# ChuhanZhou/News_Recommendation_Model

Hardware: NVIDIA B200
Metric: train_impressions_per_sec (higher is better)
Workload: dtype f32 (pair products as 3 x bf16 tcgen05 MMAs, fp32 accumulate; meets the fp32 tolerances)

## Files before the change

include/nrm_b200.h:

```cpp
#ifndef NRM_B200_H
#define NRM_B200_H

#include <stddef.h>
#include <stdint.h>

#ifdef __cplusplus
extern "C" {
#endif

#define NRM_OK            0
#define NRM_EINVAL       -1
#define NRM_EWORKSPACE   -2
#define NRM_ECUDA        -3
#define NRM_EUNSUPPORTED -4

#define NRM_PRECISION_FP32 0
#define NRM_PRECISION_BF16 1
#define NRM_PRECISION_BF16X3 2

#define NRM_MODE_BN_BATCH_STATS 1
#define NRM_MODE_KEEP_FOR_BWD   2
#define NRM_MODE_EVAL           0
#define NRM_MODE_TRAIN          3

int         nrm_version(void);
const char* nrm_last_error(void);

unsigned long long nrm_launch_count(void);
void        nrm_timing_enable(int on);
int         nrm_timing_report(char* buf, size_t buf_bytes);
int         nrm_debug_umma_selftest(const float* a0, const float* a1, const float* b0, const float* b1,
                                    float* out, int mode, int split, void* stream);

int         nrm_debug_mma_microbench(long long* out, int variant, int reps, int nk, void* stream);

size_t      nrm_peer_ctx_bytes(void);
size_t      nrm_peer_stats_bytes(void);
int         nrm_peer_flag_words(void);
int         nrm_peer_preload(void);
int         nrm_adam_step_allreduce(float* param, float* exp_avg, float* exp_avg_sq, long long n, void* adam_state,
                                    const void* peer_ctx, void* ticket, void* stream);
int         nrm_loss_backward_sparse(const long long* user_id, int B, int C, const float* grad_loss, float* dlogits, long long delta_numel,
                                     long long* sparse_uid, float* sparse_val, const void* scratch, size_t scratch_bytes, void* stream);
int         nrm_peer_wait_consumed(const void* adam_state, const void* peer_ctx, void* stream);
int         nrm_peer_allsum_stats(const double* local, int which, double* out, const void* adam_state, const void* peer_ctx, void* stream);

int         nrm_debug_rsprof(long long* host_out64);
long long   nrm_debug_ws_field(int B, int H, int C, int mode, const char* name, long long* bytes);
int         nrm_debug_headprof(long long* host_out32);

int         nrm_layout_entries(void);
const char* nrm_layout_name(int i);
long long   nrm_layout_offset(int i);
long long   nrm_layout_numel(int i);
long long   nrm_layout_fixed_floats(void);

size_t nrm_workspace_bytes(int B, int H, int C, int mode);
size_t nrm_workspace_e_offset(int B, int H, int C, int mode);

int nrm_forward(const double* x_history, const double* x_target, long long x_target_batch_stride,
                const double* x_global, long long x_global_batch_stride,
                int B, int H, int C,
                const float* params, float* bn_running_mean, float* bn_running_var,
                long long* bn_num_batches_tracked,
                int mode, int precision,
                float* logits, void* workspace, size_t workspace_bytes, void* stream);

int nrm_forward_encoder(const double* x_history, const double* x_target, long long x_target_batch_stride,
                        const double* x_global, long long x_global_batch_stride,
                        int B, int H, int C, const float* params, int mode, int precision,
                        double* bn_sums, void* workspace, size_t workspace_bytes, void* stream);
int nrm_forward_head(int B, int H, int C, const float* params, float* bn_running_mean, float* bn_running_var,
                     long long* bn_num_batches_tracked, int mode, int precision,
                     const double* bn_sums, long long bn_global_rows,
                     float* logits, void* workspace, size_t workspace_bytes, void* stream);

int nrm_backward(const double* x_history, const double* x_target, long long x_target_batch_stride,
                 const double* x_global, long long x_global_batch_stride,
                 int B, int H, int C, const float* params, int mode, int precision,
                 const float* dlogits, float* grads,
                 void* workspace, size_t workspace_bytes, void* stream);
int nrm_backward_head(int B, int H, int C, const float* params, int precision, const float* dlogits, float* grads,
                      double* bn_bwd_sums, void* workspace, size_t workspace_bytes, void* stream);
int nrm_backward_head_deferred(int B, int H, int C, const float* params, int precision, const float* dlogits, float* grads,
                               double* bn_bwd_sums, void* workspace, size_t workspace_bytes, void* stream);
int nrm_backward_encoder(const double* x_history, const double* x_target, long long x_target_batch_stride,
                         const double* x_global, long long x_global_batch_stride,
                         int B, int H, int C, const float* params, int mode, int precision,
                         const double* bn_bwd_sums, long long bn_global_rows, float* grads,
                         void* workspace, size_t workspace_bytes, void* stream);

typedef struct {
  const float* articles; int n_articles;
  const int* hist_article; const unsigned* hist_time; const float* hist_click;
  const int* cand_article; const unsigned* cand_time;
  const float* label32; double* label64;
} nrm_compact_batch;
int nrm_forward_compact(const nrm_compact_batch* batch, int B, int H, int C, const float* params, float* bn_running_mean,
                        float* bn_running_var, long long* bn_num_batches_tracked, int mode, int precision,
                        float* logits, void* workspace, size_t workspace_bytes, void* stream);
int nrm_forward_encoder_compact(const nrm_compact_batch* batch, int B, int H, int C, const float* params, int mode, int precision,
                                double* bn_sums, void* workspace, size_t workspace_bytes, void* stream);
int nrm_backward_compact(const nrm_compact_batch* batch, int B, int H, int C, const float* params, int mode, int precision,
                         const float* dlogits, float* grads, void* workspace, size_t workspace_bytes, void* stream);
int nrm_backward_encoder_compact(const nrm_compact_batch* batch, int B, int H, int C, const float* params, int mode, int precision,
                                 const double* bn_bwd_sums, long long bn_global_rows, float* grads, void* workspace,
                                 size_t workspace_bytes, void* stream);

int nrm_forward_scores(const double* x_history, const double* x_target, long long x_target_batch_stride,
                       const double* x_global, long long x_global_batch_stride, int B, int H, int C,
                       const float* params, float* bn_running_mean, float* bn_running_var, long long* bn_num_batches_tracked,
                       int mode, int precision, float* logits, float* scores, void* workspace, size_t workspace_bytes, void* stream);
int nrm_forward_scores_compact(const nrm_compact_batch* batch, int B, int H, int C, const float* params, float* bn_running_mean,
                               float* bn_running_var, long long* bn_num_batches_tracked, int mode, int precision,
                               float* logits, float* scores, void* workspace, size_t workspace_bytes, void* stream);
int nrm_history_topk(const float* scores, int B, int C, int H, int k, const double* x_history, const int* hist_article,
                     int* idx_out, float* val_out, void* stream);

size_t nrm_pool_workspace_bytes(int B, int H, int N, int chunk);
int nrm_forward_pool(const nrm_compact_batch* users, int B, int H, int N, int chunk, const float* params, const float* bn_running_mean,
                     const float* bn_running_var, int precision, float* logits, void* workspace, size_t workspace_bytes, void* stream);
int nrm_pool_topk(const float* logits, int n_models, long long model_stride, int B, int N, int k, const int* pool_article, int n_articles,
                  const int* hist_article, int H, int* pos_out, float* val_out, void* stream);

size_t nrm_loss_scratch_bytes(int B, int C);
int nrm_loss_forward(const float* logits, const float* delta, long long delta_numel,
                     const long long* user_id, const double* label, int B, int C, float alpha,
                     float* loss, void* scratch, size_t scratch_bytes, void* stream);
int nrm_loss_backward(const long long* user_id, int B, int C, const float* grad_loss,
                      float* dlogits, float* ddelta, long long delta_numel,
                      const void* scratch, size_t scratch_bytes, void* stream);

int nrm_adam_step(float* param, const float* grad, float* exp_avg, float* exp_avg_sq, long long n,
                  float lr, float beta1, float beta2, float eps, float weight_decay,
                  long long step, float grad_scale, void* stream);

int nrm_adam_step_device(float* param, const float* grad, float* exp_avg, float* exp_avg_sq, long long n,
                         void* adam_state, void* stream);

int nrm_batch_metrics(const float* scores, long long score_stride, const double* labels, long long label_stride,
                      const int* n_valid, int B, int C, int k, float* auc, float* hit, float* rr, float* ndcg,
                      void* stream);

int nrm_score_epilogue(const float* logits, int n_models, long long model_stride, long long row_stride, int B, int C,
                       const long long* empty_num, float* scores, int* ranks, void* stream);

size_t nrm_rank_strings_capacity(int B, int C);
int nrm_rank_strings(const long long* impression_id, const int* ranks, const long long* empty_num, int B, int C,
                     long long* offsets, char* out, long long capacity, void* stream);

int nrm_expand_compact(const float* articles, int n_articles, const int* hist_article, const unsigned* hist_time,
                       const float* hist_click, const int* cand_article, const unsigned* cand_time, const float* label32,
                       int B, int H, int C, double* x_history, double* x_target, double* x_global, double* label64,
                       void* stream);

#ifdef __cplusplus
}
#endif
#endif
```

news_recommendation_model_b200/_lib.py:

```python
from __future__ import annotations

import ctypes as C
import os
import subprocess
import threading

_HERE = os.path.dirname(os.path.abspath(__file__))
CSRC = os.path.join(_HERE, 'csrc')
LIB_PATH = os.path.join(CSRC, 'libnrm_b200.so')

_lock = threading.Lock()
_lib = None

vp, ll, i32, f32, sz = C.c_void_p, C.c_longlong, C.c_int, C.c_float, C.c_size_t

SIGNATURES = {
    'nrm_version': (i32, []),
    'nrm_last_error': (C.c_char_p, []),
    'nrm_launch_count': (C.c_ulonglong, []),
    'nrm_timing_enable': (None, [i32]),
    'nrm_timing_report': (i32, [C.c_char_p, sz]),
    'nrm_debug_umma_selftest': (i32, [vp, vp, vp, vp, vp, i32, i32, vp]),
    'nrm_debug_mma_microbench': (i32, [vp, i32, i32, i32, vp]),
    'nrm_debug_rsprof': (i32, [vp]),
    'nrm_debug_headprof': (i32, [vp]),
    'nrm_debug_ws_field': (ll, [i32, i32, i32, i32, C.c_char_p, vp]),
    'nrm_layout_entries': (i32, []),
    'nrm_layout_name': (C.c_char_p, [i32]),
    'nrm_layout_offset': (ll, [i32]),
    'nrm_layout_numel': (ll, [i32]),
    'nrm_layout_fixed_floats': (ll, []),
    'nrm_workspace_bytes': (sz, [i32, i32, i32, i32]),
    'nrm_workspace_e_offset': (sz, [i32, i32, i32, i32]),
    'nrm_forward': (i32, [vp, vp, ll, vp, ll, i32, i32, i32, vp, vp, vp, vp, i32, i32, vp, vp, sz, vp]),
    'nrm_forward_encoder': (i32, [vp, vp, ll, vp, ll, i32, i32, i32, vp, i32, i32, vp, vp, sz, vp]),
    'nrm_forward_head': (i32, [i32, i32, i32, vp, vp, vp, vp, i32, i32, vp, ll, vp, vp, sz, vp]),
    'nrm_backward': (i32, [vp, vp, ll, vp, ll, i32, i32, i32, vp, i32, i32, vp, vp, vp, sz, vp]),
    'nrm_forward_compact': (i32, [vp, i32, i32, i32, vp, vp, vp, vp, i32, i32, vp, vp, sz, vp]),
    'nrm_forward_encoder_compact': (i32, [vp, i32, i32, i32, vp, i32, i32, vp, vp, sz, vp]),
    'nrm_backward_compact': (i32, [vp, i32, i32, i32, vp, i32, i32, vp, vp, vp, sz, vp]),
    'nrm_backward_encoder_compact': (i32, [vp, i32, i32, i32, vp, i32, i32, vp, ll, vp, vp, sz, vp]),
    'nrm_backward_head': (i32, [i32, i32, i32, vp, i32, vp, vp, vp, vp, sz, vp]),
    'nrm_backward_head_deferred': (i32, [i32, i32, i32, vp, i32, vp, vp, vp, vp, sz, vp]),
    'nrm_backward_encoder': (i32, [vp, vp, ll, vp, ll, i32, i32, i32, vp, i32, i32, vp, ll, vp, vp, sz, vp]),
    'nrm_loss_scratch_bytes': (sz, [i32, i32]),
    'nrm_loss_forward': (i32, [vp, vp, ll, vp, vp, i32, i32, f32, vp, vp, sz, vp]),
    'nrm_loss_backward': (i32, [vp, i32, i32, vp, vp, vp, ll, vp, sz, vp]),
    'nrm_adam_step': (i32, [vp, vp, vp, vp, ll, f32, f32, f32, f32, f32, ll, f32, vp]),
    'nrm_adam_step_device': (i32, [vp, vp, vp, vp, ll, vp, vp]),
    'nrm_peer_ctx_bytes': (sz, []),
    'nrm_peer_stats_bytes': (sz, []),
    'nrm_peer_flag_words': (i32, []),
    'nrm_peer_preload': (i32, []),
    'nrm_adam_step_allreduce': (i32, [vp, vp, vp, ll, vp, vp, vp, vp]),
    'nrm_peer_wait_consumed': (i32, [vp, vp, vp]),
    'nrm_loss_backward_sparse': (i32, [vp, i32, i32, vp, vp, ll, vp, vp, vp, sz, vp]),
    'nrm_peer_allsum_stats': (i32, [vp, i32, vp, vp, vp, vp]),
    'nrm_batch_metrics': (i32, [vp, ll, vp, ll, vp, i32, i32, i32, vp, vp, vp, vp, vp]),
    'nrm_score_epilogue': (i32, [vp, i32, ll, ll, i32, i32, vp, vp, vp, vp]),
    'nrm_rank_strings_capacity': (sz, [i32, i32]),
    'nrm_rank_strings': (i32, [vp, vp, vp, i32, i32, vp, vp, ll, vp]),
    'nrm_expand_compact': (i32, [vp, i32, vp, vp, vp, vp, vp, vp, i32, i32, i32, vp, vp, vp, vp, vp]),
    'nrm_forward_scores': (i32, [vp, vp, ll, vp, ll, i32, i32, i32, vp, vp, vp, vp, i32, i32, vp, vp, vp, sz, vp]),
    'nrm_forward_scores_compact': (i32, [vp, i32, i32, i32, vp, vp, vp, vp, i32, i32, vp, vp, vp, sz, vp]),
    'nrm_history_topk': (i32, [vp, i32, i32, i32, i32, vp, vp, vp, vp, vp]),
    'nrm_pool_workspace_bytes': (sz, [i32, i32, i32, i32]),
    'nrm_forward_pool': (i32, [vp, i32, i32, i32, i32, vp, vp, vp, i32, vp, vp, sz, vp]),
    'nrm_pool_topk': (i32, [vp, i32, ll, i32, i32, i32, vp, i32, vp, i32, vp, vp, vp]),
}


class NrmError(RuntimeError):
    pass


def build(verbose: bool = False) -> str:
    out = subprocess.run(['make', '-C', CSRC, '-j8'], capture_output=True, text=True)
    if verbose or out.returncode != 0:
        print(out.stdout[-4000:])
        print(out.stderr[-4000:])
    if out.returncode != 0:
        raise NrmError('building libnrm_b200.so failed (see make output above)')
    return LIB_PATH


def load():
    global _lib
    with _lock:
        if _lib is not None:
            return _lib
        if not os.path.exists(LIB_PATH):
            raise NrmError(f'{LIB_PATH} is missing: run `python -c "import __graft_entry__ as g; g.build()"` '
                           f'(or `make -C {CSRC}`); there is no CPU fallback')
        lib = C.CDLL(LIB_PATH)
        for name, (res, args) in SIGNATURES.items():
            fn = getattr(lib, name)
            fn.restype = res
            fn.argtypes = args
        _lib = lib
        return lib


def check(rc: int, what: str) -> None:
    if rc != 0:
        msg = load().nrm_last_error().decode('utf-8', 'replace')
        raise NrmError(f'{what} failed with code {rc}: {msg}')


def layout():
    lib = load()
    entries = [(lib.nrm_layout_name(i).decode(), int(lib.nrm_layout_offset(i)), int(lib.nrm_layout_numel(i)))
               for i in range(lib.nrm_layout_entries())]
    return entries, int(lib.nrm_layout_fixed_floats())


class CompactBatchStruct(C.Structure):
    _fields_ = [('articles', C.c_void_p), ('n_articles', C.c_int), ('hist_article', C.c_void_p), ('hist_time', C.c_void_p),
                ('hist_click', C.c_void_p), ('cand_article', C.c_void_p), ('cand_time', C.c_void_p), ('label32', C.c_void_p),
                ('label64', C.c_void_p)]
```

news_recommendation_model_b200/csrc/nrm_api.cu:

```cuda
#include <cstdarg>
#include <cstdio>
#include <cstring>
#include <mutex>
#include <vector>

#include "nrm_kernels.cuh"

namespace nrm {

static thread_local char g_err[512] = "";

void set_error(const char* fmt, ...) {
  va_list ap;
  va_start(ap, fmt);
  vsnprintf(g_err, sizeof(g_err), fmt, ap);
  va_end(ap);
}
int cuda_fail(cudaError_t e, const char* what) {
  set_error("CUDA error %d (%s) at %s", (int)e, cudaGetErrorString(e), what);
  return NRM_ECUDA;
}
int current_device() {
  int dev = 0;
  if (cudaGetDevice(&dev) != cudaSuccess || dev < 0 || dev >= 64) return 0;
  return dev;
}
int sm_count() {
  static int n[64] = {};
  const int dev = current_device();
  int v = __atomic_load_n(&n[dev], __ATOMIC_RELAXED);
  if (v == 0) {
    if (cudaDeviceGetAttribute(&v, cudaDevAttrMultiProcessorCount, dev) != cudaSuccess || v <= 0) v = 148;
    __atomic_store_n(&n[dev], v, __ATOMIC_RELAXED);
  }
  return v;
}

static unsigned long long g_launches = 0;
void count_launch() { __atomic_fetch_add(&g_launches, 1ULL, __ATOMIC_RELAXED); }

constexpr int kTimerSlots = 40, kTimerRing = 256;
struct TimerSlot { const char* name; cudaEvent_t beg[kTimerRing], end[kTimerRing]; int used; bool made; };
static TimerSlot g_timers[kTimerSlots];
static int g_ntimers = 0;
static bool g_timing = false;
static std::mutex g_timer_mu;

KernelTimer::KernelTimer(const char* name, cudaStream_t stream) : slot_(-1), stream_(stream) {
  if (!g_timing) return;
  std::lock_guard<std::mutex> lock(g_timer_mu);
  int s = -1;
  for (int i = 0; i < g_ntimers; ++i) if (strcmp(g_timers[i].name, name) == 0) { s = i; break; }
  if (s < 0) { if (g_ntimers == kTimerSlots) return; s = g_ntimers++; g_timers[s].name = name; g_timers[s].used = 0; g_timers[s].made = false; }
  TimerSlot& t = g_timers[s];
  if (!t.made) { for (int i = 0; i < kTimerRing; ++i) { cudaEventCreate(&t.beg[i]); cudaEventCreate(&t.end[i]); } t.made = true; }
  if (t.used >= kTimerRing) return;
  slot_ = s;
  cudaEventRecord(t.beg[t.used], stream_);
}
KernelTimer::~KernelTimer() {
  if (slot_ < 0) return;
  std::lock_guard<std::mutex> lock(g_timer_mu);
  TimerSlot& t = g_timers[slot_];
  cudaEventRecord(t.end[t.used], stream_);
  t.used++;
}

struct SideStream {
  int dev; cudaStream_t caller;
  cudaStream_t stream; cudaEvent_t fork, join, fork2, join2, fork0, join0, join_tp, fork3, join3, fork4, join4;
  bool head_wgrad_pending = false; const float* wg_params = nullptr; float* wg_grads = nullptr; int wg_tiles = 0, wg_precision = 0;
};
static std::mutex g_side_mu;
static std::vector<SideStream*> g_sides;
static SideStream* side_stream(cudaStream_t caller) {
  const int dev = current_device();
  std::lock_guard<std::mutex> lock(g_side_mu);
  for (SideStream* p : g_sides)
    if (p->dev == dev && p->caller == caller) return p;
  SideStream* ss = new SideStream();
  ss->dev = dev; ss->caller = caller;
  bool ok = cudaStreamCreateWithFlags(&ss->stream, cudaStreamNonBlocking) == cudaSuccess;
  cudaEvent_t* evs[] = {&ss->fork, &ss->join, &ss->fork2, &ss->join2, &ss->fork0, &ss->join0, &ss->join_tp, &ss->fork3, &ss->join3,
                        &ss->fork4, &ss->join4};
  for (cudaEvent_t* e : evs) ok = ok && cudaEventCreateWithFlags(e, cudaEventDisableTiming) == cudaSuccess;
  if (!ok) { delete ss; return nullptr; }
  g_sides.push_back(ss);
  return ss;
}

bool pdl_enabled() {
  static const bool on = getenv("NRM_NO_PDL") == nullptr;
  return on;
}

struct LayoutEntry { const char* name; long long offset; long long numel; };
#define II "invariant_interest_model."
static const LayoutEntry kLayout[] = {
    {II "category_embedding.0.weight", P_CAT, NCAT * 32},
    {II "sentiment_embedding.0.weight", P_SENT_W, 16 * 3},
    {II "sentiment_embedding.0.bias", P_SENT_B, 16},
    {II "type_embedding.0.weight", P_TYPE, NTYPE * 8},
    {II "w1.weight", P_W1_W, 64 * XIN},
    {II "w1.bias", P_W1_B, 64},
    {II "year_embedding.0.weight", P_YEAR, NYEAR * 8},
    {II "month_embedding.0.weight", P_MONTH, NMONTH * 8},
    {II "day_embedding.0.weight", P_DAY, NDAY * 8},
    {II "hour_embedding.0.weight", P_HOUR, NHOUR * 8},
    {II "label_attention.mlp.fc1.weight", P_LA_FC1_W, 64 * 256},
    {II "label_attention.mlp.fc1.bias", P_LA_FC1_B, 64},
    {II "label_attention.mlp.fc2.weight", P_LA_FC2_W, 64},
    {II "label_attention.mlp.fc2.bias", P_LA_FC2_B, 1},
    {II "text_img_attention.mlp.fc1.weight", P_TI_FC1_W, 64 * 256},
    {II "text_img_attention.mlp.fc1.bias", P_TI_FC1_B, 64},
    {II "text_img_attention.mlp.fc2.weight", P_TI_FC2_W, 64},
    {II "text_img_attention.mlp.fc2.bias", P_TI_FC2_B, 1},
    {"instant_interest_model.out_fc.0.weight", P_INST_W, 8 * 3},
    {"instant_interest_model.out_fc.0.bias", P_INST_B, 8},
    {"bn.weight", P_BN_W, E},
    {"bn.bias", P_BN_B, E},
    {"gate.fc1.weight", P_GATE_FC1_W, HID * E},
    {"gate.fc1.bias", P_GATE_FC1_B, HID},
    {"gate.fc2.weight", P_GATE_FC2_W, E * HID},
    {"gate.fc2.bias", P_GATE_FC2_B, E},
    {"mlp.fc1.weight", P_MLP_FC1_W, HID * E},
    {"mlp.fc1.bias", P_MLP_FC1_B, HID},
    {"mlp.fc2.weight", P_MLP_FC2_W, E * HID},
    {"mlp.fc2.bias", P_MLP_FC2_B, E},
    {"out_mlp.fc1.weight", P_OUT_FC1_W, HID * E},
    {"out_mlp.fc1.bias", P_OUT_FC1_B, HID},
    {"out_mlp.fc2.weight", P_OUT_FC2_W, HID},
    {"out_mlp.fc2.bias", P_OUT_FC2_B, 1},
    {"delta", P_DELTA, -1},
};
#undef II
constexpr int kLayoutEntries = sizeof(kLayout) / sizeof(kLayout[0]);

size_t carve_workspace(Workspace& w, void* base, int B, int H, int C, int mode) {
  const bool training = (mode & NRM_MODE_KEEP_FOR_BWD) != 0;
  memset(&w, 0, sizeof(w));
  w.B = B; w.H = H; w.C = C;
  w.NH = (long long)B * H; w.R = (long long)B * C; w.N = w.NH + w.R;
  size_t off = 0;
  auto take = [&](size_t bytes) -> void* {
    void* p = base ? (char*)base + off : nullptr;
    off += (bytes + 255) & ~(size_t)255;
    return p;
  };
  const size_t f = sizeof(float);
  const size_t NH = (size_t)w.NH, R = (size_t)w.R, N = (size_t)w.N;
  w.xin_h = (float*)take(f * NH * XIN);
  w.xh = (float*)take(f * NH * 64);
  w.pca_h = (float*)take(f * NH * 64);
  w.e = (float*)take(f * R * E);
  w.mean = (float*)take(f * E);
  w.rstd = (float*)take(f * E);
  w.bn_sums = (double*)take(sizeof(double) * 2 * E);
  w.stat_part = (double*)take(sizeof(double) * STAT_BLOCKS * 2 * E);
  w.a1 = (float*)take(f * R * HID);
  w.gate = (float*)take(f * R * E);
  w.a2 = (float*)take(f * R * HID);
  w.y = (float*)take(f * R * E);
  w.a3 = (float*)take(f * R * HID);
  w.head_wt = (float*)take(f * (HEAD_WT_W1T + 64 * XIN));
  w.tp = (float*)take(f * 2 * R * 64);
  w.att_rs_img = (float*)take(attention_rs_image_bytes());
  w.head_img = (float*)take(head_tc_image_bytes());
  w.head_arrive = (unsigned int*)take(256);
  if (training) {
    w.da3 = (float*)take(f * R * HID); w.da2 = (float*)take(f * R * HID); w.da1 = (float*)take(f * R * HID);
    w.dy = (float*)take(f * R * E);
    w.dgate = (float*)take(f * R * E);
    w.de = (float*)take(f * R * E);
    w.dz = (float*)take(f * R * E);
    w.bn_bwd_sums = (double*)take(sizeof(double) * 2 * E);
    w.head_part_f = (float*)take(f * ((R + 31) / 32) * 68);
    w.head_part_bn = (double*)take(sizeof(double) * ((R + 31) / 32) * 2 * E);
    w.head_part_w = (float*)take(f * 5 * HEAD_WG_CHUNKS_MAX * (HID * E + E));
    w.dxh = (float*)take(f * NH * 64);
    w.dxt = (float*)take(f * R * 64);
    w.dxin_h = (float*)take(f * NH * XIN);
    {
      const size_t ffma = (size_t)ATT_BWD_CTAS_MAX * ATT_PARTIAL, tc = (size_t)ATT_TC_PARTS_MAX * ATT_TC_PARTIAL;
      w.att_part = (float*)take(f * 2 * (ffma > tc ? ffma : tc));
    }
    w.dtp = (float*)take(f * 2 * R * 64);
    {
      const size_t tiles = (size_t)attention_rs_tiles(B, H, C);
      w.att_dhid = (unsigned char*)take(tiles * 2 * 16384);
      w.att_sc = (float*)take(f * tiles * 512);
    }
    w.att_dA = (float*)take(f * 2 * 4096);
    w.tp_part = (float*)take(f * 2 * ((R + 31) / 32) * (4096 + 64));
    w.splitk = (float*)take(f * (size_t)(64 * XIN + 64) * W1_SPLITS);
    w.small_part = (float*)take(f * 1024 * 96);
    const size_t n32 = N * 6, n8 = N * 5;
    const size_t c32 = (n32 + SORT_CHUNK - 1) / SORT_CHUNK, c8 = (n8 + SORT_CHUNK - 1) / SORT_CHUNK;
    const size_t g32 = n32 / SEG_GROUP + NKEY32 + 1, g8 = n8 / SEG_GROUP + NKEY8 + 1;
    w.keys32 = (int*)take(sizeof(int) * n32); w.keys8 = (int*)take(sizeof(int) * n8);
    w.perm32 = (int*)take(sizeof(int) * n32); w.perm8 = (int*)take(sizeof(int) * n8);
    w.chunk_hist32 = (int*)take(sizeof(int) * c32 * NKEY32); w.chunk_hist8 = (int*)take(sizeof(int) * c8 * NKEY8);
    w.seg32 = (int*)take(sizeof(int) * 3 * (NKEY32 + 1)); w.seg8 = (int*)take(sizeof(int) * 3 * (NKEY8 + 1));
    w.gkey32 = (int*)take(sizeof(int) * g32); w.gkey8 = (int*)take(sizeof(int) * g8);
    w.gpart32 = (float*)take(f * g32 * 32); w.gpart8 = (float*)take(f * g8 * 8);
  }
  w.bytes = off;
  return off;
}

static int check_shape(const char* fn, int B, int H, int C) {
  if (B <= 0 || H <= 0 || C <= 0) { set_error("%s: B, H, C must be positive (got %d, %d, %d)", fn, B, H, C); return NRM_EINVAL; }
  if (((long long)B * H + (long long)B * C) * 6 >= (1LL << 31)) { set_error("%s: batch too large for 32-bit entry ids", fn); return NRM_EINVAL; }
  return NRM_OK;
}
static int get_workspace(const char* fn, Workspace& w, void* ws, size_t ws_bytes, int B, int H, int C, int mode) {
  if (ws == nullptr || ((uintptr_t)ws & 255) != 0) { set_error("%s: workspace must be non-null and 256-byte aligned", fn); return NRM_EWORKSPACE; }
  const size_t need = carve_workspace(w, ws, B, H, C, mode);
  if (need > ws_bytes) { set_error("%s: workspace too small (%zu < %zu bytes)", fn, ws_bytes, need); return NRM_EWORKSPACE; }
  return NRM_OK;
}

static int encoder_forward(const BatchPtrs& in, const float* P, Workspace& w, int mode, int precision, cudaStream_t s) {
  SideStream* ss = side_stream(s);
  if (ss == nullptr) { set_error("encoder_forward: cannot create the side stream"); return NRM_ECUDA; }
  const bool tc = precision != NRM_PRECISION_FP32;
  NRM_CUDA(cudaEventRecord(ss->fork0, s));
  NRM_CUDA(cudaStreamWaitEvent(ss->stream, ss->fork0, 0));
  NRM_TRY(launch_head_transpose(P, w, ss->stream));
  NRM_CUDA(cudaEventRecord(ss->join0, ss->stream));
  if (tc) {
    NRM_TRY(launch_attention_prep_rs(P, w, ss->stream));
    NRM_TRY(launch_head_images_tc(P, w, precision, (mode & NRM_MODE_KEEP_FOR_BWD) != 0, ss->stream));
  }
  { KernelTimer t("embed_rows", s);
    NRM_TRY(launch_embed_rows(in, P, w, (mode & NRM_MODE_KEEP_FOR_BWD) != 0, s)); }
  NRM_CUDA(cudaEventRecord(ss->fork, s));
  NRM_CUDA(cudaStreamWaitEvent(ss->stream, ss->fork, 0));
  if (tc) NRM_TRY(launch_candidate_tp(P, w, ss->stream));
  NRM_CUDA(cudaEventRecord(ss->join_tp, ss->stream));
  if (mode & NRM_MODE_KEEP_FOR_BWD) {
    NRM_TRY(launch_table_sort(w, ss->stream));
    NRM_CUDA(cudaEventRecord(ss->join, ss->stream));
  }
  NRM_CUDA(cudaStreamWaitEvent(s, ss->join0, 0));
  { KernelTimer t("w1_forward", s); NRM_TRY(launch_w1_forward(P, w, s)); }
  NRM_CUDA(cudaStreamWaitEvent(s, ss->join_tp, 0));
  if (!tc) {
    { KernelTimer t("attention_forward_label", s); NRM_TRY(launch_attention_forward(in, P, w, 0, precision, s)); }
    { KernelTimer t("attention_forward_textimg", s); NRM_TRY(launch_attention_forward(in, P, w, 1, precision, s)); }
  } else {
    KernelTimer t("attention_forward", s);
    NRM_TRY(launch_attention_forward_rs(in, w, precision, s));
  }
  if (mode & NRM_MODE_KEEP_FOR_BWD) NRM_CUDA(cudaStreamWaitEvent(s, ss->join, 0));
  return NRM_OK;
}

static int encoder_backward(const BatchPtrs& in, const float* P, Workspace& w, int precision, float* G, cudaStream_t s) {
  SideStream* ss = side_stream(s);
  if (ss == nullptr) { set_error("encoder_backward: cannot create the side stream"); return NRM_ECUDA; }
  const bool tc = precision != NRM_PRECISION_FP32;
  { KernelTimer t("attention_backward_label", s);
    if (tc) NRM_TRY(launch_attention_backward_rs(w, 0, precision, true, s)); else NRM_TRY(launch_attention_backward(in, P, w, 0, precision, s)); }
  if (tc) {
    KernelTimer t("attention_input_grad_label", s);
    NRM_TRY(launch_attention_input_grad_rs(w, precision, s));
  }
  NRM_CUDA(cudaEventRecord(ss->fork2, s));
  NRM_CUDA(cudaStreamWaitEvent(ss->stream, ss->fork2, 0));
  { KernelTimer t("attention_backward_textimg", s);
    if (tc) NRM_TRY(launch_attention_backward_rs(w, 1, precision, false, s)); else NRM_TRY(launch_attention_backward(in, P, w, 1, precision, s)); }
  { KernelTimer t("w1_backward", ss->stream);
    if (tc) NRM_TRY(launch_w1_backward_tc(P, w, G, precision, ss->stream)); else NRM_TRY(launch_w1_backward(P, w, G, ss->stream)); }
  NRM_CUDA(cudaEventRecord(ss->join2, ss->stream));
  if (ss->head_wgrad_pending) {
    ss->head_wgrad_pending = false;
    KernelTimer t("head_wgrad", ss->stream);
    NRM_TRY(launch_head_backward_wgrad(ss->wg_params, w, ss->wg_grads, ss->stream, ss->wg_tiles, ss->wg_precision));
  }
  { KernelTimer t("attention_finish", s);
    if (tc) NRM_TRY(launch_attention_finish_tc(P, w, G, s));
    else { NRM_TRY(launch_attention_finish(P, w, 0, precision, G, s)); NRM_TRY(launch_attention_finish(P, w, 1, precision, G, s)); } }
  NRM_CUDA(cudaStreamWaitEvent(s, ss->join2, 0));
  NRM_CUDA(cudaEventRecord(ss->fork3, s));
  NRM_CUDA(cudaStreamWaitEvent(ss->stream, ss->fork3, 0));
  { KernelTimer t("small_linear_grads", ss->stream); NRM_TRY(launch_small_linear_grads(in, w, G, ss->stream)); }
  NRM_CUDA(cudaEventRecord(ss->join3, ss->stream));
  NRM_TRY(launch_table_grads(w, G, s));
  NRM_CUDA(cudaStreamWaitEvent(s, ss->join3, 0));
  return NRM_OK;
}

}

using namespace nrm;

extern "C" int nrm_version(void) { return 100; }
extern "C" unsigned long long nrm_launch_count(void) { return __atomic_load_n(&g_launches, __ATOMIC_RELAXED); }
extern "C" void nrm_timing_enable(int on) {
  std::lock_guard<std::mutex> lock(g_timer_mu);
  g_timing = on != 0;
  for (int i = 0; i < g_ntimers; ++i) g_timers[i].used = 0;
}
extern "C" int nrm_timing_report(char* buf, size_t buf_bytes) {
  if (!buf || buf_bytes == 0) { set_error("nrm_timing_report: bad buffer"); return NRM_EINVAL; }
  size_t off = 0;
  buf[0] = 0;
  std::lock_guard<std::mutex> lock(g_timer_mu);
  for (int i = 0; i < g_ntimers; ++i) {
    TimerSlot& t = g_timers[i];
    double total = 0.0;
    for (int k = 0; k < t.used; ++k) {
      float ms = 0.f;
      NRM_CUDA(cudaEventSynchronize(t.end[k]));
      NRM_CUDA(cudaEventElapsedTime(&ms, t.beg[k], t.end[k]));
      total += ms;
    }
    float t_beg = 0.f, t_end = 0.f;
    if (t.used > 0 && g_ntimers > 0 && g_timers[0].used > 0) {
      cudaEventElapsedTime(&t_beg, g_timers[0].beg[g_timers[0].used - 1], t.beg[t.used - 1]);
      cudaEventElapsedTime(&t_end, g_timers[0].beg[g_timers[0].used - 1], t.end[t.used - 1]);
    }
    const int n = snprintf(buf + off, buf_bytes - off, "%s %d %.6f %.6f %.6f\n", t.name, t.used, total, t_beg, t_end);
    if (n < 0 || (size_t)n >= buf_bytes - off) break;
    off += (size_t)n;
  }
  return NRM_OK;
}
extern "C" int nrm_debug_rsprof(long long* host_out64) { return rsprof_read(host_out64); }
extern "C" long long nrm_debug_ws_field(int B, int H, int C, int mode, const char* name, long long* bytes) {
  if (B <= 0 || H <= 0 || C <= 0 || !name || !bytes) return -1;
  Workspace w;
  carve_workspace(w, reinterpret_cast<void*>(uintptr_t(256)), B, H, C, mode);
  const size_t R = (size_t)w.R, NH = (size_t)w.NH;
  struct F { const char* n; const void* p; size_t b; };
  const F fields[] = {{"e", w.e, R * E * 4}, {"de", w.de, R * E * 4}, {"dz", w.dz, R * E * 4}, {"dxh", w.dxh, NH * 64 * 4}, {"dxt", w.dxt, R * 64 * 4},
                      {"dxin_h", w.dxin_h, NH * XIN * 4}, {"att_dhid", w.att_dhid, (size_t)attention_rs_tiles(B, H, C) * 2 * 16384},
                      {"att_sc", w.att_sc, (size_t)attention_rs_tiles(B, H, C) * 512 * 4}, {"xh", w.xh, NH * 64 * 4}, {"dtp", w.dtp, 2 * R * 64 * 4},
                      {"tp", w.tp, 2 * R * 64 * 4}};
  for (const F& f : fields)
    if (strcmp(f.n, name) == 0 && f.p != nullptr) { *bytes = (long long)f.b; return (long long)(reinterpret_cast<uintptr_t>(f.p) - 256); }
  return -1;
}
extern "C" int nrm_debug_headprof(long long* host_out32) { return headprof_read(host_out32); }
extern "C" const char* nrm_last_error(void) { return g_err; }
extern "C" int nrm_layout_entries(void) { return kLayoutEntries; }
extern "C" const char* nrm_layout_name(int i) { return (i >= 0 && i < kLayoutEntries) ? kLayout[i].name : nullptr; }
extern "C" long long nrm_layout_offset(int i) { return (i >= 0 && i < kLayoutEntries) ? kLayout[i].offset : -1; }
extern "C" long long nrm_layout_numel(int i) { return (i >= 0 && i < kLayoutEntries) ? kLayout[i].numel : -1; }
extern "C" long long nrm_layout_fixed_floats(void) { return P_DELTA; }

extern "C" size_t nrm_workspace_bytes(int B, int H, int C, int mode) {
  if (B <= 0 || H <= 0 || C <= 0) return 0;
  Workspace w;
  return carve_workspace(w, nullptr, B, H, C, mode);
}

extern "C" size_t nrm_workspace_e_offset(int B, int H, int C, int mode) {
  if (B <= 0 || H <= 0 || C <= 0) return 0;
  Workspace w;
  carve_workspace(w, reinterpret_cast<void*>(uintptr_t(256)), B, H, C, mode);
  return (size_t)(reinterpret_cast<uintptr_t>(w.e) - 256);
}

static int forward_encoder_impl(const char* fn, const BatchPtrs& in, int B, int H, int C, const float* params, int mode, int precision,
                                double* bn_sums, void* workspace, size_t workspace_bytes, void* stream) {
  Workspace w;
  NRM_TRY(get_workspace(fn, w, workspace, workspace_bytes, B, H, C, mode));
  cudaStream_t s = (cudaStream_t)stream;
  NRM_TRY(encoder_forward(in, params, w, mode, precision, s));
  if (mode & NRM_MODE_BN_BATCH_STATS) {
    KernelTimer t("bn_statistics", s);
    NRM_TRY(launch_bn_partial_sums(w, s));
    if (bn_sums != nullptr && bn_sums != w.bn_sums)
      NRM_CUDA(cudaMemcpyAsync(bn_sums, w.bn_sums, sizeof(double) * 2 * E, cudaMemcpyDeviceToDevice, s));
  }
  return NRM_OK;
}

static int compact_batch(const char* fn, const nrm_compact_batch* cb, int precision, CompactPtrs& cp) {
  if (!cb || !cb->articles || cb->n_articles <= 0 || !cb->hist_article || !cb->hist_time || !cb->hist_click || !cb->cand_article || !cb->cand_time ||
      (cb->label32 && !cb->label64)) {
    set_error("%s: bad compact batch", fn); return NRM_EINVAL;
  }
  if ((reinterpret_cast<uintptr_t>(cb->articles) & 15) != 0) { set_error("%s: the article table must be 16-byte aligned", fn); return NRM_EINVAL; }
  if (precision == NRM_PRECISION_FP32) {
    set_error("%s: the compact wire format is read directly by the tensor-core precisions only (use nrm_expand_compact otherwise)", fn);
    return NRM_EUNSUPPORTED;
  }
  cp = CompactPtrs{cb->articles, cb->n_articles, cb->hist_article, cb->hist_time, cb->hist_click, cb->cand_article, cb->cand_time,
                   cb->label32, cb->label64};
  return NRM_OK;
}

extern "C" int nrm_forward_encoder(const double* x_history, const double* x_target, long long xt_bs, const double* x_global,
                                   long long xg_bs, int B, int H, int C, const float* params, int mode, int precision,
                                   double* bn_sums, void* workspace, size_t workspace_bytes, void* stream) {
  NRM_TRY(check_shape("nrm_forward_encoder", B, H, C));
  if (!x_history || !x_target || !x_global || !params) { set_error("nrm_forward_encoder: null pointer"); return NRM_EINVAL; }
  if (xt_bs < (long long)C * TC || xg_bs < (long long)C * GC) { set_error("nrm_forward_encoder: batch stride smaller than one impression"); return NRM_EINVAL; }
  const BatchPtrs in{x_history, x_target, xt_bs, x_global, xg_bs};
  return forward_encoder_impl("nrm_forward_encoder", in, B, H, C, params, mode, precision, bn_sums, workspace, workspace_bytes, stream);
}

extern "C" int nrm_forward_encoder_compact(const nrm_compact_batch* batch, int B, int H, int C, const float* params, int mode, int precision,
                                           double* bn_sums, void* workspace, size_t workspace_bytes, void* stream) {
  NRM_TRY(check_shape("nrm_forward_encoder_compact", B, H, C));
  if (!params) { set_error("nrm_forward_encoder_compact: null pointer"); return NRM_EINVAL; }
  CompactPtrs cp;
  NRM_TRY(compact_batch("nrm_forward_encoder_compact", batch, precision, cp));
  BatchPtrs in{nullptr, nullptr, 0, nullptr, 0};
  in.compact = &cp;
  return forward_encoder_impl("nrm_forward_encoder_compact", in, B, H, C, params, mode, precision, bn_sums, workspace, workspace_bytes, stream);
}

extern "C" int nrm_forward_head(int B, int H, int C, const float* params, float* bn_running_mean, float* bn_running_var,
                                  long long* bn_num_batches_tracked, int mode, int precision, const double* bn_sums,
                                  long long bn_global_rows, float* logits, void* workspace, size_t workspace_bytes,
                                  void* stream) {
  const int training = mode & NRM_MODE_BN_BATCH_STATS;
  NRM_TRY(check_shape("nrm_forward_head", B, H, C));
  if (!params || !bn_running_mean || !bn_running_var || !logits) { set_error("nrm_forward_head: null pointer"); return NRM_EINVAL; }
  if (training && !bn_num_batches_tracked) { set_error("nrm_forward_head: null num_batches_tracked"); return NRM_EINVAL; }
  Workspace w;
  NRM_TRY(get_workspace("nrm_forward_head", w, workspace, workspace_bytes, B, H, C, mode));
  const double* sums = bn_sums ? bn_sums : w.bn_sums;
  const long long rows = bn_global_rows > 0 ? bn_global_rows : w.R;
  KernelTimer t("head_forward", (cudaStream_t)stream);
  if (precision != NRM_PRECISION_FP32)
    return launch_head_forward_tc(params, w, precision, bn_running_mean, bn_running_var, bn_num_batches_tracked, training,
                                  (mode & NRM_MODE_KEEP_FOR_BWD) != 0, sums, rows, logits, (cudaStream_t)stream);
  return launch_head_forward(params, w, bn_running_mean, bn_running_var, bn_num_batches_tracked, training,
                             (mode & NRM_MODE_KEEP_FOR_BWD) != 0, sums, rows,
                             logits, (cudaStream_t)stream);
}

extern "C" int nrm_forward(const double* x_history, const double* x_target, long long xt_bs, const double* x_global,
                           long long xg_bs, int B, int H, int C, const float* params, float* bn_running_mean,
                           float* bn_running_var, long long* bn_num_batches_tracked, int mode, int precision,
                           float* logits, void* workspace, size_t workspace_bytes, void* stream) {
  NRM_TRY(nrm_forward_encoder(x_history, x_target, xt_bs, x_global, xg_bs, B, H, C, params, mode, precision, nullptr,
                              workspace, workspace_bytes, stream));
  return nrm_forward_head(B, H, C, params, bn_running_mean, bn_running_var, bn_num_batches_tracked, mode, precision, nullptr, 0,
                            logits, workspace, workspace_bytes, stream);
}

extern "C" int nrm_forward_compact(const nrm_compact_batch* batch, int B, int H, int C, const float* params, float* bn_running_mean,
                                   float* bn_running_var, long long* bn_num_batches_tracked, int mode, int precision,
                                   float* logits, void* workspace, size_t workspace_bytes, void* stream) {
  NRM_TRY(nrm_forward_encoder_compact(batch, B, H, C, params, mode, precision, nullptr, workspace, workspace_bytes, stream));
  return nrm_forward_head(B, H, C, params, bn_running_mean, bn_running_var, bn_num_batches_tracked, mode, precision, nullptr, 0,
                            logits, workspace, workspace_bytes, stream);
}

static int forward_scores_impl(const char* fn, const BatchPtrs& in, int B, int H, int C, const float* params, float* bn_running_mean,
                               float* bn_running_var, long long* bn_num_batches_tracked, int mode, int precision, float* logits,
                               float* scores, void* workspace, size_t workspace_bytes, void* stream) {
  if (mode != NRM_MODE_EVAL) { set_error("%s: scores are exported by eval-mode forwards only (mode must be NRM_MODE_EVAL, got %d)", fn, mode); return NRM_EINVAL; }
  if (!scores) { set_error("%s: null scores", fn); return NRM_EINVAL; }
  Workspace w;
  NRM_TRY(get_workspace(fn, w, workspace, workspace_bytes, B, H, C, mode));
  w.scores = scores;
  NRM_TRY(encoder_forward(in, params, w, mode, precision, (cudaStream_t)stream));
  return nrm_forward_head(B, H, C, params, bn_running_mean, bn_running_var, bn_num_batches_tracked, mode, precision, nullptr, 0,
                          logits, workspace, workspace_bytes, stream);
}

extern "C" int nrm_forward_scores(const double* x_history, const double* x_target, long long xt_bs, const double* x_global,
                                  long long xg_bs, int B, int H, int C, const float* params, float* bn_running_mean,
                                  float* bn_running_var, long long* bn_num_batches_tracked, int mode, int precision,
                                  float* logits, float* scores, void* workspace, size_t workspace_bytes, void* stream) {
  NRM_TRY(check_shape("nrm_forward_scores", B, H, C));
  if (!x_history || !x_target || !x_global || !params) { set_error("nrm_forward_scores: null pointer"); return NRM_EINVAL; }
  if (xt_bs < (long long)C * TC || xg_bs < (long long)C * GC) { set_error("nrm_forward_scores: batch stride smaller than one impression"); return NRM_EINVAL; }
  const BatchPtrs in{x_history, x_target, xt_bs, x_global, xg_bs};
  return forward_scores_impl("nrm_forward_scores", in, B, H, C, params, bn_running_mean, bn_running_var, bn_num_batches_tracked, mode,
                             precision, logits, scores, workspace, workspace_bytes, stream);
}

extern "C" int nrm_forward_scores_compact(const nrm_compact_batch* batch, int B, int H, int C, const float* params, float* bn_running_mean,
                                          float* bn_running_var, long long* bn_num_batches_tracked, int mode, int precision,
                                          float* logits, float* scores, void* workspace, size_t workspace_bytes, void* stream) {
  NRM_TRY(check_shape("nrm_forward_scores_compact", B, H, C));
  if (!params) { set_error("nrm_forward_scores_compact: null pointer"); return NRM_EINVAL; }
  CompactPtrs cp;
  NRM_TRY(compact_batch("nrm_forward_scores_compact", batch, precision, cp));
  BatchPtrs in{nullptr, nullptr, 0, nullptr, 0};
  in.compact = &cp;
  return forward_scores_impl("nrm_forward_scores_compact", in, B, H, C, params, bn_running_mean, bn_running_var, bn_num_batches_tracked,
                             mode, precision, logits, scores, workspace, workspace_bytes, stream);
}

struct PoolCarve { double* xh; double* xt; double* xg; float* out; void* ws; size_t ws_bytes, bytes; };
static void carve_pool(PoolCarve& pc, void* base, int B, int H, int N, int chunk) {
  const int C = chunk < N ? chunk : N;
  size_t off = 0;
  auto take = [&](size_t bytes) -> void* {
    void* p = base ? (char*)base + off : nullptr;
    off += (bytes + 255) & ~(size_t)255;
    return p;
  };
  pc.xh = (double*)take(sizeof(double) * B * H * HC);
  pc.xt = (double*)take(sizeof(double) * C * TC);
  pc.xg = (double*)take(sizeof(double) * C * GC);
  pc.out = (float*)take(sizeof(float) * B * C);
  Workspace w;
  pc.ws_bytes = carve_workspace(w, nullptr, B, H, C, NRM_MODE_EVAL);
  pc.ws = take(pc.ws_bytes);
  pc.bytes = off;
}

extern "C" size_t nrm_pool_workspace_bytes(int B, int H, int N, int chunk) {
  if (B <= 0 || H <= 0 || N <= 0 || chunk <= 0) return 0;
  PoolCarve pc;
  carve_pool(pc, nullptr, B, H, N, chunk);
  return pc.bytes;
}

extern "C" int nrm_forward_pool(const nrm_compact_batch* users, int B, int H, int N, int chunk, const float* params,
                                const float* bn_running_mean, const float* bn_running_var, int precision, float* logits,
                                void* workspace, size_t workspace_bytes, void* stream) {
  const char* fn = "nrm_forward_pool";
  if (B <= 0 || H <= 0 || N <= 0) { set_error("%s: B, H, N must be positive (got %d, %d, %d)", fn, B, H, N); return NRM_EINVAL; }
  if (chunk <= 0 || chunk % 8 != 0) { set_error("%s: chunk must be a positive multiple of 8 (got %d)", fn, chunk); return NRM_EINVAL; }
  if (precision < NRM_PRECISION_FP32 || precision > NRM_PRECISION_BF16X3) { set_error("%s: unknown precision %d", fn, precision); return NRM_EINVAL; }
  if (!users || !users->articles || users->n_articles <= 0 || !users->hist_article || !users->hist_time || !users->hist_click ||
      !users->cand_article || !users->cand_time) {
    set_error("%s: bad compact batch", fn); return NRM_EINVAL;
  }
  if (users->label32 || users->label64) { set_error("%s: the pool has no labels (label32 / label64 must be null)", fn); return NRM_EINVAL; }
  if ((reinterpret_cast<uintptr_t>(users->articles) & 15) != 0) { set_error("%s: the article table must be 16-byte aligned", fn); return NRM_EINVAL; }
  if (!params || !bn_running_mean || !bn_running_var || !logits) { set_error("%s: null pointer", fn); return NRM_EINVAL; }
  const int C = chunk < N ? chunk : N;
  NRM_TRY(check_shape(fn, B, H, C));
  if (workspace == nullptr || ((uintptr_t)workspace & 255) != 0) { set_error("%s: workspace must be non-null and 256-byte aligned", fn); return NRM_EWORKSPACE; }
  PoolCarve pc;
  carve_pool(pc, workspace, B, H, N, chunk);
  if (pc.bytes > workspace_bytes) { set_error("%s: workspace too small (%zu < %zu bytes)", fn, workspace_bytes, pc.bytes); return NRM_EWORKSPACE; }
  cudaStream_t s = (cudaStream_t)stream;
  const nrm_compact_batch& u = *users;
  NRM_TRY(launch_expand_compact(u.articles, u.n_articles, u.hist_article, u.hist_time, u.hist_click, nullptr, nullptr, nullptr, (long long)B * H, 0,
                                pc.xh, nullptr, nullptr, nullptr, s));
  float* run_mean = const_cast<float*>(bn_running_mean);
  float* run_var = const_cast<float*>(bn_running_var);
  for (int c0 = 0; c0 < N; c0 += C) {
    const int nc = N - c0 < C ? N - c0 : C;
    NRM_TRY(launch_expand_compact(u.articles, u.n_articles, nullptr, nullptr, nullptr, u.cand_article + c0, u.cand_time + c0, nullptr, 0, nc,
                                  nullptr, pc.xt, pc.xg, nullptr, s));
    const BatchPtrs in{pc.xh, pc.xt, 0, pc.xg, 0};
    NRM_TRY(forward_encoder_impl(fn, in, B, H, nc, params, NRM_MODE_EVAL, precision, nullptr, pc.ws, pc.ws_bytes, stream));
    float* out = nc == N ? logits : pc.out;
    NRM_TRY(nrm_forward_head(B, H, nc, params, run_mean, run_var, nullptr, NRM_MODE_EVAL, precision, nullptr, 0, out, pc.ws, pc.ws_bytes, stream));
    if (out != logits)
      NRM_CUDA(cudaMemcpy2DAsync(logits + c0, sizeof(float) * N, out, sizeof(float) * nc, sizeof(float) * nc, B, cudaMemcpyDeviceToDevice, s));
  }
  return NRM_OK;
}

static int backward_head(const char* fn, bool defer_wgrad, int B, int H, int C, const float* params, int precision, const float* dlogits, float* grads,
                         double* bn_bwd_sums, void* workspace, size_t workspace_bytes, void* stream) {
  NRM_TRY(check_shape(fn, B, H, C));
  if (!params || !dlogits || !grads) { set_error("%s: null pointer", fn); return NRM_EINVAL; }
  Workspace w;
  NRM_TRY(get_workspace(fn, w, workspace, workspace_bytes, B, H, C, NRM_MODE_KEEP_FOR_BWD));
  cudaStream_t s = (cudaStream_t)stream;
  const bool tc = precision != NRM_PRECISION_FP32;
  const int tiles = tc ? head_tc_tiles(w.R) : 0;
  if (!defer_wgrad) {
    KernelTimer t("head_backward", s);
    if (tc) NRM_TRY(launch_head_backward_dgrad_tc(params, w, precision, dlogits, grads, s));
    else { NRM_TRY(launch_head_backward_dgrad(params, w, dlogits, s)); NRM_TRY(launch_head_backward_bn(w, grads, s, 0)); }
    NRM_TRY(launch_head_backward_wgrad(params, w, grads, s, tiles, tc ? precision : 0));
  } else {
    SideStream* ss = side_stream(s);
    if (ss == nullptr) { set_error("%s: cannot create the side stream", fn); return NRM_ECUDA; }
    KernelTimer t("head_backward", s);
    if (tc) NRM_TRY(launch_head_backward_dgrad_tc(params, w, precision, dlogits, grads, s)); else NRM_TRY(launch_head_backward_dgrad(params, w, dlogits, s));
    ss->head_wgrad_pending = true; ss->wg_params = params; ss->wg_grads = grads; ss->wg_tiles = tiles; ss->wg_precision = tc ? precision : 0;
    if (!tc) NRM_TRY(launch_head_backward_bn(w, grads, s, 0));
  }
  if (bn_bwd_sums != nullptr && bn_bwd_sums != w.bn_bwd_sums)
    NRM_CUDA(cudaMemcpyAsync(bn_bwd_sums, w.bn_bwd_sums, sizeof(double) * 2 * E, cudaMemcpyDeviceToDevice, s));
  return NRM_OK;
}

extern "C" int nrm_backward_head(int B, int H, int C, const float* params, int precision, const float* dlogits, float* grads,
                                 double* bn_bwd_sums, void* workspace, size_t workspace_bytes, void* stream) {
  return backward_head("nrm_backward_head", false, B, H, C, params, precision, dlogits, grads, bn_bwd_sums, workspace, workspace_bytes, stream);
}

extern "C" int nrm_backward_head_deferred(int B, int H, int C, const float* params, int precision, const float* dlogits, float* grads,
                                          double* bn_bwd_sums, void* workspace, size_t workspace_bytes, void* stream) {
  return backward_head("nrm_backward_head_deferred", true, B, H, C, params, precision, dlogits, grads, bn_bwd_sums, workspace, workspace_bytes, stream);
}

static int backward_encoder_impl(const char* fn, const BatchPtrs& in, int B, int H, int C, const float* params, int mode, int precision,
                                 const double* bn_bwd_sums, long long bn_global_rows, float* grads, void* workspace, size_t workspace_bytes,
                                 void* stream) {
  const int training = mode & NRM_MODE_BN_BATCH_STATS;
  Workspace w;
  NRM_TRY(get_workspace(fn, w, workspace, workspace_bytes, B, H, C, NRM_MODE_KEEP_FOR_BWD));
  cudaStream_t s = (cudaStream_t)stream;
  const double* sums = bn_bwd_sums ? bn_bwd_sums : w.bn_bwd_sums;
  const long long rows = bn_global_rows > 0 ? bn_global_rows : w.R;
  NRM_TRY(launch_bn_backward_combine(params, w, training, sums, rows, precision != NRM_PRECISION_FP32, s));
  return encoder_backward(in, params, w, precision, grads, s);
}

extern "C" int nrm_backward_encoder(const double* x_history, const double* x_target, long long xt_bs,
                                    const double* x_global, long long xg_bs, int B, int H, int C, const float* params,
                                    int mode, int precision, const double* bn_bwd_sums, long long bn_global_rows,
                                    float* grads, void* workspace, size_t workspace_bytes, void* stream) {
  NRM_TRY(check_shape("nrm_backward_encoder", B, H, C));
  if (!x_history || !x_target || !x_global || !params || !grads) { set_error("nrm_backward_encoder: null pointer"); return NRM_EINVAL; }
  const BatchPtrs in{x_history, x_target, xt_bs, x_global, xg_bs};
  return backward_encoder_impl("nrm_backward_encoder", in, B, H, C, params, mode, precision, bn_bwd_sums, bn_global_rows, grads, workspace,
                               workspace_bytes, stream);
}

extern "C" int nrm_backward_encoder_compact(const nrm_compact_batch* batch, int B, int H, int C, const float* params, int mode, int precision,
                                            const double* bn_bwd_sums, long long bn_global_rows, float* grads, void* workspace,
                                            size_t workspace_bytes, void* stream) {
  NRM_TRY(check_shape("nrm_backward_encoder_compact", B, H, C));
  if (!params || !grads) { set_error("nrm_backward_encoder_compact: null pointer"); return NRM_EINVAL; }
  CompactPtrs cp;
  NRM_TRY(compact_batch("nrm_backward_encoder_compact", batch, precision, cp));
  BatchPtrs in{nullptr, nullptr, 0, nullptr, 0};
  in.compact = &cp;
  return backward_encoder_impl("nrm_backward_encoder_compact", in, B, H, C, params, mode, precision, bn_bwd_sums, bn_global_rows, grads, workspace,
                               workspace_bytes, stream);
}

static int backward_impl(const char* fn, const BatchPtrs& in, int B, int H, int C, const float* params, int mode, int precision,
                         const float* dlogits, float* grads, void* workspace, size_t workspace_bytes, void* stream) {
  const int training = mode & NRM_MODE_BN_BATCH_STATS;
  Workspace w;
  NRM_TRY(get_workspace(fn, w, workspace, workspace_bytes, B, H, C, NRM_MODE_KEEP_FOR_BWD));
  cudaStream_t s = (cudaStream_t)stream;
  SideStream* ss = side_stream(s);
  if (ss == nullptr) { set_error("%s: cannot create the side stream", fn); return NRM_ECUDA; }
  const bool htc = precision != NRM_PRECISION_FP32;
  const int tiles = htc ? head_tc_tiles(w.R) : 0;
  { KernelTimer t("head_backward", s);
    if (htc) NRM_TRY(launch_head_backward_dgrad_tc(params, w, precision, dlogits, grads, s)); else NRM_TRY(launch_head_backward_dgrad(params, w, dlogits, s));
    ss->head_wgrad_pending = true; ss->wg_params = params; ss->wg_grads = grads; ss->wg_tiles = tiles; ss->wg_precision = htc ? precision : 0;
    if (!htc) NRM_TRY(launch_head_backward_bn(w, grads, s, 0)); }
  NRM_TRY(launch_bn_backward_combine(params, w, training, w.bn_bwd_sums, w.R, htc, s));
  return encoder_backward(in, params, w, precision, grads, s);
}

extern "C" int nrm_backward(const double* x_history, const double* x_target, long long xt_bs, const double* x_global,
                            long long xg_bs, int B, int H, int C, const float* params, int mode, int precision,
                            const float* dlogits, float* grads, void* workspace, size_t workspace_bytes, void* stream) {
  NRM_TRY(check_shape("nrm_backward", B, H, C));
  if (!x_history || !x_target || !x_global || !params || !dlogits || !grads) { set_error("nrm_backward: null pointer"); return NRM_EINVAL; }
  const BatchPtrs in{x_history, x_target, xt_bs, x_global, xg_bs};
  return backward_impl("nrm_backward", in, B, H, C, params, mode, precision, dlogits, grads, workspace, workspace_bytes, stream);
}

extern "C" int nrm_backward_compact(const nrm_compact_batch* batch, int B, int H, int C, const float* params, int mode, int precision,
                                    const float* dlogits, float* grads, void* workspace, size_t workspace_bytes, void* stream) {
  NRM_TRY(check_shape("nrm_backward_compact", B, H, C));
  if (!params || !dlogits || !grads) { set_error("nrm_backward_compact: null pointer"); return NRM_EINVAL; }
  CompactPtrs cp;
  NRM_TRY(compact_batch("nrm_backward_compact", batch, precision, cp));
  BatchPtrs in{nullptr, nullptr, 0, nullptr, 0};
  in.compact = &cp;
  return backward_impl("nrm_backward_compact", in, B, H, C, params, mode, precision, dlogits, grads, workspace, workspace_bytes, stream);
}
```

news_recommendation_model_b200/csrc/nrm_head_tc.cu:

```cuda
#include "nrm_kernels.cuh"
#include <cstddef>

#include "nrm_umma.cuh"

namespace nrm {
namespace htc {

#ifdef NRM_RS_PROFILE
__device__ long long g_hprof[32];
#define HPROF(role, kind, stmt) do { const long long t__ = clock64(); stmt; if (blockIdx.x == 0 && (threadIdx.x & 31) == 0) g_hprof[(role) * 8 + (kind)] += clock64() - t__; } while (0)
#else
#define HPROF(role, kind, stmt) do { stmt; } while (0)
#endif

constexpr int ROWS = 64;
constexpr int N_EPI = 16;
constexpr int W_MMA = 16, W_LOAD = 17;
constexpr int THREADS = 32 * 20;
constexpr int EPI_THREADS = 32 * N_EPI;
constexpr int KE = 272, KH = 80;
constexpr int NN = 72;
constexpr int NW0 = 136, NW1 = 128;
constexpr uint32_t A_LBO = ROWS * 16;
constexpr uint32_t AW_PART = (KE / 8) * A_LBO;
constexpr uint32_t AN_PART = (KH / 8) * A_LBO;
constexpr uint32_t BN_LBO = NN * 16;
constexpr uint32_t BW_LBO = E * 16;
constexpr int NCHUNK = 5;
constexpr uint32_t SLOT = 3 * 8 * BN_LBO;
constexpr int STAGES = 3;
constexpr uint32_t IMG_STRIDE = 3 * (KH / 8) * BW_LBO;
constexpr uint32_t COL_W = 0, COL_N = 160, TMEM_COLS = 256;
constexpr int PAR_GAMMA = 0, PAR_BETA = E, PAR_BG2 = 2 * E, PAR_BM2 = 3 * E, PAR_BG1 = 4 * E, PAR_BM1 = 4 * E + NN, PAR_BO1 = 4 * E + 2 * NN,
              PAR_WO2 = 4 * E + 3 * NN, PAR_FLOATS = 8 * E;

__host__ __device__ constexpr int narrow_chunk_kb(int c) { return c < 4 ? 8 : 2; }
template <int NP> __host__ __device__ constexpr uint32_t narrow_chunk_off(int c) { return (uint32_t)c * NP * 8 * BN_LBO; }
template <int NP> __host__ __device__ constexpr uint32_t wide_chunk_off(int c) { return (uint32_t)c * NP * 2 * BW_LBO; }

__host__ __device__ constexpr int n_products(int NP) { return NP == 1 ? 1 : NP == 2 ? 3 : 6; }
__host__ __device__ constexpr int prod_a(int NP, int p) { return NP == 2 ? (p == 2 ? 1 : 0) : (p == 2 || p == 3) ? 1 : p == 5 ? 2 : 0; }
__host__ __device__ constexpr int prod_b(int NP, int p) { return NP == 2 ? (p == 1 ? 1 : 0) : (p == 1 || p == 3) ? 1 : p == 4 ? 2 : 0; }

template <int NP>
__device__ __forceinline__ void split_store8(unsigned char* dst, uint32_t part_bytes, const float* v) {
  uint32_t h[4], m[4], l[4];
#pragma unroll
  for (int i = 0; i < 4; ++i) {
    const float a = v[2 * i], b = v[2 * i + 1];
    const __nv_bfloat162 hh = __floats2bfloat162_rn(a, b);
    h[i] = *reinterpret_cast<const uint32_t*>(&hh);
    if (NP >= 2) {
      const float ra = a - __uint_as_float(h[i] << 16), rb = b - __uint_as_float(h[i] & 0xffff0000u);
      const __nv_bfloat162 mm = __floats2bfloat162_rn(ra, rb);
      m[i] = *reinterpret_cast<const uint32_t*>(&mm);
      if (NP >= 3) {
        const __nv_bfloat162 ll = __floats2bfloat162_rn(ra - __uint_as_float(m[i] << 16), rb - __uint_as_float(m[i] & 0xffff0000u));
        l[i] = *reinterpret_cast<const uint32_t*>(&ll);
      }
    }
  }
  *reinterpret_cast<uint4*>(dst) = make_uint4(h[0], h[1], h[2], h[3]);
  if (NP >= 2) *reinterpret_cast<uint4*>(dst + part_bytes) = make_uint4(m[0], m[1], m[2], m[3]);
  if (NP >= 3) *reinterpret_cast<uint4*>(dst + 2 * part_bytes) = make_uint4(l[0], l[1], l[2], l[3]);
}

struct ImgDesc { long long src; int so, si, narrow; };
__constant__ ImgDesc c_img[10] = {
    {P_GATE_FC1_W, E, 1, 1},   {P_GATE_FC2_W, HID, 1, 0}, {P_MLP_FC1_W, E, 1, 1},  {P_MLP_FC2_W, HID, 1, 0}, {P_OUT_FC1_W, E, 1, 1},
    {P_OUT_FC1_W, 1, E, 0},    {P_MLP_FC2_W, 1, HID, 1},  {P_MLP_FC1_W, 1, E, 0},  {P_GATE_FC2_W, 1, HID, 1}, {P_GATE_FC1_W, 1, E, 0}};

template <int NP>
__global__ void __launch_bounds__(256)
head_image_kernel(const float* __restrict__ P, unsigned char* __restrict__ img, int first_layer, unsigned int* __restrict__ arrive) {
  pdl_wait();
  pdl_trigger();
  if (blockIdx.x == 0 && blockIdx.y == 0 && threadIdx.x == 0) *arrive = 0u;
  const int layer = first_layer + blockIdx.y;
  const ImgDesc d = c_img[layer];
  const float* src = P + d.src;
  unsigned char* out = img + (size_t)layer * IMG_STRIDE;
  const int nrow = d.narrow ? NN : E, nkb = d.narrow ? KE / 8 : KH / 8;
  const int nout = d.narrow ? HID : E, nin = d.narrow ? E : HID;
  for (int it = blockIdx.x * 256 + threadIdx.x; it < nrow * nkb; it += gridDim.x * 256) {
    const int n = it % nrow, kb = it / nrow;
    float v[8];
#pragma unroll
    for (int i = 0; i < 8; ++i) {
      const int k = 8 * kb + i;
      v[i] = (n < nout && k < nin) ? __ldg(src + (long long)n * d.so + (long long)k * d.si) : 0.f;
    }
    uint32_t off, part;
    if (d.narrow) {
      const int c = kb < 32 ? kb >> 3 : 4, kbl = kb - 8 * c;
      part = (uint32_t)narrow_chunk_kb(c) * BN_LBO;
      off = narrow_chunk_off<NP>(c) + (uint32_t)kbl * BN_LBO;
    } else {
      const int c = kb >> 1, kbl = kb & 1;
      part = 2 * BW_LBO;
      off = wide_chunk_off<NP>(c) + (uint32_t)kbl * BW_LBO;
    }
    split_store8<NP>(out + off + (uint32_t)(n >> 3) * 128u + (uint32_t)(n & 7) * 16u, part, v);
  }
}

struct Smem {
  __align__(128) unsigned char aw[3 * AW_PART];
  __align__(128) unsigned char an[3 * AN_PART];
  __align__(128) unsigned char ring[STAGES][SLOT];
  float mean[E], rstd[E];
  float red[4][ROWS + 4];
  float par[PAR_FLOATS];
  uint64_t full[STAGES], empty[STAGES];
  uint64_t a_ready, d_ready;
  uint32_t tmem_base;
};

__device__ __forceinline__ void epi_sync() { __syncwarp(); asm volatile("bar.sync 1, %0;\n" ::"n"(EPI_THREADS) : "memory"); }
__device__ __forceinline__ void operand_written(uint64_t* bar) {
  umma::fence_async_smem();
  umma::fence_before_sync();
  __syncwarp();
  if ((threadIdx.x & 31) == 0) umma::mbar_arrive(bar);
}

template <int NP>
__device__ __forceinline__ void loader(Smem& sm, const unsigned char* __restrict__ img, int first_layer, bool first_narrow, long long my_tiles) {
  uint32_t g = 0;
  for (long long t = 0; t < my_tiles; ++t)
    for (int l = 0; l < 5; ++l) {
      const bool narrow = ((l & 1) == 0) == first_narrow;
      const unsigned char* base = img + (size_t)(first_layer + l) * IMG_STRIDE;
      for (int c = 0; c < NCHUNK; ++c, ++g) {
        const int slot = g % STAGES, use = g / STAGES;
        if (use > 0) HPROF(0, 0, umma::mbar_wait(&sm.empty[slot], (uint32_t)((use - 1) & 1)));
        const uint32_t off = narrow ? narrow_chunk_off<NP>(c) : wide_chunk_off<NP>(c);
        const uint32_t bytes = narrow ? (uint32_t)(NP * narrow_chunk_kb(c)) * BN_LBO : (uint32_t)NP * 2 * BW_LBO;
        umma::bulk_load(sm.ring[slot], base + off, bytes, &sm.full[slot]);
      }
    }
}

template <int NP, int KS>
__device__ __forceinline__ void narrow_chunk(uint32_t tmem_d, uint32_t a_addr, uint32_t b_addr, bool accumulate) {
  constexpr uint32_t ID_N = umma::make_idesc_bf16(64, NN);
  constexpr uint32_t bpart = (uint32_t)(2 * KS) * BN_LBO;
#pragma unroll
  for (int p = 0; p < n_products(NP); ++p) {
    const uint64_t da = umma::make_desc(a_addr + prod_a(NP, p) * AW_PART, A_LBO, 128);
    const uint64_t db = umma::make_desc(b_addr + prod_b(NP, p) * bpart, BN_LBO, 128);
#pragma unroll
    for (int ks = 0; ks < KS; ++ks)
      umma::mma_bf16(tmem_d, da + (uint64_t)(ks * ((2 * A_LBO) >> 4)), db + (uint64_t)(ks * ((2 * BN_LBO) >> 4)), ID_N,
                     (accumulate || p > 0 || ks > 0) ? 1u : 0u);
  }
}

template <int NP>
__device__ __forceinline__ void issuer(Smem& sm, uint32_t tmem, bool first_narrow, long long my_tiles) {
  constexpr uint32_t ID_W0 = umma::make_idesc_bf16(64, NW0), ID_W1 = umma::make_idesc_bf16(64, NW1);
  const uint32_t aw = umma::smem_u32(sm.aw), an = umma::smem_u32(sm.an);
  uint32_t g = 0, ause = 0;
  for (long long t = 0; t < my_tiles; ++t)
    for (int l = 0; l < 5; ++l) {
      const bool narrow = ((l & 1) == 0) == first_narrow;
      HPROF(1, 0, umma::mbar_wait(&sm.a_ready, ause & 1));
      ++ause;
      umma::fence_after_sync();
      for (int c = 0; c < NCHUNK; ++c, ++g) {
        const int slot = g % STAGES;
        HPROF(1, 1, umma::mbar_wait(&sm.full[slot], (uint32_t)((g / STAGES) & 1)));
        umma::fence_after_sync();
        const uint32_t rb = umma::smem_u32(sm.ring[slot]);
        if (narrow) {
          const uint32_t a0 = aw + (uint32_t)(8 * c) * A_LBO;
          if (c < 4) narrow_chunk<NP, 4>(tmem + COL_N, a0, rb, c > 0);
          else narrow_chunk<NP, 1>(tmem + COL_N, a0, rb, true);
        } else {
#pragma unroll
          for (int p = 0; p < n_products(NP); ++p) {
            const uint64_t da = umma::make_desc(an + prod_a(NP, p) * AN_PART + (uint32_t)(2 * c) * A_LBO, A_LBO, 128);
            const uint64_t db = umma::make_desc(rb + prod_b(NP, p) * (2 * BW_LBO), BW_LBO, 128);
            const uint32_t acc = (c > 0 || p > 0) ? 1u : 0u;
            umma::mma_bf16(tmem + COL_W, da, db, ID_W0, acc);
            umma::mma_bf16(tmem + COL_W + (16u << 16), da, db + (uint64_t)(((NW0 / 8) * 128) >> 4), ID_W1, acc);
          }
        }
        umma::mma_commit(&sm.empty[slot]);
      }
      umma::mma_commit(&sm.d_ready);
    }
}

__device__ __forceinline__ int wide_kb0(int q) { return q == 0 ? 0 : 4 * q + 1; }
__device__ __forceinline__ int wide_nkb(int q) { return q == 0 ? 5 : 4; }
__device__ __forceinline__ int narrow_kb0(int q) { return q == 0 ? 0 : 2 * q + 1; }
__device__ __forceinline__ int narrow_nkb(int q) { return q == 0 ? 3 : 2; }

__device__ __forceinline__ void load_wide(uint32_t tmem_lane, int q, float* v ) {
  const uint32_t a = tmem_lane + COL_W + 8 * wide_kb0(q);
  umma::tmem_ld32(a, v);
  if (q == 0) umma::tmem_ld8(a + 32, v + 32);
}
__device__ __forceinline__ void load_narrow(uint32_t tmem_lane, int q, float* v ) {
  const uint32_t a = tmem_lane + COL_N + 8 * narrow_kb0(q);
  umma::tmem_ld16(a, v);
  if (q == 0) umma::tmem_ld8(a + 16, v + 16);
}

__device__ __forceinline__ uint32_t a_off(int row, int kb) { return (uint32_t)kb * A_LBO + (uint32_t)(row >> 3) * 128u + (uint32_t)(row & 7) * 16u; }

template <int NP>
__global__ void __launch_bounds__(THREADS, 1)
head_forward_tc_kernel(const float* __restrict__ e, const double* __restrict__ bn_sums, long long bn_rows, int training,
                       float* __restrict__ run_mean, float* __restrict__ run_var, long long* __restrict__ nbt,
                       float* __restrict__ mean_out, float* __restrict__ rstd_out, const float* __restrict__ P,
                       const unsigned char* __restrict__ img, long long R, int keep, float* __restrict__ a1g, float* __restrict__ gateg,
                       float* __restrict__ a2g, float* __restrict__ yg, float* __restrict__ a3g, float* __restrict__ logits) {
#ifdef NRM_RS_PROFILE
  const long long t_entry = clock64();
#endif
  pdl_wait();
  pdl_trigger();
  extern __shared__ __align__(128) unsigned char smem_raw[];
  Smem& sm = *reinterpret_cast<Smem*>(smem_raw);
  const int tid = threadIdx.x, warp = tid >> 5, lane = tid & 31;
  const long long ntiles = (R + ROWS - 1) / ROWS;
  const long long my_tiles = (long long)blockIdx.x < ntiles ? (ntiles - 1 - blockIdx.x) / gridDim.x + 1 : 0;
  if (tid == 0) {
    for (int j = 0; j < STAGES; ++j) { umma::mbar_init(&sm.full[j], 1); umma::mbar_init(&sm.empty[j], 1); }
    umma::mbar_init(&sm.a_ready, N_EPI);
    umma::mbar_init(&sm.d_ready, 1);
  }
  if (warp == W_MMA) umma::tmem_alloc(&sm.tmem_base, TMEM_COLS);
  if (tid < ROWS) {
#pragma unroll
    for (int p = 0; p < 3; ++p) {
      *reinterpret_cast<uint4*>(sm.aw + p * AW_PART + a_off(tid, KE / 8 - 1)) = make_uint4(0, 0, 0, 0);
      *reinterpret_cast<uint4*>(sm.an + p * AN_PART + a_off(tid, KH / 8 - 1)) = make_uint4(0, 0, 0, 0);
    }
  }
  umma::fence_async_smem();
  umma::fence_before_sync();
  __syncthreads();
  umma::fence_after_sync();
  const uint32_t tmem = sm.tmem_base;

  if (warp >= N_EPI) {
    asm volatile("setmaxnreg.dec.sync.aligned.u32 32;\n");
    if (warp == W_LOAD) {
      if (umma::elect_one()) HPROF(0, 7, loader<NP>(sm, img, 0, true, my_tiles));
    } else if (warp == W_MMA) {
      if (umma::elect_one()) HPROF(1, 7, issuer<NP>(sm, tmem, true, my_tiles));
    }
  } else {
    asm volatile("setmaxnreg.inc.sync.aligned.u32 112;\n");
    const int sp = warp & 3, q = warp >> 2, l16 = lane & 15, half = lane >> 4;
    const int row = 16 * sp + l16;
    const uint32_t tmem_lane = tmem + ((uint32_t)(32 * sp) << 16);
    for (int i = tid; i < E; i += EPI_THREADS) {
      sm.par[PAR_GAMMA + i] = __ldg(P + P_BN_W + i); sm.par[PAR_BETA + i] = __ldg(P + P_BN_B + i);
      sm.par[PAR_BG2 + i] = __ldg(P + P_GATE_FC2_B + i); sm.par[PAR_BM2 + i] = __ldg(P + P_MLP_FC2_B + i);
    }
    if (tid < NN) {
      const bool in = tid < HID;
      sm.par[PAR_BG1 + tid] = in ? __ldg(P + P_GATE_FC1_B + tid) : 0.f; sm.par[PAR_BM1 + tid] = in ? __ldg(P + P_MLP_FC1_B + tid) : 0.f;
      sm.par[PAR_BO1 + tid] = in ? __ldg(P + P_OUT_FC1_B + tid) : 0.f;  sm.par[PAR_WO2 + tid] = in ? __ldg(P + P_OUT_FC2_W + tid) : 0.f;
    }
    if (tid < E) {
      const int n = tid;
      float m, v;
      if (training) {
        const double dm = bn_sums[n] / (double)bn_rows;
        double dv = bn_sums[E + n] / (double)bn_rows - dm * dm;
        if (dv < 0.0) dv = 0.0;
        m = (float)dm; v = (float)dv;
        if (blockIdx.x == 0) {
          const double unbiased = bn_rows > 1 ? dv * (double)bn_rows / (double)(bn_rows - 1) : dv;
          run_mean[n] = (1.f - BN_MOMENTUM) * run_mean[n] + BN_MOMENTUM * m;
          run_var[n] = (1.f - BN_MOMENTUM) * run_var[n] + BN_MOMENTUM * (float)unbiased;
          if (n == 0) *nbt += 1;
        }
      } else {
        m = run_mean[n]; v = run_var[n];
      }
      const float rs = 1.0f / sqrtf(v + BN_EPS);
      sm.mean[n] = m; sm.rstd[n] = rs;
      if (blockIdx.x == 0) { mean_out[n] = m; rstd_out[n] = rs; }
    }
    constexpr int PRO_ITEMS = ROWS * (E / 8), PRO_IT = (PRO_ITEMS + EPI_THREADS - 1) / EPI_THREADS;
    auto load_e_items = [&](long long r0, int nr, float4 (&ev)[PRO_IT][2]) {
#pragma unroll
      for (int u = 0; u < PRO_IT; ++u) {
        const int it = tid + u * EPI_THREADS, r = it & (ROWS - 1), kb = it >> 6;
        ev[u][0] = ev[u][1] = make_float4(0.f, 0.f, 0.f, 0.f);
        if (it < PRO_ITEMS && r < nr) {
          const float4* ep = reinterpret_cast<const float4*>(e + (r0 + r) * E + 8 * kb);
          ev[u][0] = __ldg(ep); ev[u][1] = __ldg(ep + 1);
        }
      }
    };
    epi_sync();
#ifdef NRM_RS_PROFILE
    if (blockIdx.x == 0 && tid == 0) g_hprof[24] += clock64() - t_entry;
#endif
    uint32_t duse = 0;
    for (long long t = 0; t < my_tiles; ++t) {
      const long long r0 = ((long long)blockIdx.x + t * gridDim.x) * ROWS;
      const int nr = (int)min((long long)ROWS, R - r0);
      const bool live = row < nr;
#ifdef NRM_RS_PROFILE
      const long long tp0 = clock64();
#endif
      float4 ev0[PRO_IT][2];
      load_e_items(r0, nr, ev0);
#pragma unroll
      for (int u = 0; u < PRO_IT; ++u) {
        const int it = tid + u * EPI_THREADS, r = it & (ROWS - 1), kb = it >> 6;
        if (it >= PRO_ITEMS) break;
        (void)nr;
        const float xv[8] = {ev0[u][0].x, ev0[u][0].y, ev0[u][0].z, ev0[u][0].w, ev0[u][1].x, ev0[u][1].y, ev0[u][1].z, ev0[u][1].w};
        float z[8];
#pragma unroll
        for (int i = 0; i < 8; ++i) {
          const int c = 8 * kb + i;
          z[i] = (xv[i] - sm.mean[c]) * sm.rstd[c] * sm.par[PAR_GAMMA + c] + sm.par[PAR_BETA + c];
        }
        split_store8<NP>(sm.aw + a_off(r, kb), AW_PART, z);
      }
      operand_written(&sm.a_ready);
#ifdef NRM_RS_PROFILE
      if (blockIdx.x == 0 && tid == 0) g_hprof[2 * 8 + 2] += clock64() - tp0;
#endif

      auto narrow_epilogue = [&](const float* bias, float* keepg, bool last, float& dot) {
        HPROF(2, 0, umma::mbar_wait(&sm.d_ready, duse & 1));
        ++duse;
        umma::fence_after_sync();
        float v[24];
        HPROF(2, 4, load_narrow(tmem_lane, q, v));
        umma::fence_before_sync();
        if (half == 0) {
          const int kb0 = narrow_kb0(q), nkb = narrow_nkb(q);
#pragma unroll
          for (int j = 0; j < 3; ++j) {
            if (j >= nkb) break;
            const int kb = kb0 + j;
            float a[8], gl[8];
#pragma unroll
            for (int i = 0; i < 8; ++i) {
              a[i] = v[8 * j + i] + bias[8 * kb + i];
              gl[i] = gelu_f(a[i]);
            }
            if (keepg != nullptr && live) {
              float* kp = keepg + (r0 + row) * HID + 8 * kb;
              if (kb < 8) {
#pragma unroll
                for (int i = 0; i < 4; ++i) reinterpret_cast<float2*>(kp)[i] = make_float2(a[2 * i], a[2 * i + 1]);
              } else {
                reinterpret_cast<float2*>(kp)[0] = make_float2(a[0], a[1]);
              }
            }
            if (last) {
#pragma unroll
              for (int i = 0; i < 8; ++i) dot = fmaf(gl[i], sm.par[PAR_WO2 + 8 * kb + i], dot);
            } else {
              split_store8<NP>(sm.an + a_off(row, kb), AN_PART, gl);
            }
          }
        }
      };
      auto wide_epilogue = [&](const float* bias, float* keepg, bool gating) {
        const int kb0 = wide_kb0(q);
        const int nkb = (half == 1 && q == 3) ? 3 : wide_nkb(q);
        const int c00 = NW0 * half + 8 * kb0;
        float4 ge[5][2];
        if (gating) {
#pragma unroll
          for (int j = 0; j < 5; ++j) {
            ge[j][0] = ge[j][1] = make_float4(0.f, 0.f, 0.f, 0.f);
            if (j < nkb && live) {
              const float4* ep = reinterpret_cast<const float4*>(e + (r0 + row) * E + c00 + 8 * j);
              ge[j][0] = __ldg(ep); ge[j][1] = __ldg(ep + 1);
            }
          }
        }
        HPROF(2, 1, umma::mbar_wait(&sm.d_ready, duse & 1));
        ++duse;
        umma::fence_after_sync();
        float v[40];
        HPROF(2, 4, load_wide(tmem_lane, q, v));
        umma::fence_before_sync();
#pragma unroll
        for (int j = 0; j < 5; ++j) {
          if (j >= nkb) break;
          const int c0 = c00 + 8 * j;
          float o[8];
          const float4 b0 = *reinterpret_cast<const float4*>(bias + c0), b1 = *reinterpret_cast<const float4*>(bias + c0 + 4);
          o[0] = v[8 * j] + b0.x; o[1] = v[8 * j + 1] + b0.y; o[2] = v[8 * j + 2] + b0.z; o[3] = v[8 * j + 3] + b0.w;
          o[4] = v[8 * j + 4] + b1.x; o[5] = v[8 * j + 5] + b1.y; o[6] = v[8 * j + 6] + b1.z; o[7] = v[8 * j + 7] + b1.w;
          if (live) {
            if (keepg != nullptr) {
              float4* kp = reinterpret_cast<float4*>(keepg + (r0 + row) * E + c0);
              kp[0] = make_float4(o[0], o[1], o[2], o[3]);
              kp[1] = make_float4(o[4], o[5], o[6], o[7]);
            }
            if (gating) {
              o[0] *= ge[j][0].x; o[1] *= ge[j][0].y; o[2] *= ge[j][0].z; o[3] *= ge[j][0].w;
              o[4] *= ge[j][1].x; o[5] *= ge[j][1].y; o[6] *= ge[j][1].z; o[7] *= ge[j][1].w;
            }
          } else {
#pragma unroll
            for (int i = 0; i < 8; ++i) o[i] = 0.f;
          }
          split_store8<NP>(sm.aw + a_off(row, (NW0 / 8) * half + kb0 + j), AW_PART, o);
        }
      };
      float dot = 0.f;
      narrow_epilogue(sm.par + PAR_BG1, keep ? a1g : nullptr, false, dot);
      HPROF(2, 3, operand_written(&sm.a_ready));
      wide_epilogue(sm.par + PAR_BG2, keep ? gateg : nullptr, true);
      HPROF(2, 3, operand_written(&sm.a_ready));
      narrow_epilogue(sm.par + PAR_BM1, keep ? a2g : nullptr, false, dot);
      HPROF(2, 3, operand_written(&sm.a_ready));
      wide_epilogue(sm.par + PAR_BM2, keep ? yg : nullptr, false);
      HPROF(2, 3, operand_written(&sm.a_ready));
      narrow_epilogue(sm.par + PAR_BO1, keep ? a3g : nullptr, true, dot);
      if (half == 0) sm.red[q][row] = dot;
      epi_sync();
#ifdef NRM_RS_PROFILE
      if (blockIdx.x == 0 && tid == 0) g_hprof[2 * 8 + 7] += clock64() - tp0;
#endif
      if (tid < ROWS && tid < nr) logits[r0 + tid] = ((sm.red[0][tid] + sm.red[1][tid]) + sm.red[2][tid]) + sm.red[3][tid] + __ldg(P + P_OUT_FC2_B);
      epi_sync();
    }
  }
  umma::fence_before_sync();
  __syncthreads();
  if (warp == W_MMA) umma::tmem_dealloc(tmem, TMEM_COLS);
#ifdef NRM_RS_PROFILE
  if (blockIdx.x == 0 && tid == 0) g_hprof[25] += clock64() - t_entry;
#endif
}


constexpr int HB_F = 68;

template <int NP>
__global__ void __launch_bounds__(THREADS, 1)
head_backward_tc_kernel(const float* __restrict__ e, const float* __restrict__ mean, const float* __restrict__ rstd,
                        const float* __restrict__ P, const unsigned char* __restrict__ img, long long R, const float* __restrict__ dr,
                        const float* __restrict__ a1g, const float* __restrict__ gateg, const float* __restrict__ a2g,
                        const float* __restrict__ a3g, float* __restrict__ da3g, float* __restrict__ dyg, float* __restrict__ da2g,
                        float* __restrict__ dgateg, float* __restrict__ da1g, float* __restrict__ dzg, float* __restrict__ deg,
                        float* __restrict__ part_f, double* __restrict__ part_bn, unsigned int* __restrict__ arrive,
                        float* __restrict__ grads, double* __restrict__ bn_bwd_sums) {
  pdl_wait();
  pdl_trigger();
  extern __shared__ __align__(128) unsigned char smem_raw[];
  Smem& sm = *reinterpret_cast<Smem*>(smem_raw);
  const int tid = threadIdx.x, warp = tid >> 5, lane = tid & 31;
  const long long ntiles = (R + ROWS - 1) / ROWS;
  const long long my_tiles = (long long)blockIdx.x < ntiles ? (ntiles - 1 - blockIdx.x) / gridDim.x + 1 : 0;
  if (tid == 0) {
    for (int j = 0; j < STAGES; ++j) { umma::mbar_init(&sm.full[j], 1); umma::mbar_init(&sm.empty[j], 1); }
    umma::mbar_init(&sm.a_ready, N_EPI);
    umma::mbar_init(&sm.d_ready, 1);
  }
  if (warp == W_MMA) umma::tmem_alloc(&sm.tmem_base, TMEM_COLS);
  if (tid < ROWS) {
#pragma unroll
    for (int p = 0; p < 3; ++p) {
      *reinterpret_cast<uint4*>(sm.aw + p * AW_PART + a_off(tid, KE / 8 - 1)) = make_uint4(0, 0, 0, 0);
      *reinterpret_cast<uint4*>(sm.an + p * AN_PART + a_off(tid, KH / 8 - 1)) = make_uint4(0, 0, 0, 0);
    }
  }
  umma::fence_async_smem();
  umma::fence_before_sync();
  __syncthreads();
  umma::fence_after_sync();
  const uint32_t tmem = sm.tmem_base;

  if (warp >= N_EPI) {
    asm volatile("setmaxnreg.dec.sync.aligned.u32 32;\n");
    if (warp == W_LOAD) {
      if (umma::elect_one()) loader<NP>(sm, img, 5, false, my_tiles);
    } else if (warp == W_MMA) {
      if (umma::elect_one()) issuer<NP>(sm, tmem, false, my_tiles);
    }
  } else {
    asm volatile("setmaxnreg.inc.sync.aligned.u32 112;\n");
    const int sp = warp & 3, q = warp >> 2, l16 = lane & 15, half = lane >> 4;
    const int row = 16 * sp + l16;
    const uint32_t tmem_lane = tmem + ((uint32_t)(32 * sp) << 16);
    for (int i = tid; i < E; i += EPI_THREADS) { sm.mean[i] = __ldg(mean + i); sm.rstd[i] = __ldg(rstd + i); }
    uint32_t duse = 0;
    for (long long t = 0; t < my_tiles; ++t) {
      const long long tile = (long long)blockIdx.x + t * gridDim.x;
      const long long r0 = tile * ROWS;
      const int nr = (int)min((long long)ROWS, R - r0);
      const bool live = row < nr;
      float* colsum = sm.par;
      constexpr int PRO_ITEMS = ROWS * (NN / 8);
#pragma unroll
      for (int u = 0; u < (PRO_ITEMS + EPI_THREADS - 1) / EPI_THREADS; ++u) {
        const int it = tid + u * EPI_THREADS;
        if (it >= PRO_ITEMS) break;
        const int r = it & (ROWS - 1), kb = it >> 6;
        float d[8], tg[8];
#pragma unroll
        for (int i = 0; i < 8; ++i) { d[i] = 0.f; tg[i] = 0.f; }
        if (r < nr) {
          const float drr = __ldg(dr + r0 + r);
          const float* ap = a3g + (r0 + r) * HID + 8 * kb;
          float av[8];
#pragma unroll
          for (int i = 0; i < 4; ++i) {
            float2 x = make_float2(0.f, 0.f);
            if (8 * kb + 2 * i < HID) x = __ldg(reinterpret_cast<const float2*>(ap) + i);
            av[2 * i] = x.x; av[2 * i + 1] = x.y;
          }
#pragma unroll
          for (int i = 0; i < 8; ++i) {
            const int c = 8 * kb + i;
            if (c < HID) {
              float gp;
              const float g = gelu_both(av[i], gp);
              d[i] = drr * __ldg(P + P_OUT_FC2_W + c) * gp;
              tg[i] = drr * g;
            }
          }
          float* dp = da3g + (r0 + r) * HID + 8 * kb;
#pragma unroll
          for (int i = 0; i < 4; ++i)
            if (8 * kb + 2 * i < HID) reinterpret_cast<float2*>(dp)[i] = make_float2(d[2 * i], d[2 * i + 1]);
        }
        split_store8<NP>(sm.an + a_off(r, kb), AN_PART, d);
#pragma unroll
        for (int i = 0; i < 8; ++i) {
#pragma unroll
          for (int o = 16; o > 0; o >>= 1) tg[i] += __shfl_xor_sync(0xffffffffu, tg[i], o);
        }
        if (lane == 0) {
#pragma unroll
          for (int i = 0; i < 8; ++i) colsum[(r >> 5) * NN + 8 * kb + i] = tg[i];
        }
      }
      operand_written(&sm.a_ready);
      if (warp == 0) {
        float s = (lane < nr ? __ldg(dr + r0 + lane) : 0.f) + (lane + 32 < nr ? __ldg(dr + r0 + lane + 32) : 0.f);
#pragma unroll
        for (int o = 16; o > 0; o >>= 1) s += __shfl_xor_sync(0xffffffffu, s, o);
        if (lane == 0) part_f[tile * HB_F + HID] = s;
      }
      epi_sync();
      if (tid < HID) part_f[tile * HB_F + tid] = colsum[tid] + colsum[NN + tid];

      auto wide_layer = [&](auto&& prefetch, auto&& finish, bool to_operand) {
        const int kb0 = wide_kb0(q);
        const int nkb = (half == 1 && q == 3) ? 3 : wide_nkb(q);
        const int c00 = NW0 * half + 8 * kb0;
        prefetch(c00, nkb);
        umma::mbar_wait(&sm.d_ready, duse & 1);
        ++duse;
        umma::fence_after_sync();
        float v[40];
        load_wide(tmem_lane, q, v);
        umma::fence_before_sync();
#pragma unroll
        for (int j = 0; j < 5; ++j) {
          if (j >= nkb) break;
          float o[8];
#pragma unroll
          for (int i = 0; i < 8; ++i) o[i] = live ? v[8 * j + i] : 0.f;
          finish(j, c00 + 8 * j, o);
          if (to_operand) split_store8<NP>(sm.aw + a_off(row, (NW0 / 8) * half + kb0 + j), AW_PART, o);
        }
      };
      auto narrow_layer = [&](const float* ag, float* dag) {
        const int kb0 = narrow_kb0(q), nkb = narrow_nkb(q);
        float av[24];
#pragma unroll
        for (int i = 0; i < 24; ++i) av[i] = 0.f;
        if (half == 0 && live) {
#pragma unroll
          for (int j = 0; j < 3; ++j) {
            if (j >= nkb) break;
            const float* ap = ag + (r0 + row) * HID + 8 * (kb0 + j);
#pragma unroll
            for (int i = 0; i < 4; ++i)
              if (8 * (kb0 + j) + 2 * i < HID) {
                const float2 x = __ldg(reinterpret_cast<const float2*>(ap) + i);
                av[8 * j + 2 * i] = x.x; av[8 * j + 2 * i + 1] = x.y;
              }
          }
        }
        umma::mbar_wait(&sm.d_ready, duse & 1);
        ++duse;
        umma::fence_after_sync();
        float v[24];
        load_narrow(tmem_lane, q, v);
        umma::fence_before_sync();
        if (half == 0) {
#pragma unroll
          for (int j = 0; j < 3; ++j) {
            if (j >= nkb) break;
            const int kb = kb0 + j;
            float d[8];
#pragma unroll
            for (int i = 0; i < 8; ++i) d[i] = (live && 8 * kb + i < HID) ? v[8 * j + i] * gelu_grad_f(av[8 * j + i]) : 0.f;
            if (live) {
              float* dp = dag + (r0 + row) * HID + 8 * kb;
#pragma unroll
              for (int i = 0; i < 4; ++i)
                if (8 * kb + 2 * i < HID) reinterpret_cast<float2*>(dp)[i] = make_float2(d[2 * i], d[2 * i + 1]);
            }
            split_store8<NP>(sm.an + a_off(row, kb), AN_PART, d);
          }
        }
      };
      auto store8 = [&](float* base, int c0, const float* o) {
        float4* p4 = reinterpret_cast<float4*>(base + (r0 + row) * E + c0);
        p4[0] = make_float4(o[0], o[1], o[2], o[3]);
        p4[1] = make_float4(o[4], o[5], o[6], o[7]);
      };
      auto load8 = [&](const float* base, int c0, float4 (&x)[2]) {
        const float4* p4 = reinterpret_cast<const float4*>(base + (r0 + row) * E + c0);
        x[0] = __ldg(p4); x[1] = __ldg(p4 + 1);
      };

      wide_layer([](int, int) {}, [&](int, int c0, float* o) { if (live) store8(dyg, c0, o); }, true);
      operand_written(&sm.a_ready);
      narrow_layer(a2g, da2g);
      operand_written(&sm.a_ready);
      {
        float4 ev[5][2];
        wide_layer(
            [&](int c00, int nkb) {
#pragma unroll
              for (int j = 0; j < 5; ++j) {
                ev[j][0] = ev[j][1] = make_float4(0.f, 0.f, 0.f, 0.f);
                if (j < nkb && live) load8(e, c00 + 8 * j, ev[j]);
              }
            },
            [&](int j, int c0, float* o) {
              if (live) store8(deg, c0, o);
              o[0] *= ev[j][0].x; o[1] *= ev[j][0].y; o[2] *= ev[j][0].z; o[3] *= ev[j][0].w;
              o[4] *= ev[j][1].x; o[5] *= ev[j][1].y; o[6] *= ev[j][1].z; o[7] *= ev[j][1].w;
              if (live) store8(dgateg, c0, o);
            },
            true);
      }
      operand_written(&sm.a_ready);
      narrow_layer(a1g, da1g);
      operand_written(&sm.a_ready);
      {
        float4 ev[5][2];
        float* bnp = sm.par;
        const uint32_t hmask = half ? 0xffff0000u : 0x0000ffffu;
        wide_layer(
            [&](int c00, int nkb) {
#pragma unroll
              for (int j = 0; j < 5; ++j) {
                ev[j][0] = ev[j][1] = make_float4(0.f, 0.f, 0.f, 0.f);
                if (j < nkb && live) load8(e, c00 + 8 * j, ev[j]);
              }
              epi_sync();
            },
            [&](int j, int c0, float* o) {
              if (live) store8(dzg, c0, o);
              const float xe[8] = {ev[j][0].x, ev[j][0].y, ev[j][0].z, ev[j][0].w, ev[j][1].x, ev[j][1].y, ev[j][1].z, ev[j][1].w};
#pragma unroll
              for (int i = 0; i < 8; ++i) {
                float s = o[i];
                float sx = o[i] * ((xe[i] - sm.mean[c0 + i]) * sm.rstd[c0 + i]);
#pragma unroll
                for (int of = 8; of > 0; of >>= 1) {
                  s += __shfl_xor_sync(hmask, s, of);
                  sx += __shfl_xor_sync(hmask, sx, of);
                }
                if (l16 == 0) { bnp[sp * 2 * E + c0 + i] = s; bnp[sp * 2 * E + E + c0 + i] = sx; }
              }
            },
            false);
      }
      epi_sync();
      for (int i = tid; i < 2 * E; i += EPI_THREADS)
        part_bn[tile * 2 * E + i] = ((double)sm.par[i] + (double)sm.par[2 * E + i]) + ((double)sm.par[4 * E + i] + (double)sm.par[6 * E + i]);
      epi_sync();
    }
    __threadfence();
    epi_sync();
    if (tid == 0) {
      const unsigned int prev = atomicAdd(arrive, 1u);
      sm.tmem_base = (prev == gridDim.x - 1) ? 1u : 0u;
    }
    epi_sync();
    if (sm.tmem_base != 0u) {
      __threadfence();
      for (int i = tid; i < 2 * E; i += EPI_THREADS) {
        double acc = 0.0;
#pragma unroll 8
        for (long long tl = 0; tl < ntiles; ++tl) acc += __ldcg(part_bn + tl * 2 * E + i);
        bn_bwd_sums[i] = acc;
        if (i < E) grads[P_BN_B + i] = (float)acc; else grads[P_BN_W + (i - E)] = (float)acc;
      }
      if (tid == 0) *arrive = 0u;
    }
  }
  umma::fence_before_sync();
  __syncthreads();
  if (warp == W_MMA) umma::tmem_dealloc(tmem, TMEM_COLS);
}


constexpr int WG_THREADS = 256;
constexpr uint32_t WG_QPART = (KE / 8) * A_LBO, WG_PPART = (KH / 8) * A_LBO;
constexpr uint32_t WG_COLS = 256;
constexpr int WG_PART = HID * E + E;
struct WgSmem {
  __align__(128) unsigned char q[2 * WG_QPART];
  __align__(128) unsigned char p[2 * WG_PPART];
  uint64_t mbar;
  uint32_t tmem_base;
};

template <int NP>
__global__ void __launch_bounds__(WG_THREADS, 1)
head_wgrad_tc_kernel(const float* __restrict__ e, const float* __restrict__ mean, const float* __restrict__ rstd, const float* __restrict__ P,
                     long long R, int rows_per_chunk, const float* __restrict__ a1g, const float* __restrict__ gateg,
                     const float* __restrict__ a2g, const float* __restrict__ yg, const float* __restrict__ da3g, const float* __restrict__ dyg,
                     const float* __restrict__ da2g, const float* __restrict__ dgateg, const float* __restrict__ da1g, float* __restrict__ part) {
  pdl_wait();
  pdl_trigger();
  extern __shared__ __align__(128) unsigned char smem_raw[];
  WgSmem& sm = *reinterpret_cast<WgSmem*>(smem_raw);
  const int layer = blockIdx.y, tid = threadIdx.x, warp = tid >> 5, lane = tid & 31;
  const long long rbeg = (long long)blockIdx.x * rows_per_chunk, rend = min(R, rbeg + rows_per_chunk);
  const float* Psrc = layer == 0 ? da3g : layer == 1 ? a2g : layer == 2 ? da2g : layer == 3 ? a1g : da1g;
  const float* Qsrc = layer == 0 ? yg : layer == 1 ? dyg : layer == 2 ? gateg : layer == 3 ? dgateg : e;
  const bool p_gelu = layer == 1 || layer == 3, wide_bias = p_gelu;
  if (tid == 0) umma::mbar_init(&sm.mbar, 1);
  if (warp == 0) umma::tmem_alloc(&sm.tmem_base, WG_COLS);
  umma::fence_before_sync();
  __syncthreads();
  umma::fence_after_sync();
  const uint32_t tmem = sm.tmem_base;
  constexpr uint32_t ID128 = umma::make_idesc_bf16(128, NN, true, true), ID64 = umma::make_idesc_bf16(64, NN, true, true);
  uint32_t phase = 0;
  bool started = false;
  for (long long t0 = rbeg; t0 < rend; t0 += ROWS) {
    const int nr = (int)min((long long)ROWS, rend - t0);
    constexpr int QITEMS = ROWS * (KE / 8), QIT = (QITEMS + WG_THREADS - 1) / WG_THREADS;
    constexpr int QBATCH = 5;
#pragma unroll 1
    for (int u0 = 0; u0 < QIT; u0 += QBATCH) {
      float4 qv[QBATCH][2], ev[QBATCH][2];
#pragma unroll
      for (int u = 0; u < QBATCH; ++u) {
        const int it = tid + (u0 + u) * WG_THREADS, r = it & (ROWS - 1), kb = it >> 6;
        qv[u][0] = qv[u][1] = ev[u][0] = ev[u][1] = make_float4(0.f, 0.f, 0.f, 0.f);
        if (u0 + u < QIT && it < QITEMS && r < nr && kb < E / 8) {
          const long long gi = (t0 + r) * E + 8 * kb;
          qv[u][0] = __ldg(reinterpret_cast<const float4*>(Qsrc + gi)); qv[u][1] = __ldg(reinterpret_cast<const float4*>(Qsrc + gi) + 1);
          if (layer == 2) { ev[u][0] = __ldg(reinterpret_cast<const float4*>(e + gi)); ev[u][1] = __ldg(reinterpret_cast<const float4*>(e + gi) + 1); }
        }
      }
#pragma unroll
      for (int u = 0; u < QBATCH; ++u) {
        const int it = tid + (u0 + u) * WG_THREADS, r = it & (ROWS - 1), kb = it >> 6;
        if (u0 + u >= QIT || it >= QITEMS) break;
        float v[8] = {qv[u][0].x, qv[u][0].y, qv[u][0].z, qv[u][0].w, qv[u][1].x, qv[u][1].y, qv[u][1].z, qv[u][1].w};
        if (r < nr) {
          if (kb < E / 8) {
            if (layer == 2) {
              v[0] *= ev[u][0].x; v[1] *= ev[u][0].y; v[2] *= ev[u][0].z; v[3] *= ev[u][0].w;
              v[4] *= ev[u][1].x; v[5] *= ev[u][1].y; v[6] *= ev[u][1].z; v[7] *= ev[u][1].w;
            } else if (layer == 4) {
#pragma unroll
              for (int i = 0; i < 8; ++i) {
                const int c = 8 * kb + i;
                v[i] = (v[i] - __ldg(mean + c)) * __ldg(rstd + c) * __ldg(P + P_BN_W + c) + __ldg(P + P_BN_B + c);
              }
            }
          } else {
            v[0] = 1.0f;
          }
        }
        split_store8<NP>(sm.q + a_off(r, kb), WG_QPART, v);
      }
    }
    for (int it = tid; it < ROWS * (KH / 8); it += WG_THREADS) {
      const int r = it & (ROWS - 1), kb = it >> 6;
      float v[8];
#pragma unroll
      for (int i = 0; i < 8; ++i) v[i] = 0.f;
      if (r < nr) {
        const float* ap = Psrc + (t0 + r) * HID + 8 * kb;
#pragma unroll
        for (int i = 0; i < 4; ++i)
          if (8 * kb + 2 * i < HID) {
            const float2 x = __ldg(reinterpret_cast<const float2*>(ap) + i);
            v[2 * i] = p_gelu ? gelu_f(x.x) : x.x; v[2 * i + 1] = p_gelu ? gelu_f(x.y) : x.y;
          }
        if (kb == HID / 8) v[HID & 7] = 1.0f;
      }
      split_store8<NP>(sm.p + a_off(r, kb), WG_PPART, v);
    }
    umma::fence_async_smem();
    umma::fence_before_sync();
    __syncthreads();
    if (warp == 0 && umma::elect_one()) {
      umma::fence_after_sync();
      const uint32_t qa = umma::smem_u32(sm.q), pa = umma::smem_u32(sm.p);
#pragma unroll
      for (int pr = 0; pr < n_products(NP); ++pr) {
        const uint32_t qo = prod_a(NP, pr) * WG_QPART, po = prod_b(NP, pr) * WG_PPART;
        const uint64_t db = umma::make_desc(pa + po, 128, A_LBO);
#pragma unroll
        for (int blk = 0; blk < 3; ++blk) {
          const uint32_t f0 = blk == 0 ? 0 : blk == 1 ? 128 : 208;
          const uint64_t da = umma::make_desc(qa + qo + (f0 / 8) * A_LBO, 128, A_LBO);
#pragma unroll
          for (int ks = 0; ks < ROWS / 16; ++ks)
            umma::mma_bf16(tmem + NN * blk, da + (uint64_t)(ks * (256 >> 4)), db + (uint64_t)(ks * (256 >> 4)), blk == 2 ? ID64 : ID128,
                           (started || pr > 0 || ks > 0) ? 1u : 0u);
        }
      }
      umma::mma_commit(&sm.mbar);
    }
    started = true;
    umma::mbar_wait(&sm.mbar, phase);
    phase ^= 1;
  }
  umma::fence_after_sync();
  float* out = part + ((long long)layer * gridDim.x + blockIdx.x) * WG_PART;
  const int sp = warp & 3, half = warp >> 2;
  float v[40];
#pragma unroll 1
  for (int blk = 0; blk < 3; ++blk) {
    const uint32_t a = tmem + NN * blk + 36 * half + ((uint32_t)(32 * sp) << 16);
    umma::tmem_ld32(a, v);
    umma::tmem_ld8(a + 32, v + 32);
    int f;
    bool ok;
    if (blk < 2) { f = 128 * blk + 32 * sp + lane; ok = true; }
    else { f = 208 + 16 * sp + lane; ok = lane < 16 && f >= 256; }
    if (ok) {
#pragma unroll
      for (int j = 0; j < 36; ++j) {
        const int n = 36 * half + j;
        const float x = started ? v[j] : 0.f;
        if (f < E) {
          if (n < HID) out[n * E + f] = x;
          else if (n == HID && wide_bias) out[HID * E + f] = x;
        } else if (f == E && !wide_bias && n < HID) {
          out[HID * E + n] = x;
        }
      }
    }
  }
  umma::fence_before_sync();
  __syncthreads();
  if (warp == 0) umma::tmem_dealloc(tmem, WG_COLS);
}

}

int headprof_read(long long* host_out32) {
#ifdef NRM_RS_PROFILE
  long long zero[32] = {0};
  NRM_CUDA(cudaDeviceSynchronize());
  NRM_CUDA(cudaMemcpyFromSymbol(host_out32, htc::g_hprof, sizeof(zero)));
  NRM_CUDA(cudaMemcpyToSymbol(htc::g_hprof, zero, sizeof(zero)));
  return NRM_OK;
#else
  (void)host_out32;
  set_error("nrm_debug_headprof: library built without -DNRM_RS_PROFILE");
  return NRM_EINVAL;
#endif
}

size_t head_tc_image_bytes() { return (size_t)10 * htc::IMG_STRIDE; }

static int head_np(int precision) { return precision == NRM_PRECISION_BF16 ? 2 : 3; }

int launch_head_images_tc(const float* P, Workspace& w, int precision, bool with_backward, cudaStream_t s) {
  unsigned char* img = reinterpret_cast<unsigned char*>(w.head_img);
  const dim3 grid(10, with_backward ? 10 : 5);
  if (head_np(precision) == 2) launch_pdl(htc::head_image_kernel<2>, grid, dim3(256), 0, s, P, img, 0, w.head_arrive);
  else launch_pdl(htc::head_image_kernel<3>, grid, dim3(256), 0, s, P, img, 0, w.head_arrive);
  NRM_LAUNCH_CHECK("head_image_kernel");
  return NRM_OK;
}

template <int NP>
static int launch_fwd(const float* P, Workspace& w, float* run_mean, float* run_var, long long* nbt, int training, int keep,
                      const double* bn_sums, long long bn_rows, float* logits, cudaStream_t s) {
  static DeviceOnce configured;
  if (configured.first_time())
    NRM_CUDA(cudaFuncSetAttribute(htc::head_forward_tc_kernel<NP>, cudaFuncAttributeMaxDynamicSharedMemorySize, (int)sizeof(htc::Smem)));
  const long long ntiles = (w.R + htc::ROWS - 1) / htc::ROWS;
  const int grid = (int)min(ntiles, (long long)sm_count());
  launch_pdl(htc::head_forward_tc_kernel<NP>, dim3(grid), dim3(htc::THREADS), sizeof(htc::Smem), s, w.e, bn_sums, bn_rows, training, run_mean,
             run_var, nbt, w.mean, w.rstd, P, reinterpret_cast<const unsigned char*>(w.head_img), w.R, keep, w.a1, w.gate, w.a2, w.y, w.a3, logits);
  NRM_LAUNCH_CHECK("head_forward_tc_kernel");
  return NRM_OK;
}

int launch_head_forward_tc(const float* P, Workspace& w, int precision, float* run_mean, float* run_var, long long* nbt, int training, int keep,
                           const double* bn_sums, long long bn_rows, float* logits, cudaStream_t s) {
  return head_np(precision) == 2 ? launch_fwd<2>(P, w, run_mean, run_var, nbt, training, keep, bn_sums, bn_rows, logits, s)
                                 : launch_fwd<3>(P, w, run_mean, run_var, nbt, training, keep, bn_sums, bn_rows, logits, s);
}


template <int NP>
static int launch_bwd(const float* P, Workspace& w, const float* dlogits, float* G, cudaStream_t s) {
  static DeviceOnce configured;
  if (configured.first_time())
    NRM_CUDA(cudaFuncSetAttribute(htc::head_backward_tc_kernel<NP>, cudaFuncAttributeMaxDynamicSharedMemorySize, (int)sizeof(htc::Smem)));
  const long long ntiles = (w.R + htc::ROWS - 1) / htc::ROWS;
  const int grid = (int)min(ntiles, (long long)sm_count());
  launch_pdl(htc::head_backward_tc_kernel<NP>, dim3(grid), dim3(htc::THREADS), sizeof(htc::Smem), s, w.e, w.mean, w.rstd, P,
             reinterpret_cast<const unsigned char*>(w.head_img), w.R, dlogits, w.a1, w.gate, w.a2, w.a3, w.da3, w.dy, w.da2, w.dgate, w.da1, w.dz,
             w.de, w.head_part_f, w.head_part_bn, w.head_arrive, G, w.bn_bwd_sums);
  NRM_LAUNCH_CHECK("head_backward_tc_kernel");
  return NRM_OK;
}


int launch_head_wgrad_tc(const float* P, Workspace& w, int precision, int rows_per_chunk, int nchunks, cudaStream_t s) {
  static DeviceOnce configured;
  if (configured.first_time()) {
    NRM_CUDA(cudaFuncSetAttribute(htc::head_wgrad_tc_kernel<1>, cudaFuncAttributeMaxDynamicSharedMemorySize, (int)sizeof(htc::WgSmem)));
    NRM_CUDA(cudaFuncSetAttribute(htc::head_wgrad_tc_kernel<2>, cudaFuncAttributeMaxDynamicSharedMemorySize, (int)sizeof(htc::WgSmem)));
  }
  if (precision == NRM_PRECISION_BF16)
    launch_pdl(htc::head_wgrad_tc_kernel<1>, dim3(nchunks, 5), dim3(htc::WG_THREADS), sizeof(htc::WgSmem), s, w.e, w.mean, w.rstd, P, w.R, rows_per_chunk,
               w.a1, w.gate, w.a2, w.y, w.da3, w.dy, w.da2, w.dgate, w.da1, w.head_part_w);
  else
    launch_pdl(htc::head_wgrad_tc_kernel<2>, dim3(nchunks, 5), dim3(htc::WG_THREADS), sizeof(htc::WgSmem), s, w.e, w.mean, w.rstd, P, w.R, rows_per_chunk,
               w.a1, w.gate, w.a2, w.y, w.da3, w.dy, w.da2, w.dgate, w.da1, w.head_part_w);
  NRM_LAUNCH_CHECK("head_wgrad_tc_kernel");
  return NRM_OK;
}

int head_tc_tiles(long long R) { return (int)((R + htc::ROWS - 1) / htc::ROWS); }
int launch_head_backward_dgrad_tc(const float* P, Workspace& w, int precision, const float* dlogits, float* G, cudaStream_t s) {
  return head_np(precision) == 2 ? launch_bwd<2>(P, w, dlogits, G, s) : launch_bwd<3>(P, w, dlogits, G, s);
}

}
```

news_recommendation_model_b200/csrc/nrm_kernels.cuh:

```cuda
#pragma once
#include "nrm_common.cuh"

namespace nrm {

struct CompactPtrs {
  const float* articles; int n_articles;
  const int* hist_article; const unsigned* hist_time; const float* hist_click;
  const int* cand_article; const unsigned* cand_time;
  const float* label32; double* label64;
};
struct BatchPtrs {
  const double* xh;
  const double* xt; long long xt_bs;
  const double* xg; long long xg_bs;
  const CompactPtrs* compact = nullptr;
};

int launch_embed_rows(const BatchPtrs& in, const float* P, Workspace& w, bool with_keys, cudaStream_t s);
int launch_table_sort(Workspace& w, cudaStream_t s);
int launch_table_grads(Workspace& w, float* grads, cudaStream_t s);
int launch_small_linear_grads(const BatchPtrs& in, Workspace& w, float* grads, cudaStream_t s);

int launch_w1_forward(const float* P, Workspace& w, cudaStream_t s);
int launch_w1_backward(const float* P, Workspace& w, float* grads, cudaStream_t s);

int launch_w1_backward_tc(const float* P, Workspace& w, float* grads, int precision, cudaStream_t s);

int launch_attention_forward(const BatchPtrs& in, const float* P, Workspace& w, int branch, int precision, cudaStream_t s);
int launch_attention_backward(const BatchPtrs& in, const float* P, Workspace& w, int branch, int precision, cudaStream_t s);
int launch_attention_finish(const float* P, Workspace& w, int branch, int precision, float* grads, cudaStream_t s);

int launch_candidate_tp(const float* P, Workspace& w, cudaStream_t s);
int launch_attention_finish_tc(const float* P, Workspace& w, float* grads, cudaStream_t s);

size_t attention_rs_image_bytes();
int rsprof_read(long long* host_out64);
int launch_attention_prep_rs(const float* P, Workspace& w, cudaStream_t s);
int launch_attention_forward_rs(const BatchPtrs& in, Workspace& w, int precision, cudaStream_t s);
int launch_attention_forward_rs_scores(Workspace& w, int precision, cudaStream_t s);
int launch_attention_backward_rs(Workspace& w, int branch, int precision, bool export_dhid, cudaStream_t s);
int launch_attention_input_grad_rs(Workspace& w, int precision, cudaStream_t s);
long long attention_rs_tiles(int B, int H, int C);

int launch_head_transpose(const float* P, Workspace& w, cudaStream_t s);
int launch_head_forward_fused(const float* P, Workspace& w, float* run_mean, float* run_var, long long* nbt, int training, int keep,
                              const double* bn_sums, long long bn_rows, float* logits, cudaStream_t s);
int launch_head_backward_dgrad(const float* P, Workspace& w, const float* dlogits, cudaStream_t s);
int launch_head_backward_bn(Workspace& w, float* grads, cudaStream_t s, int dgrad_tiles);
int launch_head_backward_wgrad(const float* P, Workspace& w, float* grads, cudaStream_t s, int dgrad_tiles, int tc_precision = 0);
int launch_head_backward_fused(const float* P, Workspace& w, const float* dlogits, float* grads, cudaStream_t s);

size_t head_tc_image_bytes();
int headprof_read(long long* host_out32);
int launch_head_images_tc(const float* P, Workspace& w, int precision, bool with_backward, cudaStream_t s);
int head_tc_tiles(long long R);
int launch_head_wgrad_tc(const float* P, Workspace& w, int precision, int rows_per_chunk, int nchunks, cudaStream_t s);
int launch_head_backward_dgrad_tc(const float* P, Workspace& w, int precision, const float* dlogits, float* grads, cudaStream_t s);
int launch_head_forward_tc(const float* P, Workspace& w, int precision, float* run_mean, float* run_var, long long* nbt, int training, int keep,
                           const double* bn_sums, long long bn_rows, float* logits, cudaStream_t s);

int launch_expand_compact(const float* articles, int n_articles, const int* hist_article, const unsigned* hist_time, const float* hist_click,
                          const int* cand_article, const unsigned* cand_time, const float* label32, long long NH, long long R,
                          double* x_history, double* x_target, double* x_global, double* label64, cudaStream_t s);

int launch_pool_topk(const float* logits, int n_models, long long model_stride, int B, int N, int k, const int* pool_article, int n_articles,
                     const int* hist_article, int H, int* pos_out, float* val_out, cudaStream_t s);

int launch_bn_partial_sums(Workspace& w, cudaStream_t s);
int launch_head_forward(const float* P, Workspace& w, float* run_mean, float* run_var, long long* nbt,
                        int training, int keep, const double* bn_sums, long long global_rows, float* logits, cudaStream_t s);
int launch_head_backward(const float* P, Workspace& w, const float* dlogits, float* grads, cudaStream_t s);
int launch_bn_backward_combine(const float* P, Workspace& w, int training, const double* bn_bwd_sums,
                               long long global_rows, bool de_holds_dx, cudaStream_t s);

}
```

news_recommendation_model_b200/csrc/nrm_loss_adam.cu:

```cuda
#include "nrm_kernels.cuh"

namespace nrm {

constexpr int LOSS_BLOCKS = 64;

struct LossScratch {
  float* dlog;
  float* drow;
  double* lpart;
  unsigned* ticket;
};
static size_t carve_loss(LossScratch& ls, void* base, int B, int C) {
  size_t off = 0;
  auto take = [&](size_t bytes) { void* p = base ? (char*)base + off : nullptr; off += (bytes + 255) & ~(size_t)255; return p; };
  ls.dlog = (float*)take(sizeof(float) * (size_t)B * C);
  ls.drow = (float*)take(sizeof(float) * (size_t)B);
  ls.lpart = (double*)take(sizeof(double) * LOSS_BLOCKS * 2);
  ls.ticket = (unsigned*)take(sizeof(unsigned));
  return off;
}

__device__ __forceinline__ float warp_max(float v) {
#pragma unroll
  for (int o = 16; o > 0; o >>= 1) v = fmaxf(v, __shfl_xor_sync(0xffffffffu, v, o));
  return v;
}
__device__ __forceinline__ float warp_sum(float v) {
#pragma unroll
  for (int o = 16; o > 0; o >>= 1) v += __shfl_xor_sync(0xffffffffu, v, o);
  return v;
}

__device__ __forceinline__ float bce_softmax_term(const float* __restrict__ out, const double* __restrict__ label, int C,
                                                  float shift, float invN, float coef, float* __restrict__ dl,
                                                  bool accumulate, float* rowsum) {
  const int lane = threadIdx.x & 31;
  float mx = -INFINITY;
  for (int c = lane; c < C; c += 32) mx = fmaxf(mx, out[c] + shift);
  mx = warp_max(mx);
  float sum = 0.f;
  for (int c = lane; c < C; c += 32) sum += expf(out[c] + shift - mx);
  sum = warp_sum(sum);
  float loss = 0.f, dot = 0.f;
  for (int c = lane; c < C; c += 32) {
    const float p = expf(out[c] + shift - mx) / sum;
    const float y = (float)label[c];
    loss -= y * fmaxf(logf(p), -100.f) + (1.f - y) * fmaxf(logf(1.f - p), -100.f);
    const float dp = (p - y) / fmaxf((1.f - p) * p, 1e-12f) * invN;
    dot = fmaf(dp, p, dot);
  }
  dot = warp_sum(dot);
  float rs = 0.f;
  for (int c = lane; c < C; c += 32) {
    const float p = expf(out[c] + shift - mx) / sum;
    const float y = (float)label[c];
    const float dp = (p - y) / fmaxf((1.f - p) * p, 1e-12f) * invN;
    const float d = coef * p * (dp - dot);
    dl[c] = accumulate ? dl[c] + d : d;
    rs += d;
  }
  *rowsum = warp_sum(rs);
  return loss;
}

__global__ void __launch_bounds__(256)
loss_forward_kernel(const float* __restrict__ logits, const float* __restrict__ delta, const long long* __restrict__ uid,
                    const double* __restrict__ label, int B, int C, long long delta_numel, float alpha, float* __restrict__ dlog,
                    float* __restrict__ drow, double* __restrict__ lpart, unsigned* __restrict__ ticket, float* __restrict__ loss) {
  pdl_wait();
  pdl_trigger();
  __shared__ double red[8][2];
  const int warp = threadIdx.x >> 5, lane = threadIdx.x & 31;
  const float invN = 1.0f / ((float)B * (float)C);
  double l1 = 0.0, l2 = 0.0;
  for (int b = blockIdx.x * 8 + warp; b < B; b += gridDim.x * 8) {
    const float* o = logits + (long long)b * C;
    const double* y = label + (long long)b * C;
    float* dl = dlog + (long long)b * C;
    const long long id = uid[b];
    const bool id_ok = id >= 0 && id < delta_numel;
    const float sh = id_ok ? delta[id] : 0.f;
    if (!id_ok) l2 = __longlong_as_double(0x7ff8000000000000LL);
    float rs1, rs2;
    const float a = bce_softmax_term(o, y, C, 0.f, invN, 1.f - alpha, dl, false, &rs1);
    __syncwarp();
    const float c = bce_softmax_term(o, y, C, sh, invN, alpha, dl, true, &rs2);
    l1 += (double)warp_sum(a);
    l2 += (double)warp_sum(c);
    if (lane == 0) drow[b] = rs2;
  }
  if (lane == 0) { red[warp][0] = l1; red[warp][1] = l2; }
  __syncthreads();
  __shared__ unsigned last_block;
  if (threadIdx.x == 0) {
    double s1 = 0.0, s2 = 0.0;
    for (int i = 0; i < 8; ++i) { s1 += red[i][0]; s2 += red[i][1]; }
    lpart[blockIdx.x * 2 + 0] = s1; lpart[blockIdx.x * 2 + 1] = s2;
    __threadfence();
    last_block = atomicAdd(ticket, 1u) == gridDim.x - 1 ? 1u : 0u;
  }
  __syncthreads();
  if (last_block != 0u && warp == 0) {
    __threadfence();
    double s1 = 0.0, s2 = 0.0;
    for (unsigned i = lane; i < gridDim.x; i += 32) { s1 += __ldcg(lpart + i * 2); s2 += __ldcg(lpart + i * 2 + 1); }
    double t1 = 0.0, t2 = 0.0;
    for (int l = 0; l < 32; ++l) { t1 += __shfl_sync(0xffffffffu, s1, l); t2 += __shfl_sync(0xffffffffu, s2, l); }
    if (lane == 0) {
      const double n = (double)B * (double)C;
      const float a = (float)(t1 / n), c = (float)(t2 / n);
      *loss = (1.f - alpha) * a + alpha * c;
      *ticket = 0u;
    }
  }
}

constexpr int LOSS_UID_STAGE = 4096;
__global__ void __launch_bounds__(256)
loss_backward_kernel(const float* __restrict__ dlog, const float* __restrict__ grad_loss, long long n, int nscale, float* __restrict__ out,
                     const long long* __restrict__ uid, const float* __restrict__ drow, int B, float* __restrict__ ddelta,
                     long long delta_numel) {
  pdl_wait();
  pdl_trigger();
  if ((int)blockIdx.x < nscale) {
    const long long i = (long long)blockIdx.x * 256 + threadIdx.x;
    if (i < n) out[i] = dlog[i] * __ldg(grad_loss);
    return;
  }
  extern __shared__ long long s_uid[];
  const bool staged = B <= LOSS_UID_STAGE;
  if (staged) {
    for (int j = threadIdx.x; j < B; j += 256) s_uid[j] = uid[j];
    __syncthreads();
  }
  const long long* ids = staged ? s_uid : uid;
  const int b = (blockIdx.x - nscale) * 8 + (threadIdx.x >> 5);
  const int lane = threadIdx.x & 31;
  if (b >= B) return;
  const long long id = ids[b];
  if (id < 0 || id >= delta_numel) return;
  bool dup = false;
  for (int j0 = 0; j0 < b && !dup; j0 += 32) {
    const int j = j0 + lane;
    dup = __any_sync(0xffffffffu, j < b && ids[j] == id);
  }
  if (dup) return;
  float acc = 0.f;
  for (int j = b + lane; j < B; j += 32) if (ids[j] == id) acc += drow[j];
  float tot = 0.f;
  for (int l = 0; l < 32; ++l) tot += __shfl_sync(0xffffffffu, acc, l);
  if (lane == 0) ddelta[id] = tot * __ldg(grad_loss);
}

__global__ void __launch_bounds__(256)
loss_backward_sparse_kernel(const float* __restrict__ dlog, const float* __restrict__ grad_loss, long long n, float* __restrict__ out,
                            const long long* __restrict__ uid, const float* __restrict__ drow, int B, long long delta_numel,
                            long long* __restrict__ suid, float* __restrict__ sval) {
  pdl_wait();
  pdl_trigger();
  const long long i = (long long)blockIdx.x * 256 + threadIdx.x;
  const float gl = __ldg(grad_loss);
  if (i < n) out[i] = dlog[i] * gl;
  if (i < B) {
    const long long id = uid[i];
    suid[i] = (id >= 0 && id < delta_numel) ? id : -1;
    sval[i] = drow[i] * gl;
  }
}

struct AdamArgs { float step_size, bc2_sqrt, beta1, beta2, eps, wd, grad_scale; };

__device__ __forceinline__ void adam_one(float& p, float g, float& m, float& v, const AdamArgs& a) {
  g = fmaf(a.wd, p, g * a.grad_scale);
  m = m + (g - m) * (1.f - a.beta1);
  v = fmaf((1.f - a.beta2) * g, g, v * a.beta2);
  const float denom = sqrtf(v) / a.bc2_sqrt + a.eps;
  p = p - a.step_size * (m / denom);
}

__global__ void __launch_bounds__(256)
adam_kernel(float* __restrict__ p, const float* __restrict__ g, float* __restrict__ m, float* __restrict__ v,
            long long n, AdamArgs a) {
  pdl_wait();
  pdl_trigger();
  const long long n4 = n >> 2;
  const long long stride = (long long)gridDim.x * 256;
  for (long long i = (long long)blockIdx.x * 256 + threadIdx.x; i < n4; i += stride) {
    float4 pp = reinterpret_cast<float4*>(p)[i];
    const float4 gg = reinterpret_cast<const float4*>(g)[i];
    float4 mm = reinterpret_cast<float4*>(m)[i];
    float4 vv = reinterpret_cast<float4*>(v)[i];
    adam_one(pp.x, gg.x, mm.x, vv.x, a); adam_one(pp.y, gg.y, mm.y, vv.y, a);
    adam_one(pp.z, gg.z, mm.z, vv.z, a); adam_one(pp.w, gg.w, mm.w, vv.w, a);
    reinterpret_cast<float4*>(p)[i] = pp; reinterpret_cast<float4*>(m)[i] = mm; reinterpret_cast<float4*>(v)[i] = vv;
  }
  for (long long i = (n4 << 2) + (long long)blockIdx.x * 256 + threadIdx.x; i < n; i += stride)
    adam_one(p[i], g[i], m[i], v[i], a);
}

__global__ void __launch_bounds__(256)
adam_scalar_kernel(float* __restrict__ p, const float* __restrict__ g, float* __restrict__ m, float* __restrict__ v,
                   long long n, AdamArgs a) {
  pdl_wait();
  pdl_trigger();
  const long long stride = (long long)gridDim.x * 256;
  for (long long i = (long long)blockIdx.x * 256 + threadIdx.x; i < n; i += stride) adam_one(p[i], g[i], m[i], v[i], a);
}

struct AdamDeviceState {
  long long step;
  float lr, beta1, beta2, eps, wd, grad_scale;
  float step_size, bc2_sqrt;
};
static_assert(sizeof(AdamDeviceState) == 40, "AdamDeviceState layout is part of the C ABI");

__global__ void adam_prepare_kernel(AdamDeviceState* st) {
  pdl_wait();
  pdl_trigger();
  if (threadIdx.x != 0 || blockIdx.x != 0) return;
  const long long t = ++st->step;
  const double bc1 = 1.0 - pow((double)st->beta1, (double)t);
  const double bc2 = 1.0 - pow((double)st->beta2, (double)t);
  st->step_size = (float)((double)st->lr / bc1);
  st->bc2_sqrt = (float)sqrt(bc2);
}

__global__ void __launch_bounds__(256)
adam_device_kernel(float* __restrict__ p, const float* __restrict__ g, float* __restrict__ m, float* __restrict__ v,
                   long long n, const AdamDeviceState* __restrict__ st) {
  pdl_wait();
  pdl_trigger();
  AdamArgs a;
  a.step_size = st->step_size; a.bc2_sqrt = st->bc2_sqrt; a.beta1 = st->beta1; a.beta2 = st->beta2;
  a.eps = st->eps; a.wd = st->wd; a.grad_scale = st->grad_scale;
  const long long n4 = n >> 2;
  const long long stride = (long long)gridDim.x * 256;
  for (long long i = (long long)blockIdx.x * 256 + threadIdx.x; i < n4; i += stride) {
    float4 pp = reinterpret_cast<float4*>(p)[i];
    const float4 gg = reinterpret_cast<const float4*>(g)[i];
    float4 mm = reinterpret_cast<float4*>(m)[i];
    float4 vv = reinterpret_cast<float4*>(v)[i];
    adam_one(pp.x, gg.x, mm.x, vv.x, a); adam_one(pp.y, gg.y, mm.y, vv.y, a);
    adam_one(pp.z, gg.z, mm.z, vv.z, a); adam_one(pp.w, gg.w, mm.w, vv.w, a);
    reinterpret_cast<float4*>(p)[i] = pp; reinterpret_cast<float4*>(m)[i] = mm; reinterpret_cast<float4*>(v)[i] = vv;
  }
  for (long long i = (n4 << 2) + (long long)blockIdx.x * 256 + threadIdx.x; i < n; i += stride)
    adam_one(p[i], g[i], m[i], v[i], a);
}

constexpr int PEER_MAX = 8;
constexpr int PEER_FLAG_BASE = 64;
enum { PEER_SLOT_READY = 0, PEER_SLOT_CONSUMED = 1, PEER_SLOT_STATS_FWD = 2, PEER_SLOT_STATS_BWD = 3 };
constexpr int BN_STATS = 2 * E;
struct PeerCtx {
  int rank, world;
  long long n;
  const float* grad[PEER_MAX];
  unsigned* pad[PEER_MAX];
  double* stats[PEER_MAX];
  const long long* suid[PEER_MAX];
  const float* sval[PEER_MAX];
  long long* acc;
  unsigned* gridbar;
  long long delta_off, delta_n;
  long long rows;
};
static_assert(sizeof(PeerCtx) == 16 + 5 * 8 * PEER_MAX + 5 * 8, "PeerCtx layout is part of the C ABI");
constexpr double DELTA_FIXED_SCALE = 17592186044416.0;

__device__ __forceinline__ void st_release_sys(unsigned* p, unsigned v) { asm volatile("st.release.sys.global.u32 [%0], %1;\n" ::"l"(p), "r"(v) : "memory"); }
__device__ __forceinline__ unsigned ld_acquire_sys(const unsigned* p) {
  unsigned v;
  asm volatile("ld.acquire.sys.global.u32 %0, [%1];\n" : "=r"(v) : "l"(p) : "memory");
  return v;
}
__device__ __forceinline__ float4 ld_peer_f4(const float* p) {
  float4 v;
  asm volatile("ld.volatile.global.v4.f32 {%0, %1, %2, %3}, [%4];\n" : "=f"(v.x), "=f"(v.y), "=f"(v.z), "=f"(v.w) : "l"(p) : "memory");
  return v;
}
__device__ __forceinline__ float ld_peer_f(const float* p) { float v; asm volatile("ld.volatile.global.f32 %0, [%1];\n" : "=f"(v) : "l"(p) : "memory"); return v; }
__device__ __forceinline__ double ld_peer_d(const double* p) { double v; asm volatile("ld.volatile.global.f64 %0, [%1];\n" : "=d"(v) : "l"(p) : "memory"); return v; }

__device__ __forceinline__ void peer_signal(const PeerCtx* c, int slot, unsigned epoch) {
  if ((int)threadIdx.x < c->world) {
    __threadfence_system();
    st_release_sys(c->pad[threadIdx.x] + PEER_FLAG_BASE + slot * PEER_MAX + c->rank, epoch);
  }
}
__device__ __forceinline__ void peer_wait(const PeerCtx* c, int slot, unsigned epoch) {
  if ((int)threadIdx.x < c->world) {
    const unsigned* p = c->pad[c->rank] + PEER_FLAG_BASE + slot * PEER_MAX + threadIdx.x;
    const long long t0 = clock64();
    while ((int)(ld_acquire_sys(p) - epoch) < 0) {
      if (clock64() - t0 > 20000000000LL) asm volatile("trap;\n");
    }
  }
}

__global__ void __launch_bounds__(256)
adam_allreduce_kernel(float* __restrict__ p, float* __restrict__ m, float* __restrict__ v, const AdamDeviceState* __restrict__ st,
                      const PeerCtx* __restrict__ c, unsigned* __restrict__ ticket) {
  pdl_wait();
  pdl_trigger();
  __shared__ int is_last;
  const unsigned epoch = (unsigned)st->step;
  if (blockIdx.x == 0) peer_signal(c, PEER_SLOT_READY, epoch);
  peer_wait(c, PEER_SLOT_READY, epoch);
  __syncthreads();
  AdamArgs a;
  a.step_size = st->step_size; a.bc2_sqrt = st->bc2_sqrt; a.beta1 = st->beta1; a.beta2 = st->beta2;
  a.eps = st->eps; a.wd = st->wd; a.grad_scale = st->grad_scale;
  const int world = c->world;
  const float inv = 1.0f / (float)world;
  const bool sparse = c->delta_n > 0;
  const long long n = sparse ? c->delta_off : c->n, n4 = n >> 2;
  const long long stride = (long long)gridDim.x * 256;
  if (sparse) {
    const long long rows = c->rows, total = rows * world;
    for (long long e = (long long)blockIdx.x * 256 + threadIdx.x; e < total; e += stride) {
      const int r = (int)(e / rows);
      const long long b = e - r * rows;
      long long id; float val;
      asm volatile("ld.volatile.global.s64 %0, [%1];\n" : "=l"(id) : "l"(c->suid[r] + b) : "memory");
      val = ld_peer_f(c->sval[r] + b);
      if (id >= 0 && id < c->delta_n) atomicAdd(reinterpret_cast<unsigned long long*>(c->acc + id), (unsigned long long)__double2ll_rn((double)val * DELTA_FIXED_SCALE));
    }
  }
  for (long long i = (long long)blockIdx.x * 256 + threadIdx.x; i < n4; i += stride) {
    float4 x[PEER_MAX];
#pragma unroll
    for (int r = 0; r < PEER_MAX; ++r)
      if (r < world) x[r] = ld_peer_f4(c->grad[r] + 4 * i);
    float4 gg = x[0];
#pragma unroll
    for (int r = 1; r < PEER_MAX; ++r)
      if (r < world) { gg.x += x[r].x; gg.y += x[r].y; gg.z += x[r].z; gg.w += x[r].w; }
    gg.x *= inv; gg.y *= inv; gg.z *= inv; gg.w *= inv;
    float4 pp = reinterpret_cast<float4*>(p)[i];
    float4 mm = reinterpret_cast<float4*>(m)[i];
    float4 vv = reinterpret_cast<float4*>(v)[i];
    adam_one(pp.x, gg.x, mm.x, vv.x, a); adam_one(pp.y, gg.y, mm.y, vv.y, a);
    adam_one(pp.z, gg.z, mm.z, vv.z, a); adam_one(pp.w, gg.w, mm.w, vv.w, a);
    reinterpret_cast<float4*>(p)[i] = pp; reinterpret_cast<float4*>(m)[i] = mm; reinterpret_cast<float4*>(v)[i] = vv;
  }
  for (long long i = (n4 << 2) + (long long)blockIdx.x * 256 + threadIdx.x; i < n; i += stride) {
    float g = ld_peer_f(c->grad[0] + i);
    for (int r = 1; r < world; ++r) g += ld_peer_f(c->grad[r] + i);
    adam_one(p[i], g * inv, m[i], v[i], a);
  }
  if (sparse) {
    __syncthreads();
    if (threadIdx.x == 0) {
      __threadfence();
      const unsigned gen = *reinterpret_cast<volatile unsigned*>(c->gridbar + 1);
      if (atomicAdd(c->gridbar, 1u) == gridDim.x - 1) {
        *reinterpret_cast<volatile unsigned*>(c->gridbar) = 0u;
        __threadfence();
        atomicAdd(c->gridbar + 1, 1u);
      } else {
        const long long t0 = clock64();
        while (*reinterpret_cast<volatile unsigned*>(c->gridbar + 1) == gen) {
          if (clock64() - t0 > 20000000000LL) asm volatile("trap;\n");
        }
      }
      __threadfence();
    }
    __syncthreads();
    const double unscale = 1.0 / DELTA_FIXED_SCALE;
    float* dp = p + c->delta_off; float* dm = m + c->delta_off; float* dv = v + c->delta_off;
    for (long long i = (long long)blockIdx.x * 256 + threadIdx.x; i < c->delta_n; i += stride) {
      const long long acc = c->acc[i];
      if (acc != 0) c->acc[i] = 0;
      adam_one(dp[i], (float)((double)acc * unscale) * inv, dm[i], dv[i], a);
    }
  }
  __syncthreads();
  if (threadIdx.x == 0) {
    __threadfence();
    is_last = atomicAdd(ticket, 1u) == gridDim.x - 1;
  }
  __syncthreads();
  if (is_last) {
    if (threadIdx.x == 0) *ticket = 0u;
    peer_signal(c, PEER_SLOT_CONSUMED, epoch);
  }
}

__global__ void peer_wait_consumed_kernel(const AdamDeviceState* __restrict__ st, const PeerCtx* __restrict__ c) {
  pdl_wait();
  pdl_trigger();
  peer_wait(c, PEER_SLOT_CONSUMED, (unsigned)st->step);
}

__global__ void __launch_bounds__(544)
peer_allsum_stats_kernel(const double* __restrict__ local, int which, double* __restrict__ out, const AdamDeviceState* __restrict__ st,
                         const PeerCtx* __restrict__ c) {
  pdl_wait();
  pdl_trigger();
  const unsigned epoch = (unsigned)st->step + 1u;
  const int t = threadIdx.x;
  double* mine = c->stats[c->rank] + which * BN_STATS;
  if (t < BN_STATS) mine[t] = local[t];
  __threadfence_system();
  __syncthreads();
  peer_signal(c, PEER_SLOT_STATS_FWD + which, epoch);
  peer_wait(c, PEER_SLOT_STATS_FWD + which, epoch);
  __syncthreads();
  if (t < BN_STATS) {
    double x[PEER_MAX];
#pragma unroll
    for (int r = 0; r < PEER_MAX; ++r)
      if (r < c->world) x[r] = ld_peer_d(c->stats[r] + which * BN_STATS + t);
    double s = 0.0;
#pragma unroll
    for (int r = 0; r < PEER_MAX; ++r)
      if (r < c->world) s += x[r];
    out[t] = s;
  }
}

}

using namespace nrm;

extern "C" size_t nrm_peer_ctx_bytes(void) { return sizeof(PeerCtx); }
extern "C" size_t nrm_peer_stats_bytes(void) { return sizeof(double) * 2 * BN_STATS; }
extern "C" int nrm_peer_flag_words(void) { return PEER_FLAG_BASE + 4 * PEER_MAX; }
extern "C" int nrm_peer_preload(void) {
  cudaFuncAttributes a;
  NRM_CUDA(cudaFuncGetAttributes(&a, adam_allreduce_kernel));
  NRM_CUDA(cudaFuncGetAttributes(&a, peer_wait_consumed_kernel));
  NRM_CUDA(cudaFuncGetAttributes(&a, peer_allsum_stats_kernel));
  NRM_CUDA(cudaFuncGetAttributes(&a, loss_backward_sparse_kernel));
  return NRM_OK;
}

extern "C" int nrm_adam_step_allreduce(float* param, float* exp_avg, float* exp_avg_sq, long long n, void* adam_state,
                                       const void* peer_ctx, void* ticket, void* stream) {
  if (!param || !exp_avg || !exp_avg_sq || !adam_state || !peer_ctx || !ticket || n <= 0) { set_error("nrm_adam_step_allreduce: bad argument"); return NRM_EINVAL; }
  if ((((uintptr_t)param | (uintptr_t)exp_avg | (uintptr_t)exp_avg_sq) & 15) != 0) { set_error("nrm_adam_step_allreduce: buffers must be 16-byte aligned"); return NRM_EINVAL; }
  cudaStream_t s = (cudaStream_t)stream;
  AdamDeviceState* st = (AdamDeviceState*)adam_state;
  launch_pdl(adam_prepare_kernel, dim3(1), dim3(32), 0, s, st);
  NRM_LAUNCH_CHECK("adam_prepare_kernel");
  long long blocks = ((n + 3) / 4 + 255) / 256;
  static DeviceOnce configured;
  static int per_sm[64];
  const int dev = current_device();
  if (configured.first_time() || per_sm[dev & 63] == 0) {
    int nb = 0;
    NRM_CUDA(cudaOccupancyMaxActiveBlocksPerMultiprocessor(&nb, adam_allreduce_kernel, 256, 0));
    per_sm[dev & 63] = nb > 0 ? nb : 1;
  }
  const long long cap = (long long)sm_count() * per_sm[dev & 63];
  if (blocks > cap) blocks = cap;
  KernelTimer t("adam", s);
  launch_pdl(adam_allreduce_kernel, dim3((int)blocks), dim3(256), 0, s, param, exp_avg, exp_avg_sq, st, (const PeerCtx*)peer_ctx, (unsigned*)ticket);
  NRM_LAUNCH_CHECK("adam_allreduce_kernel");
  return NRM_OK;
}
extern "C" int nrm_peer_wait_consumed(const void* adam_state, const void* peer_ctx, void* stream) {
  if (!adam_state || !peer_ctx) { set_error("nrm_peer_wait_consumed: bad argument"); return NRM_EINVAL; }
  launch_pdl(peer_wait_consumed_kernel, dim3(1), dim3(32), 0, (cudaStream_t)stream, (const AdamDeviceState*)adam_state, (const PeerCtx*)peer_ctx);
  NRM_LAUNCH_CHECK("peer_wait_consumed_kernel");
  return NRM_OK;
}
extern "C" int nrm_peer_allsum_stats(const double* local, int which, double* out, const void* adam_state, const void* peer_ctx, void* stream) {
  if (!local || !out || !adam_state || !peer_ctx || which < 0 || which > 1) { set_error("nrm_peer_allsum_stats: bad argument"); return NRM_EINVAL; }
  launch_pdl(peer_allsum_stats_kernel, dim3(1), dim3(544), 0, (cudaStream_t)stream, local, which, out, (const AdamDeviceState*)adam_state,
             (const PeerCtx*)peer_ctx);
  NRM_LAUNCH_CHECK("peer_allsum_stats_kernel");
  return NRM_OK;
}

extern "C" int nrm_adam_step_device(float* param, const float* grad, float* exp_avg, float* exp_avg_sq, long long n,
                                    void* adam_state, void* stream) {
  if (!param || !grad || !exp_avg || !exp_avg_sq || !adam_state || n < 0) { set_error("nrm_adam_step_device: bad argument"); return NRM_EINVAL; }
  if ((((uintptr_t)param | (uintptr_t)grad | (uintptr_t)exp_avg | (uintptr_t)exp_avg_sq) & 15) != 0) {
    set_error("nrm_adam_step_device: buffers must be 16-byte aligned"); return NRM_EINVAL;
  }
  cudaStream_t s = (cudaStream_t)stream;
  AdamDeviceState* st = (AdamDeviceState*)adam_state;
  launch_pdl(adam_prepare_kernel, dim3(1), dim3(32), 0, s, st);
  NRM_LAUNCH_CHECK("adam_prepare_kernel");
  if (n == 0) return NRM_OK;
  long long blocks = ((n + 3) / 4 + 255) / 256;
  const long long cap = (long long)sm_count() * 16;
  if (blocks > cap) blocks = cap;
  KernelTimer t("adam", s);
  launch_pdl(adam_device_kernel, dim3((int)blocks), dim3(256), 0, s, param, grad, exp_avg, exp_avg_sq, n, st);
  NRM_LAUNCH_CHECK("adam_device_kernel");
  return NRM_OK;
}

extern "C" size_t nrm_loss_scratch_bytes(int B, int C) {
  LossScratch ls;
  return carve_loss(ls, nullptr, B > 0 ? B : 1, C > 0 ? C : 1);
}

extern "C" int nrm_loss_forward(const float* logits, const float* delta, long long delta_numel, const long long* user_id,
                                const double* label, int B, int C, float alpha, float* loss, void* scratch, size_t scratch_bytes,
                                void* stream) {
  if (!logits || !delta || delta_numel <= 0 || !user_id || !label || !loss || !scratch || B <= 0 || C <= 0) {
    set_error("nrm_loss_forward: bad argument"); return NRM_EINVAL;
  }
  LossScratch ls;
  if (carve_loss(ls, scratch, B, C) > scratch_bytes) { set_error("nrm_loss_forward: scratch too small"); return NRM_EWORKSPACE; }
  cudaStream_t s = (cudaStream_t)stream;
  const int blocks = min(LOSS_BLOCKS, (B + 7) / 8);
  launch_pdl(loss_forward_kernel, dim3(blocks), dim3(256), 0, s, logits, delta, user_id, label, B, C, delta_numel, alpha, ls.dlog, ls.drow, ls.lpart,
             ls.ticket, loss);
  NRM_LAUNCH_CHECK("loss_forward_kernel");
  return NRM_OK;
}

extern "C" int nrm_loss_backward(const long long* user_id, int B, int C, const float* grad_loss, float* dlogits,
                                 float* ddelta, long long delta_numel, const void* scratch, size_t scratch_bytes, void* stream) {
  if (!user_id || !grad_loss || !dlogits || !scratch || B <= 0 || C <= 0) {
    set_error("nrm_loss_backward: bad argument"); return NRM_EINVAL;
  }
  LossScratch ls;
  if (carve_loss(ls, const_cast<void*>(scratch), B, C) > scratch_bytes) { set_error("nrm_loss_backward: scratch too small"); return NRM_EWORKSPACE; }
  cudaStream_t s = (cudaStream_t)stream;
  const long long n = (long long)B * C;
  const int nscale = (int)((n + 255) / 256);
  const bool want_delta = ddelta != nullptr && delta_numel > 0;
  if (want_delta) NRM_CUDA(cudaMemsetAsync(ddelta, 0, sizeof(float) * (size_t)delta_numel, s));
  launch_pdl(loss_backward_kernel, dim3(nscale + (want_delta ? (B + 7) / 8 : 0)), dim3(256),
             (want_delta && B <= LOSS_UID_STAGE) ? sizeof(long long) * (size_t)B : 0, s, ls.dlog, grad_loss, n, nscale, dlogits,
             user_id, ls.drow, B, ddelta, delta_numel);
  NRM_LAUNCH_CHECK("loss_backward_kernel");
  return NRM_OK;
}

extern "C" int nrm_loss_backward_sparse(const long long* user_id, int B, int C, const float* grad_loss, float* dlogits, long long delta_numel,
                                        long long* sparse_uid, float* sparse_val, const void* scratch, size_t scratch_bytes, void* stream) {
  if (!user_id || !grad_loss || !dlogits || !sparse_uid || !sparse_val || !scratch || B <= 0 || C <= 0) {
    set_error("nrm_loss_backward_sparse: bad argument"); return NRM_EINVAL;
  }
  LossScratch ls;
  if (carve_loss(ls, const_cast<void*>(scratch), B, C) > scratch_bytes) { set_error("nrm_loss_backward_sparse: scratch too small"); return NRM_EWORKSPACE; }
  const long long n = (long long)B * C;
  launch_pdl(loss_backward_sparse_kernel, dim3((int)((n + 255) / 256)), dim3(256), 0, (cudaStream_t)stream, ls.dlog, grad_loss, n, dlogits, user_id,
             ls.drow, B, delta_numel, sparse_uid, sparse_val);
  NRM_LAUNCH_CHECK("loss_backward_sparse_kernel");
  return NRM_OK;
}

extern "C" int nrm_adam_step(float* param, const float* grad, float* exp_avg, float* exp_avg_sq, long long n, float lr,
                             float beta1, float beta2, float eps, float weight_decay, long long step, float grad_scale,
                             void* stream) {
  if (!param || !grad || !exp_avg || !exp_avg_sq || n < 0 || step < 1) { set_error("nrm_adam_step: bad argument"); return NRM_EINVAL; }
  if (n == 0) return NRM_OK;
  AdamArgs a;
  const double bc1 = 1.0 - pow((double)beta1, (double)step);
  const double bc2 = 1.0 - pow((double)beta2, (double)step);
  a.step_size = (float)((double)lr / bc1);
  a.bc2_sqrt = (float)sqrt(bc2);
  a.beta1 = beta1; a.beta2 = beta2; a.eps = eps; a.wd = weight_decay; a.grad_scale = grad_scale;
  cudaStream_t s = (cudaStream_t)stream;
  const bool aligned = (((uintptr_t)param | (uintptr_t)grad | (uintptr_t)exp_avg | (uintptr_t)exp_avg_sq) & 15) == 0;
  const long long work = aligned ? (n + 3) / 4 : n;
  long long blocks = (work + 255) / 256;
  const long long cap = (long long)sm_count() * 16;
  if (blocks > cap) blocks = cap;
  KernelTimer t("adam", s);
  if (aligned) launch_pdl(adam_kernel, dim3((int)blocks), dim3(256), 0, s, param, grad, exp_avg, exp_avg_sq, n, a);
  else launch_pdl(adam_scalar_kernel, dim3((int)blocks), dim3(256), 0, s, param, grad, exp_avg, exp_avg_sq, n, a);
  NRM_LAUNCH_CHECK("adam_kernel");
  return NRM_OK;
}
```

news_recommendation_model_b200/trainer.py:

```python
from __future__ import annotations

import ctypes
import struct
from typing import List, Optional

import torch

from . import _lib, engine
from .config import HIST_COLS, TGT_COLS, GLOBAL_COLS

_p = engine._ptr


class _Slot:
    def __init__(self, B, H, C, dev):
        self.xh = torch.empty(B, H, HIST_COLS, dtype=torch.float64, device=dev)
        self.xt = torch.empty(B, C, TGT_COLS, dtype=torch.float64, device=dev)
        self.xg = torch.empty(B, C, GLOBAL_COLS, dtype=torch.float64, device=dev)
        self.label = torch.empty(B, C, dtype=torch.float64, device=dev)
        self.uid = torch.empty(B, dtype=torch.int64, device=dev)
        self.ready = torch.cuda.Event()
        self.consumed = torch.cuda.Event()
        self.graph_fb: Optional[torch.cuda.CUDAGraph] = None
        self.graph_adam: Optional[torch.cuda.CUDAGraph] = None
        self.used = False
        self.compact = None
        self.wire = 'packed'
        self.rows = B
        self.graph_wire = None


class LossHandle:

    def __init__(self, host_slot: torch.Tensor, event: torch.cuda.Event):
        self._host, self._event = host_slot, event

    def item(self) -> float:
        self._event.synchronize()
        return float(self._host.item())


class FusedTrainStep:
    SYNC_BN = True
    SPARSE_DELTA_MIN = 65536

    def __init__(self, model, B: int, H: int, C: int, *, lr=1e-3, betas=(0.9, 0.999), eps=1e-8, weight_decay=1e-5,
                 alpha=0.95, use_graph=True, ring=8, nslots=2, articles=None):
        self.model, self.B, self.H, self.C, self.alpha = model, B, H, C, float(alpha)
        self.articles = articles
        self.flat = model.flat_parameters()
        dev = self.flat.device
        self.dev, self.lib = dev, _lib.load()
        self.dp = model._dp
        world = self.dp.world if self.dp is not None else 1
        self.precision = model._precision_code()
        self.mode = engine.MODE_BN_BATCH_STATS | engine.MODE_KEEP_FOR_BWD
        self.compact_direct = self.precision != 0
        n = self.flat.total
        self.sparse_delta = self.dp is not None and self.flat.delta_numel >= self.SPARSE_DELTA_MIN
        self.peer = None
        if self.dp is not None:
            self.peer = self.dp.peer_context(n, dev, B, self.flat.fixed, self.flat.delta_numel if self.sparse_delta else 0)
        self.sparse_delta = self.sparse_delta and self.peer is not None
        self.grads = self.peer.grads if self.peer is not None else torch.zeros(n, dtype=torch.float32, device=dev)
        self.exp_avg = torch.zeros(n, dtype=torch.float32, device=dev)
        self.exp_avg_sq = torch.zeros(n, dtype=torch.float32, device=dev)
        raw = struct.pack('<q8f', 0, lr, betas[0], betas[1], eps, weight_decay, 1.0, 0.0, 0.0)
        self.adam_state = torch.frombuffer(bytearray(raw), dtype=torch.uint8).to(dev)
        ws_bytes = int(self.lib.nrm_workspace_bytes(B, H, C, self.mode))
        self.ws = torch.empty(ws_bytes, dtype=torch.uint8, device=dev)
        ls_bytes = int(self.lib.nrm_loss_scratch_bytes(B, C))
        self.loss_scratch = torch.zeros(ls_bytes, dtype=torch.uint8, device=dev)
        self.logits = torch.empty(B, C, dtype=torch.float32, device=dev)
        self.dlogits = torch.empty(B, C, dtype=torch.float32, device=dev)
        self.one = torch.ones((), dtype=torch.float32, device=dev)
        self.loss_dev = torch.zeros(ring, dtype=torch.float32, device=dev)
        self.loss_host = torch.zeros(ring, dtype=torch.float32).pin_memory()
        self.ring, self.count = ring, 0
        self.slots: List[_Slot] = [_Slot(B, H, C, dev) for _ in range(nslots)]
        self.loaded = 0
        self.copy_stream = torch.cuda.Stream(dev)
        self.use_graph = use_graph and not (self.dp is not None and self.dp.sync_bn and self.peer is None)
        self.one_graph = self.dp is None or self.peer is not None
        self.world = world
        self._tail_scratch = {}
        self._warmup()

    def _warmup(self):
        lib, m, f, s = self.lib, self.model, self.flat, self.slots[0]
        for t in (s.xh, s.xt, s.xg, s.label, s.uid):
            t.zero_()
        saved = (m.bn.running_mean.clone(), m.bn.running_var.clone(), m.bn.num_batches_tracked.clone())
        scratch_loss = self.loss_dev.new_zeros(())
        n0 = lib.nrm_launch_count()
        self._warming = True
        self._forward_backward(s, scratch_loss)
        self._warming = False
        if self.peer is not None:
            _lib.check(lib.nrm_peer_preload(), 'nrm_peer_preload')
        self.launches_per_step = int(lib.nrm_launch_count() - n0) + 2
        with torch.no_grad():
            m.bn.running_mean.copy_(saved[0]); m.bn.running_var.copy_(saved[1]); m.bn.num_batches_tracked.copy_(saved[2])
        self.grads.zero_()
        st = self.adam_state.clone()
        tiny = [torch.zeros(4, dtype=torch.float32, device=self.dev) for _ in range(4)]
        _lib.check(lib.nrm_adam_step_device(_p(tiny[0]), _p(tiny[1]), _p(tiny[2]), _p(tiny[3]), 4, _p(st),
                                            engine._stream(self.dev)), 'nrm_adam_step_device')
        torch.cuda.synchronize(self.dev)

    def _forward_backward(self, s: _Slot, loss_out: torch.Tensor, B: Optional[int] = None, loss_scratch: Optional[torch.Tensor] = None):
        lib, m, f = self.lib, self.model, self.flat
        st = engine._stream(self.dev)
        H, C = self.H, self.C
        B = self.B if B is None else B
        loss_scratch = self.loss_scratch if loss_scratch is None else loss_scratch
        warming = getattr(self, '_warming', False)
        sync_bn = self.dp is not None and self.dp.sync_bn and not warming
        direct = s.wire == 'compact' and self.compact_direct
        cb = ctypes.byref(s.cstruct) if direct else None
        if not sync_bn:
            if direct:
                _lib.check(lib.nrm_forward_compact(cb, B, H, C, _p(f.buf), _p(m.bn.running_mean), _p(m.bn.running_var),
                                                   _p(m.bn.num_batches_tracked), self.mode, self.precision, _p(self.logits), _p(self.ws),
                                                   self.ws.numel(), st), 'nrm_forward_compact')
            else:
                _lib.check(lib.nrm_forward(_p(s.xh), _p(s.xt), C * TGT_COLS, _p(s.xg), C * GLOBAL_COLS, B, H, C, _p(f.buf),
                                           _p(m.bn.running_mean), _p(m.bn.running_var), _p(m.bn.num_batches_tracked), self.mode,
                                           self.precision, _p(self.logits), _p(self.ws), self.ws.numel(), st), 'nrm_forward')
        else:
            sums = self._bn_sums(0)
            if direct:
                _lib.check(lib.nrm_forward_encoder_compact(cb, B, H, C, _p(f.buf), self.mode, self.precision, _p(sums), _p(self.ws),
                                                           self.ws.numel(), st), 'nrm_forward_encoder_compact')
            else:
                _lib.check(lib.nrm_forward_encoder(_p(s.xh), _p(s.xt), C * TGT_COLS, _p(s.xg), C * GLOBAL_COLS, B, H, C, _p(f.buf), self.mode,
                                                   self.precision, _p(sums), _p(self.ws), self.ws.numel(), st), 'nrm_forward_encoder')
            gsums = self._exchange_stats(0, sums, B * C)
            _lib.check(lib.nrm_forward_head(B, H, C, _p(f.buf), _p(m.bn.running_mean), _p(m.bn.running_var), _p(m.bn.num_batches_tracked),
                                            self.mode, self.precision, _p(gsums), B * C * self.world, _p(self.logits), _p(self.ws), self.ws.numel(), st),
                       'nrm_forward_head')
        delta = f.buf[f.fixed:f.fixed + f.delta_numel]
        _lib.check(lib.nrm_loss_forward(_p(self.logits), _p(delta), f.delta_numel, _p(s.uid), _p(s.label), B, C, self.alpha, _p(loss_out),
                                        _p(loss_scratch), loss_scratch.numel(), st), 'nrm_loss_forward')
        if self.peer is not None and not warming:
            _lib.check(lib.nrm_peer_wait_consumed(_p(self.adam_state), _p(self.peer.ctx), st), 'nrm_peer_wait_consumed')
        if self.sparse_delta and not warming:
            _lib.check(lib.nrm_loss_backward_sparse(_p(s.uid), B, C, _p(self.one), _p(self.dlogits), f.delta_numel, _p(self.peer.sparse_uid),
                                                    _p(self.peer.sparse_val), _p(loss_scratch), loss_scratch.numel(), st), 'nrm_loss_backward_sparse')
        else:
            ddelta = self.grads[f.fixed:f.fixed + f.delta_numel]
            _lib.check(lib.nrm_loss_backward(_p(s.uid), B, C, _p(self.one), _p(self.dlogits), _p(ddelta), f.delta_numel,
                                             _p(loss_scratch), loss_scratch.numel(), st), 'nrm_loss_backward')
        if not sync_bn:
            if direct:
                _lib.check(lib.nrm_backward_compact(cb, B, H, C, _p(f.buf), self.mode, self.precision, _p(self.dlogits), _p(self.grads),
                                                    _p(self.ws), self.ws.numel(), st), 'nrm_backward_compact')
            else:
                _lib.check(lib.nrm_backward(_p(s.xh), _p(s.xt), C * TGT_COLS, _p(s.xg), C * GLOBAL_COLS, B, H, C, _p(f.buf), self.mode,
                                            self.precision, _p(self.dlogits), _p(self.grads), _p(self.ws), self.ws.numel(), st),
                           'nrm_backward')
        else:
            sums = self._bn_sums(1)
            _lib.check(lib.nrm_backward_head_deferred(B, H, C, _p(f.buf), self.precision, _p(self.dlogits), _p(self.grads), _p(sums), _p(self.ws),
                                                      self.ws.numel(), st), 'nrm_backward_head_deferred')
            gsums = self._exchange_stats(1, sums, B * C)
            if direct:
                _lib.check(lib.nrm_backward_encoder_compact(cb, B, H, C, _p(f.buf), self.mode, self.precision, _p(gsums), B * C * self.world,
                                                            _p(self.grads), _p(self.ws), self.ws.numel(), st), 'nrm_backward_encoder_compact')
            else:
                _lib.check(lib.nrm_backward_encoder(_p(s.xh), _p(s.xt), C * TGT_COLS, _p(s.xg), C * GLOBAL_COLS, B, H, C, _p(f.buf), self.mode,
                                                    self.precision, _p(gsums), B * C * self.world, _p(self.grads), _p(self.ws), self.ws.numel(), st),
                           'nrm_backward_encoder')

    def _bn_sums(self, which: int) -> torch.Tensor:
        if self.peer is not None:
            return self.peer.stats_local[which]
        if not hasattr(self, '_sums_local'):
            self._sums_local = torch.zeros(2, 528, dtype=torch.float64, device=self.dev)
        return self._sums_local[which]

    def _exchange_stats(self, which: int, sums: torch.Tensor, local_rows: int) -> torch.Tensor:
        if self.peer is not None:
            out = self.peer.stats_out[which]
            _lib.check(self.lib.nrm_peer_allsum_stats(_p(sums), which, _p(out), _p(self.adam_state), _p(self.peer.ctx),
                                                      engine._stream(self.dev)), 'nrm_peer_allsum_stats')
            return out
        self.dp.all_reduce_stats(sums, local_rows)
        return sums

    def _adam(self):
        if self.peer is not None:
            _lib.check(self.lib.nrm_adam_step_allreduce(_p(self.flat.buf), _p(self.exp_avg), _p(self.exp_avg_sq), self.flat.total,
                                                        _p(self.adam_state), _p(self.peer.ctx), _p(self.peer.ticket), engine._stream(self.dev)),
                       'nrm_adam_step_allreduce')
            return
        _lib.check(self.lib.nrm_adam_step_device(_p(self.flat.buf), _p(self.grads), _p(self.exp_avg), _p(self.exp_avg_sq),
                                                 self.flat.total, _p(self.adam_state), engine._stream(self.dev)),
                   'nrm_adam_step_device')

    _ADAM_FIELDS = ('lr', 'beta1', 'beta2', 'eps', 'weight_decay', 'grad_scale')

    def _adam_host(self):
        step, lr, b1, b2, eps, wd, gs, _, _ = struct.unpack('<q8f', bytes(self.adam_state.cpu().numpy().tobytes()))
        return {'step': step, 'lr': lr, 'beta1': b1, 'beta2': b2, 'eps': eps, 'weight_decay': wd, 'grad_scale': gs}

    def set_hyper(self, **kw):
        unknown = set(kw) - set(self._ADAM_FIELDS)
        if unknown:
            raise ValueError(f'unknown Adam hyper-parameter(s): {sorted(unknown)}')
        cur = self._adam_host() if len(kw) < len(self._ADAM_FIELDS) else {}
        cur.update({k: float(v) for k, v in kw.items()})
        raw = struct.pack('<6f', *[cur[k] for k in self._ADAM_FIELDS])
        host = torch.frombuffer(bytearray(raw), dtype=torch.uint8)
        self.adam_state[8:32].copy_(host.to(self.dev, non_blocking=False))

    def set_lr(self, lr: float):
        self.set_hyper(lr=lr)

    def state_dict(self):
        torch.cuda.current_stream(self.dev).synchronize()
        return {'exp_avg': self.exp_avg.detach().clone(), 'exp_avg_sq': self.exp_avg_sq.detach().clone(), **self._adam_host(),
                'layout': [(name, off, n) for name, off, n, _ in self.flat.slots]}

    def load_state_dict(self, sd):
        if [tuple(x) for x in sd['layout']] != [(name, off, n) for name, off, n, _ in self.flat.slots]:
            raise _lib.NrmError('FusedTrainStep.load_state_dict: the saved moments use another parameter layout (user_num?)')
        self.exp_avg.copy_(sd['exp_avg']); self.exp_avg_sq.copy_(sd['exp_avg_sq'])
        raw = struct.pack('<q8f', int(sd['step']), sd['lr'], sd['beta1'], sd['beta2'], sd['eps'], sd['weight_decay'], sd['grad_scale'], 0.0, 0.0)
        self.adam_state.copy_(torch.frombuffer(bytearray(raw), dtype=torch.uint8).to(self.dev))

    def _load_compact(self, s: _Slot, batch):
        from . import wire
        if self.articles is None:
            raise _lib.NrmError('FusedTrainStep: pass articles=ArticleTable to feed CompactBatches')
        b, bh, bc = batch.shape
        if b > self.B or (bh, bc) != (self.H, self.C):
            raise ValueError(f'CompactBatch of shape {batch.shape} does not fit this step (B <= {self.B}, H = {self.H}, C = {self.C})')
        if s.compact is None:
            s.compact = wire.CompactBatch(*[torch.zeros((self.B,) + tuple(getattr(batch, f).shape[1:]), dtype=getattr(batch, f).dtype, device=self.dev)
                                            for f in batch.__dataclass_fields__])
            c = s.compact
            s.cstruct = _lib.CompactBatchStruct(self.articles.rows.data_ptr(), int(self.articles.n), c.hist_article.data_ptr(),
                                                c.hist_time.data_ptr(), c.hist_click.data_ptr(), c.cand_article.data_ptr(),
                                                c.cand_time.data_ptr(), c.label.data_ptr(), s.label.data_ptr())
            self._expand(s)
            self.copy_stream.wait_stream(torch.cuda.current_stream(self.dev))
        with torch.cuda.stream(self.copy_stream):
            if s.used:
                self.copy_stream.wait_event(s.consumed)
            fields = ('hist_article', 'hist_time', 'hist_click', 'cand_article', 'cand_time', 'label')
            if b == self.B:
                torch._foreach_copy_([getattr(s.compact, f) for f in fields] + [s.uid], [getattr(batch, f) for f in fields] + [batch.user_id],
                                     non_blocking=True)
            else:
                for f in fields:
                    getattr(s.compact, f)[:b].copy_(getattr(batch, f), non_blocking=True)
                s.uid[:b].copy_(batch.user_id, non_blocking=True)
            s.ready.record(self.copy_stream)
        loader = getattr(batch, '_loader', None)
        if loader is not None:
            ev = torch.cuda.Event()
            ev.record(self.copy_stream)
            loader.release(batch, ev)
        s.wire = 'compact'
        s.rows = b
        return s

    def _expand(self, s: _Slot):
        from . import wire
        if self.compact_direct:
            return
        wire.expand_into(self.articles, s.compact, s.xh, s.xt, s.xg, s.label)

    def load(self, batch) -> _Slot:
        s = self.slots[self.loaded % len(self.slots)]
        self.loaded += 1
        if hasattr(batch, 'hist_article'):
            return self._load_compact(s, batch)
        s.wire = 'packed'
        b = int(batch.x_history.shape[0])
        if b > self.B or tuple(batch.x_history.shape[1:]) != (self.H, HIST_COLS) or tuple(batch.x_target.shape[1:]) != (self.C, TGT_COLS):
            raise ValueError(f'batch of shape {tuple(batch.x_history.shape)} / {tuple(batch.x_target.shape)} does not fit this step '
                             f'(B <= {self.B}, H = {self.H}, C = {self.C})')
        s.rows = b
        with torch.cuda.stream(self.copy_stream):
            if s.used:
                self.copy_stream.wait_event(s.consumed)
            if b == self.B:
                torch._foreach_copy_([s.xh, s.xt, s.xg, s.label, s.uid], [batch.x_history, batch.x_target, batch.x_global, batch.label, batch.user_id],
                                     non_blocking=True)
            else:
                s.xh[:b].copy_(batch.x_history, non_blocking=True)
                s.xt[:b].copy_(batch.x_target, non_blocking=True)
                s.xg[:b].copy_(batch.x_global, non_blocking=True)
                s.label[:b].copy_(batch.label, non_blocking=True)
                s.uid[:b].copy_(batch.user_id, non_blocking=True)
            s.ready.record(self.copy_stream)
        return s

    def run(self, s: _Slot) -> LossHandle:
        cur = torch.cuda.current_stream(self.dev)
        cur.wait_event(s.ready)
        k = self.count % self.ring
        loss_out = self.loss_dev[k:k + 1]
        if s.rows != self.B:
            if self.dp is not None:
                raise _lib.NrmError('FusedTrainStep: ragged batches under data parallelism would bias the gradient average; '
                                    'drop or pad the tail')
            scratch = self._tail_scratch.get(s.rows)
            if scratch is None:
                scratch = self._tail_scratch[s.rows] = torch.zeros(int(self.lib.nrm_loss_scratch_bytes(s.rows, self.C)),
                                                                   dtype=torch.uint8, device=self.dev)
            if s.wire == 'compact':
                self._expand(s)
            self._forward_backward(s, loss_out, B=s.rows, loss_scratch=scratch)
            self._adam()
        elif self.use_graph:
            if s.graph_fb is None or s.graph_wire != s.wire:
                s.graph_fb = torch.cuda.CUDAGraph()
                s.loss_slot = self.loss_dev.new_zeros(())
                with torch.cuda.graph(s.graph_fb, capture_error_mode='thread_local'):
                    if s.wire == 'compact':
                        self._expand(s)
                    self._forward_backward(s, s.loss_slot)
                    if self.one_graph:
                        self._adam()
                s.graph_wire = s.wire
                if not self.one_graph:
                    s.graph_adam = torch.cuda.CUDAGraph()
                    with torch.cuda.graph(s.graph_adam, capture_error_mode='thread_local'):
                        self._adam()
            s.graph_fb.replay()
            if not self.one_graph:
                self.dp.buckets.reduce(self.grads, 0, self.grads.numel())
                self.dp.buckets.wait()
                s.graph_adam.replay()
            loss_out = s.loss_slot.view(1)
        else:
            if s.wire == 'compact':
                self._expand(s)
            self._forward_backward(s, loss_out)
            if self.dp is not None and self.peer is None:
                self.dp.buckets.reduce(self.grads, 0, self.grads.numel())
                self.dp.buckets.wait()
            self._adam()
        s.consumed.record(cur)
        s.used = True
        self.loss_host[k:k + 1].copy_(loss_out, non_blocking=True)
        ev = torch.cuda.Event()
        ev.record(cur)
        self.count += 1
        return LossHandle(self.loss_host[k], ev)

    def step(self, batch) -> LossHandle:
        return self.run(self.load(batch))
```

Before: 1.824 million.

## Fold softmax-BCE loss gradient into tensor-core head backward, run loss on side stream

Adds a train-backward entry point in which the tensor-core head backward kernel recomputes the per-impression softmax-BCE gradient in its epilogue from staged logits and labels, instead of reading dlogits written by a separate loss kernel. The loss forward and the delta-gradient part of the loss backward move to a side stream that overlaps with the head backward and joins at the end. This removes the serial loss-forward to loss-backward to head dependency on the critical path. In exchange each tile redundantly recomputes softmax rows and uses more shared memory, and large C falls back to the old path.

Measured after the change: 1.854 million (median of 6 runs). 1.02x the previous value.

```diff
diff --git a/include/nrm_b200.h b/include/nrm_b200.h
--- a/include/nrm_b200.h
+++ b/include/nrm_b200.h
@@ -107,6 +107,19 @@
                                  const double* bn_bwd_sums, long long bn_global_rows, float* grads, void* workspace,
                                  size_t workspace_bytes, void* stream);
 
+int nrm_train_backward(const double* x_history, const double* x_target, long long x_target_batch_stride,
+                       const double* x_global, long long x_global_batch_stride,
+                       int B, int H, int C, const float* params, int mode, int precision,
+                       const float* logits, const long long* user_id, const double* label, const float* delta, long long delta_numel,
+                       float alpha, const float* grad_loss, float* loss, void* loss_scratch, size_t loss_scratch_bytes,
+                       float* dlogits, float* grads, float* ddelta, long long* sparse_uid, float* sparse_val,
+                       void* workspace, size_t workspace_bytes, void* stream);
+int nrm_train_backward_compact(const nrm_compact_batch* batch, int B, int H, int C, const float* params, int mode, int precision,
+                               const float* logits, const long long* user_id, const double* label, const float* delta, long long delta_numel,
+                               float alpha, const float* grad_loss, float* loss, void* loss_scratch, size_t loss_scratch_bytes,
+                               float* dlogits, float* grads, float* ddelta, long long* sparse_uid, float* sparse_val,
+                               void* workspace, size_t workspace_bytes, void* stream);
+
 int nrm_forward_scores(const double* x_history, const double* x_target, long long x_target_batch_stride,
                        const double* x_global, long long x_global_batch_stride, int B, int H, int C,
                        const float* params, float* bn_running_mean, float* bn_running_var, long long* bn_num_batches_tracked,
diff --git a/news_recommendation_model_b200/_lib.py b/news_recommendation_model_b200/_lib.py
--- a/news_recommendation_model_b200/_lib.py
+++ b/news_recommendation_model_b200/_lib.py
@@ -43,6 +43,10 @@
     'nrm_backward_head': (i32, [i32, i32, i32, vp, i32, vp, vp, vp, vp, sz, vp]),
     'nrm_backward_head_deferred': (i32, [i32, i32, i32, vp, i32, vp, vp, vp, vp, sz, vp]),
     'nrm_backward_encoder': (i32, [vp, vp, ll, vp, ll, i32, i32, i32, vp, i32, i32, vp, ll, vp, vp, sz, vp]),
+    'nrm_train_backward': (i32, [vp, vp, ll, vp, ll, i32, i32, i32, vp, i32, i32, vp, vp, vp, vp, ll, f32, vp, vp, vp, sz, vp, vp, vp, vp, vp,
+                                 vp, sz, vp]),
+    'nrm_train_backward_compact': (i32, [vp, i32, i32, i32, vp, i32, i32, vp, vp, vp, vp, ll, f32, vp, vp, vp, sz, vp, vp, vp, vp, vp, vp, sz,
+                                         vp]),
     'nrm_loss_scratch_bytes': (sz, [i32, i32]),
     'nrm_loss_forward': (i32, [vp, vp, ll, vp, vp, i32, i32, f32, vp, vp, sz, vp]),
     'nrm_loss_backward': (i32, [vp, i32, i32, vp, vp, vp, ll, vp, sz, vp]),
diff --git a/news_recommendation_model_b200/csrc/nrm_api.cu b/news_recommendation_model_b200/csrc/nrm_api.cu
--- a/news_recommendation_model_b200/csrc/nrm_api.cu
+++ b/news_recommendation_model_b200/csrc/nrm_api.cu
@@ -68,7 +68,7 @@
 
 struct SideStream {
   int dev; cudaStream_t caller;
-  cudaStream_t stream; cudaEvent_t fork, join, fork2, join2, fork0, join0, join_tp, fork3, join3, fork4, join4;
+  cudaStream_t stream; cudaEvent_t fork, join, fork2, join2, fork0, join0, join_tp, fork3, join3, fork4, join4, fork_loss, join_loss;
   bool head_wgrad_pending = false; const float* wg_params = nullptr; float* wg_grads = nullptr; int wg_tiles = 0, wg_precision = 0;
 };
 static std::mutex g_side_mu;
@@ -82,7 +82,7 @@
   ss->dev = dev; ss->caller = caller;
   bool ok = cudaStreamCreateWithFlags(&ss->stream, cudaStreamNonBlocking) == cudaSuccess;
   cudaEvent_t* evs[] = {&ss->fork, &ss->join, &ss->fork2, &ss->join2, &ss->fork0, &ss->join0, &ss->join_tp, &ss->fork3, &ss->join3,
-                        &ss->fork4, &ss->join4};
+                        &ss->fork4, &ss->join4, &ss->fork_loss, &ss->join_loss};
   for (cudaEvent_t* e : evs) ok = ok && cudaEventCreateWithFlags(e, cudaEventDisableTiming) == cudaSuccess;
   if (!ok) { delete ss; return nullptr; }
   g_sides.push_back(ss);
@@ -632,7 +632,8 @@
 }
 
 static int backward_impl(const char* fn, const BatchPtrs& in, int B, int H, int C, const float* params, int mode, int precision,
-                         const float* dlogits, float* grads, void* workspace, size_t workspace_bytes, void* stream) {
+                         const float* dlogits, float* grads, void* workspace, size_t workspace_bytes, void* stream,
+                         const HeadLossArgs* la = nullptr) {
   const int training = mode & NRM_MODE_BN_BATCH_STATS;
   Workspace w;
   NRM_TRY(get_workspace(fn, w, workspace, workspace_bytes, B, H, C, NRM_MODE_KEEP_FOR_BWD));
@@ -642,7 +643,9 @@
   const bool htc = precision != NRM_PRECISION_FP32;
   const int tiles = htc ? head_tc_tiles(w.R) : 0;
   { KernelTimer t("head_backward", s);
-    if (htc) NRM_TRY(launch_head_backward_dgrad_tc(params, w, precision, dlogits, grads, s)); else NRM_TRY(launch_head_backward_dgrad(params, w, dlogits, s));
+    if (la != nullptr) NRM_TRY(launch_head_backward_dgrad_loss_tc(params, w, precision, *la, grads, s));
+    else if (htc) NRM_TRY(launch_head_backward_dgrad_tc(params, w, precision, dlogits, grads, s));
+    else NRM_TRY(launch_head_backward_dgrad(params, w, dlogits, s));
     ss->head_wgrad_pending = true; ss->wg_params = params; ss->wg_grads = grads; ss->wg_tiles = tiles; ss->wg_precision = htc ? precision : 0;
     if (!htc) NRM_TRY(launch_head_backward_bn(w, grads, s, 0)); }
   NRM_TRY(launch_bn_backward_combine(params, w, training, w.bn_bwd_sums, w.R, htc, s));
@@ -668,3 +671,72 @@
   in.compact = &cp;
   return backward_impl("nrm_backward_compact", in, B, H, C, params, mode, precision, dlogits, grads, workspace, workspace_bytes, stream);
 }
+
+static int check_fold_precision(const char* fn, int precision) {
+  if (precision != NRM_PRECISION_FP32) return NRM_OK;
+  set_error("%s: the loss is folded into the tensor-core head backward only (precision bf16 / bf16x3); use nrm_loss_forward, "
+            "nrm_loss_backward and nrm_backward", fn);
+  return NRM_EUNSUPPORTED;
+}
+
+static int train_backward_impl(const char* fn, const BatchPtrs& in, int B, int H, int C, const float* params, int mode, int precision,
+                               const float* logits, const long long* user_id, const double* label, const float* delta, long long delta_numel,
+                               float alpha, const float* grad_loss, float* loss, void* loss_scratch, size_t loss_scratch_bytes,
+                               float* dlogits, float* grads, float* ddelta, long long* sparse_uid, float* sparse_val,
+                               void* workspace, size_t workspace_bytes, void* stream) {
+  if (!params || !logits || !user_id || !label || !delta || delta_numel <= 0 || !grad_loss || !loss || !loss_scratch || !dlogits || !grads) {
+    set_error("%s: null pointer or empty delta", fn); return NRM_EINVAL;
+  }
+  const bool sparse = sparse_uid != nullptr || sparse_val != nullptr;
+  if (sparse && (!sparse_uid || !sparse_val || ddelta)) { set_error("%s: give either ddelta or both sparse_uid and sparse_val", fn); return NRM_EINVAL; }
+  if (nrm_loss_scratch_bytes(B, C) > loss_scratch_bytes) { set_error("%s: loss scratch too small", fn); return NRM_EWORKSPACE; }
+  cudaStream_t s = (cudaStream_t)stream;
+  if (C > head_tc_loss_max_c()) {
+    NRM_TRY(nrm_loss_forward(logits, delta, delta_numel, user_id, label, B, C, alpha, loss, loss_scratch, loss_scratch_bytes, stream));
+    if (sparse) NRM_TRY(launch_loss_backward_sparse(user_id, B, C, grad_loss, dlogits, delta_numel, sparse_uid, sparse_val, loss_scratch, s));
+    else NRM_TRY(launch_loss_backward(user_id, B, C, grad_loss, dlogits, ddelta, delta_numel, loss_scratch, s));
+    return backward_impl(fn, in, B, H, C, params, mode, precision, dlogits, grads, workspace, workspace_bytes, stream);
+  }
+  SideStream* ss = side_stream(s);
+  if (ss == nullptr) { set_error("%s: cannot create the side stream", fn); return NRM_ECUDA; }
+  NRM_CUDA(cudaEventRecord(ss->fork_loss, s));
+  NRM_CUDA(cudaStreamWaitEvent(ss->stream, ss->fork_loss, 0));
+  NRM_TRY(nrm_loss_forward(logits, delta, delta_numel, user_id, label, B, C, alpha, loss, loss_scratch, loss_scratch_bytes, ss->stream));
+  if (sparse) NRM_TRY(launch_loss_backward_sparse(user_id, B, C, grad_loss, nullptr, delta_numel, sparse_uid, sparse_val, loss_scratch, ss->stream));
+  else NRM_TRY(launch_loss_backward(user_id, B, C, grad_loss, nullptr, ddelta, delta_numel, loss_scratch, ss->stream));
+  NRM_CUDA(cudaEventRecord(ss->join_loss, ss->stream));
+  const HeadLossArgs la{logits, user_id, label, delta, delta_numel, alpha, grad_loss, B, C, dlogits};
+  NRM_TRY(backward_impl(fn, in, B, H, C, params, mode, precision, dlogits, grads, workspace, workspace_bytes, stream, &la));
+  NRM_CUDA(cudaStreamWaitEvent(s, ss->join_loss, 0));
+  return NRM_OK;
+}
+
+extern "C" int nrm_train_backward(const double* x_history, const double* x_target, long long xt_bs, const double* x_global, long long xg_bs,
+                                  int B, int H, int C, const float* params, int mode, int precision, const float* logits, const long long* user_id,
+                                  const double* label, const float* delta, long long delta_numel, float alpha, const float* grad_loss, float* loss,
+                                  void* loss_scratch, size_t loss_scratch_bytes, float* dlogits, float* grads, float* ddelta, long long* sparse_uid,
+                                  float* sparse_val, void* workspace, size_t workspace_bytes, void* stream) {
+  NRM_TRY(check_shape("nrm_train_backward", B, H, C));
+  NRM_TRY(check_fold_precision("nrm_train_backward", precision));
+  if (!x_history || !x_target || !x_global) { set_error("nrm_train_backward: null pointer"); return NRM_EINVAL; }
+  const BatchPtrs in{x_history, x_target, xt_bs, x_global, xg_bs};
+  return train_backward_impl("nrm_train_backward", in, B, H, C, params, mode, precision, logits, user_id, label, delta, delta_numel, alpha,
+                             grad_loss, loss, loss_scratch, loss_scratch_bytes, dlogits, grads, ddelta, sparse_uid, sparse_val, workspace,
+                             workspace_bytes, stream);
+}
+
+extern "C" int nrm_train_backward_compact(const nrm_compact_batch* batch, int B, int H, int C, const float* params, int mode, int precision,
+                                          const float* logits, const long long* user_id, const double* label, const float* delta,
+                                          long long delta_numel, float alpha, const float* grad_loss, float* loss, void* loss_scratch,
+                                          size_t loss_scratch_bytes, float* dlogits, float* grads, float* ddelta, long long* sparse_uid,
+                                          float* sparse_val, void* workspace, size_t workspace_bytes, void* stream) {
+  NRM_TRY(check_shape("nrm_train_backward_compact", B, H, C));
+  NRM_TRY(check_fold_precision("nrm_train_backward_compact", precision));
+  CompactPtrs cp;
+  NRM_TRY(compact_batch("nrm_train_backward_compact", batch, precision, cp));
+  BatchPtrs in{nullptr, nullptr, 0, nullptr, 0};
+  in.compact = &cp;
+  return train_backward_impl("nrm_train_backward_compact", in, B, H, C, params, mode, precision, logits, user_id, label, delta, delta_numel,
+                             alpha, grad_loss, loss, loss_scratch, loss_scratch_bytes, dlogits, grads, ddelta, sparse_uid, sparse_val,
+                             workspace, workspace_bytes, stream);
+}
diff --git a/news_recommendation_model_b200/csrc/nrm_head_tc.cu b/news_recommendation_model_b200/csrc/nrm_head_tc.cu
--- a/news_recommendation_model_b200/csrc/nrm_head_tc.cu
+++ b/news_recommendation_model_b200/csrc/nrm_head_tc.cu
@@ -1,6 +1,7 @@
 #include "nrm_kernels.cuh"
 #include <cstddef>
 
+#include "nrm_loss.cuh"
 #include "nrm_umma.cuh"
 
 namespace nrm {
@@ -65,6 +66,7 @@
   if (NP >= 3) *reinterpret_cast<uint4*>(dst + 2 * part_bytes) = make_uint4(l[0], l[1], l[2], l[3]);
 }
 
+#ifndef NRM_HEAD_TC_LOSS_TU
 struct ImgDesc { long long src; int so, si, narrow; };
 __constant__ ImgDesc c_img[10] = {
     {P_GATE_FC1_W, E, 1, 1},   {P_GATE_FC2_W, HID, 1, 0}, {P_MLP_FC1_W, E, 1, 1},  {P_MLP_FC2_W, HID, 1, 0}, {P_OUT_FC1_W, E, 1, 1},
@@ -103,6 +105,7 @@
     split_store8<NP>(out + off + (uint32_t)(n >> 3) * 128u + (uint32_t)(n & 7) * 16u, part, v);
   }
 }
+#endif
 
 struct Smem {
   __align__(128) unsigned char aw[3 * AW_PART];
@@ -445,16 +448,18 @@
 
 
 constexpr int HB_F = 68;
-
-template <int NP>
-__global__ void __launch_bounds__(THREADS, 1)
-head_backward_tc_kernel(const float* __restrict__ e, const float* __restrict__ mean, const float* __restrict__ rstd,
-                        const float* __restrict__ P, const unsigned char* __restrict__ img, long long R, const float* __restrict__ dr,
-                        const float* __restrict__ a1g, const float* __restrict__ gateg, const float* __restrict__ a2g,
-                        const float* __restrict__ a3g, float* __restrict__ da3g, float* __restrict__ dyg, float* __restrict__ da2g,
-                        float* __restrict__ dgateg, float* __restrict__ da1g, float* __restrict__ dzg, float* __restrict__ deg,
-                        float* __restrict__ part_f, double* __restrict__ part_bn, unsigned int* __restrict__ arrive,
-                        float* __restrict__ grads, double* __restrict__ bn_bwd_sums) {
+constexpr int LOSS_SPAN = PAR_FLOATS / 4;
+static_assert(offsetof(Smem, par) % 8 == 0, "the staged labels are doubles");
+
+template <int NP, bool kLoss>
+__device__ __forceinline__ void
+head_backward_tc(const float* __restrict__ e, const float* __restrict__ mean, const float* __restrict__ rstd,
+                 const float* __restrict__ P, const unsigned char* __restrict__ img, long long R, const float* __restrict__ dr,
+                 const float* __restrict__ a1g, const float* __restrict__ gateg, const float* __restrict__ a2g,
+                 const float* __restrict__ a3g, float* __restrict__ da3g, float* __restrict__ dyg, float* __restrict__ da2g,
+                 float* __restrict__ dgateg, float* __restrict__ da1g, float* __restrict__ dzg, float* __restrict__ deg,
+                 float* __restrict__ part_f, double* __restrict__ part_bn, unsigned int* __restrict__ arrive,
+                 float* __restrict__ grads, double* __restrict__ bn_bwd_sums, const HeadLossArgs& la) {
   pdl_wait();
   pdl_trigger();
   extern __shared__ __align__(128) unsigned char smem_raw[];
@@ -494,12 +499,48 @@
     const int row = 16 * sp + l16;
     const uint32_t tmem_lane = tmem + ((uint32_t)(32 * sp) << 16);
     for (int i = tid; i < E; i += EPI_THREADS) { sm.mean[i] = __ldg(mean + i); sm.rstd[i] = __ldg(rstd + i); }
+    float grad_loss = 0.f;
+    if constexpr (kLoss) grad_loss = __ldg(la.grad_loss);
     uint32_t duse = 0;
     for (long long t = 0; t < my_tiles; ++t) {
       const long long tile = (long long)blockIdx.x + t * gridDim.x;
       const long long r0 = tile * ROWS;
       const int nr = (int)min((long long)ROWS, R - r0);
       const bool live = row < nr;
+      if constexpr (kLoss) {
+        float* dls = sm.par;
+        float* lgs = sm.par + LOSS_SPAN;
+        double* lbs = reinterpret_cast<double*>(sm.par + 2 * LOSS_SPAN);
+        float* shs = sm.red[1];
+        const long long b0 = r0 / la.C, b1 = (r0 + nr - 1) / la.C;
+        const int nimp = (int)(b1 - b0 + 1), span = nimp * la.C;
+        const float* lg = la.logits + b0 * la.C;
+        const double* lb = la.label + b0 * la.C;
+        if (tid < nimp) {
+          const long long id = la.uid[b0 + tid];
+          shs[tid] = (id >= 0 && id < la.delta_numel) ? la.delta[id] : 0.f;
+        }
+        for (int i = tid; i < span; i += EPI_THREADS) { lgs[i] = lg[i]; lbs[i] = lb[i]; }
+        epi_sync();
+        const float invN = 1.0f / ((float)la.B * (float)la.C);
+        for (int j = warp; j < nimp; j += N_EPI) {
+          float rs1, rs2;
+          bce_softmax_term(lgs + j * la.C, lbs + j * la.C, la.C, 0.f, invN, 1.f - la.alpha, dls + j * la.C, false, &rs1);
+          __syncwarp();
+          bce_softmax_term(lgs + j * la.C, lbs + j * la.C, la.C, shs[j], invN, la.alpha, dls + j * la.C, true, &rs2);
+        }
+        epi_sync();
+        if (tid < nr) {
+          const float d = dls[r0 - b0 * la.C + tid] * grad_loss;
+          sm.red[0][tid] = d;
+          la.dlogits[r0 + tid] = d;
+        }
+        epi_sync();
+      }
+      auto dr_at = [&](int r) -> float {
+        if constexpr (kLoss) return sm.red[0][r];
+        else return __ldg(dr + r0 + r);
+      };
       float* colsum = sm.par;
       constexpr int PRO_ITEMS = ROWS * (NN / 8);
 #pragma unroll
@@ -511,7 +552,7 @@
 #pragma unroll
         for (int i = 0; i < 8; ++i) { d[i] = 0.f; tg[i] = 0.f; }
         if (r < nr) {
-          const float drr = __ldg(dr + r0 + r);
+          const float drr = dr_at(r);
           const float* ap = a3g + (r0 + r) * HID + 8 * kb;
           float av[8];
 #pragma unroll
@@ -548,7 +589,7 @@
       }
       operand_written(&sm.a_ready);
       if (warp == 0) {
-        float s = (lane < nr ? __ldg(dr + r0 + lane) : 0.f) + (lane + 32 < nr ? __ldg(dr + r0 + lane + 32) : 0.f);
+        float s = (lane < nr ? dr_at(lane) : 0.f) + (lane + 32 < nr ? dr_at(lane + 32) : 0.f);
 #pragma unroll
         for (int o = 16; o > 0; o >>= 1) s += __shfl_xor_sync(0xffffffffu, s, o);
         if (lane == 0) part_f[tile * HB_F + HID] = s;
@@ -712,6 +753,34 @@
   __syncthreads();
   if (warp == W_MMA) umma::tmem_dealloc(tmem, TMEM_COLS);
 }
+
+#ifndef NRM_HEAD_TC_LOSS_TU
+template <int NP>
+__global__ void __launch_bounds__(THREADS, 1)
+head_backward_tc_kernel(const float* __restrict__ e, const float* __restrict__ mean, const float* __restrict__ rstd,
+                        const float* __restrict__ P, const unsigned char* __restrict__ img, long long R, const float* __restrict__ dr,
+                        const float* __restrict__ a1g, const float* __restrict__ gateg, const float* __restrict__ a2g,
+                        const float* __restrict__ a3g, float* __restrict__ da3g, float* __restrict__ dyg, float* __restrict__ da2g,
+                        float* __restrict__ dgateg, float* __restrict__ da1g, float* __restrict__ dzg, float* __restrict__ deg,
+                        float* __restrict__ part_f, double* __restrict__ part_bn, unsigned int* __restrict__ arrive,
+                        float* __restrict__ grads, double* __restrict__ bn_bwd_sums) {
+  head_backward_tc<NP, false>(e, mean, rstd, P, img, R, dr, a1g, gateg, a2g, a3g, da3g, dyg, da2g, dgateg, da1g, dzg, deg, part_f, part_bn,
+                              arrive, grads, bn_bwd_sums, HeadLossArgs{});
+}
+#else
+template <int NP>
+__global__ void __launch_bounds__(THREADS, 1)
+head_backward_loss_tc_kernel(const float* __restrict__ e, const float* __restrict__ mean, const float* __restrict__ rstd,
+                             const float* __restrict__ P, const unsigned char* __restrict__ img, long long R, const float* __restrict__ a1g,
+                             const float* __restrict__ gateg, const float* __restrict__ a2g, const float* __restrict__ a3g,
+                             float* __restrict__ da3g, float* __restrict__ dyg, float* __restrict__ da2g, float* __restrict__ dgateg,
+                             float* __restrict__ da1g, float* __restrict__ dzg, float* __restrict__ deg, float* __restrict__ part_f,
+                             double* __restrict__ part_bn, unsigned int* __restrict__ arrive, float* __restrict__ grads,
+                             double* __restrict__ bn_bwd_sums, const HeadLossArgs la) {
+  head_backward_tc<NP, true>(e, mean, rstd, P, img, R, nullptr, a1g, gateg, a2g, a3g, da3g, dyg, da2g, dgateg, da1g, dzg, deg, part_f, part_bn,
+                             arrive, grads, bn_bwd_sums, la);
+}
+#endif
 
 
 constexpr int WG_THREADS = 256;
@@ -867,6 +936,9 @@
 
 }
 
+static int head_np(int precision) { return precision == NRM_PRECISION_BF16 ? 2 : 3; }
+
+#ifndef NRM_HEAD_TC_LOSS_TU
 int headprof_read(long long* host_out32) {
 #ifdef NRM_RS_PROFILE
   long long zero[32] = {0};
@@ -883,8 +955,6 @@
 
 size_t head_tc_image_bytes() { return (size_t)10 * htc::IMG_STRIDE; }
 
-static int head_np(int precision) { return precision == NRM_PRECISION_BF16 ? 2 : 3; }
-
 int launch_head_images_tc(const float* P, Workspace& w, int precision, bool with_backward, cudaStream_t s) {
   unsigned char* img = reinterpret_cast<unsigned char*>(w.head_img);
   const dim3 grid(10, with_backward ? 10 : 5);
@@ -951,4 +1021,27 @@
   return head_np(precision) == 2 ? launch_bwd<2>(P, w, dlogits, G, s) : launch_bwd<3>(P, w, dlogits, G, s);
 }
 
-}
+#else
+int head_tc_loss_max_c() { return (htc::LOSS_SPAN - htc::ROWS) / 2 + 1; }
+
+template <int NP>
+static int launch_bwd_loss(const float* P, Workspace& w, const HeadLossArgs& la, float* G, cudaStream_t s) {
+  static DeviceOnce configured;
+  if (configured.first_time())
+    NRM_CUDA(cudaFuncSetAttribute(htc::head_backward_loss_tc_kernel<NP>, cudaFuncAttributeMaxDynamicSharedMemorySize, (int)sizeof(htc::Smem)));
+  const long long ntiles = (w.R + htc::ROWS - 1) / htc::ROWS;
+  const int grid = (int)min(ntiles, (long long)sm_count());
+  launch_pdl(htc::head_backward_loss_tc_kernel<NP>, dim3(grid), dim3(htc::THREADS), sizeof(htc::Smem), s, w.e, w.mean, w.rstd, P,
+             reinterpret_cast<const unsigned char*>(w.head_img), w.R, w.a1, w.gate, w.a2, w.a3, w.da3, w.dy, w.da2, w.dgate, w.da1, w.dz,
+             w.de, w.head_part_f, w.head_part_bn, w.head_arrive, G, w.bn_bwd_sums, la);
+  NRM_LAUNCH_CHECK("head_backward_loss_tc_kernel");
+  return NRM_OK;
+}
+
+int launch_head_backward_dgrad_loss_tc(const float* P, Workspace& w, int precision, const HeadLossArgs& la, float* G, cudaStream_t s) {
+  if (la.C > head_tc_loss_max_c()) { set_error("head_backward_loss_tc_kernel: C = %d exceeds %d", la.C, head_tc_loss_max_c()); return NRM_EUNSUPPORTED; }
+  return head_np(precision) == 2 ? launch_bwd_loss<2>(P, w, la, G, s) : launch_bwd_loss<3>(P, w, la, G, s);
+}
+#endif
+
+}
diff --git a/news_recommendation_model_b200/csrc/nrm_head_tc_loss.cu b/news_recommendation_model_b200/csrc/nrm_head_tc_loss.cu
--- /dev/null
+++ b/news_recommendation_model_b200/csrc/nrm_head_tc_loss.cu
@@ -0,0 +1,2 @@
+#define NRM_HEAD_TC_LOSS_TU
+#include "nrm_head_tc.cu"
diff --git a/news_recommendation_model_b200/csrc/nrm_kernels.cuh b/news_recommendation_model_b200/csrc/nrm_kernels.cuh
--- a/news_recommendation_model_b200/csrc/nrm_kernels.cuh
+++ b/news_recommendation_model_b200/csrc/nrm_kernels.cuh
@@ -58,6 +58,13 @@
 int launch_head_backward_dgrad_tc(const float* P, Workspace& w, int precision, const float* dlogits, float* grads, cudaStream_t s);
 int launch_head_forward_tc(const float* P, Workspace& w, int precision, float* run_mean, float* run_var, long long* nbt, int training, int keep,
                            const double* bn_sums, long long bn_rows, float* logits, cudaStream_t s);
+struct HeadLossArgs {
+  const float* logits; const long long* uid; const double* label; const float* delta; long long delta_numel;
+  float alpha; const float* grad_loss; int B, C;
+  float* dlogits;
+};
+int head_tc_loss_max_c();
+int launch_head_backward_dgrad_loss_tc(const float* P, Workspace& w, int precision, const HeadLossArgs& la, float* G, cudaStream_t s);
 
 int launch_expand_compact(const float* articles, int n_articles, const int* hist_article, const unsigned* hist_time, const float* hist_click,
                           const int* cand_article, const unsigned* cand_time, const float* label32, long long NH, long long R,
@@ -65,6 +72,11 @@
 
 int launch_pool_topk(const float* logits, int n_models, long long model_stride, int B, int N, int k, const int* pool_article, int n_articles,
                      const int* hist_article, int H, int* pos_out, float* val_out, cudaStream_t s);
+
+int launch_loss_backward(const long long* user_id, int B, int C, const float* grad_loss, float* dlogits, float* ddelta, long long delta_numel,
+                         const void* scratch, cudaStream_t s);
+int launch_loss_backward_sparse(const long long* user_id, int B, int C, const float* grad_loss, float* dlogits, long long delta_numel,
+                                long long* sparse_uid, float* sparse_val, const void* scratch, cudaStream_t s);
 
 int launch_bn_partial_sums(Workspace& w, cudaStream_t s);
 int launch_head_forward(const float* P, Workspace& w, float* run_mean, float* run_var, long long* nbt,
diff --git a/news_recommendation_model_b200/csrc/nrm_loss.cuh b/news_recommendation_model_b200/csrc/nrm_loss.cuh
--- /dev/null
+++ b/news_recommendation_model_b200/csrc/nrm_loss.cuh
@@ -0,0 +1,49 @@
+#pragma once
+#include "nrm_common.cuh"
+
+namespace nrm {
+
+__device__ __forceinline__ float warp_max(float v) {
+#pragma unroll
+  for (int o = 16; o > 0; o >>= 1) v = fmaxf(v, __shfl_xor_sync(0xffffffffu, v, o));
+  return v;
+}
+__device__ __forceinline__ float warp_sum(float v) {
+#pragma unroll
+  for (int o = 16; o > 0; o >>= 1) v += __shfl_xor_sync(0xffffffffu, v, o);
+  return v;
+}
+
+__device__ __forceinline__ float bce_softmax_term(const float* __restrict__ out, const double* __restrict__ label, int C,
+                                                  float shift, float invN, float coef, float* __restrict__ dl,
+                                                  bool accumulate, float* rowsum) {
+  const int lane = threadIdx.x & 31;
+  float mx = -INFINITY;
+  for (int c = lane; c < C; c += 32) mx = fmaxf(mx, out[c] + shift);
+  mx = warp_max(mx);
+  float sum = 0.f;
+  for (int c = lane; c < C; c += 32) sum += expf(out[c] + shift - mx);
+  sum = warp_sum(sum);
+  float loss = 0.f, dot = 0.f;
+  for (int c = lane; c < C; c += 32) {
+    const float p = expf(out[c] + shift - mx) / sum;
+    const float y = (float)label[c];
+    loss -= y * fmaxf(logf(p), -100.f) + (1.f - y) * fmaxf(logf(1.f - p), -100.f);
+    const float dp = (p - y) / fmaxf((1.f - p) * p, 1e-12f) * invN;
+    dot = fmaf(dp, p, dot);
+  }
+  dot = warp_sum(dot);
+  float rs = 0.f;
+  for (int c = lane; c < C; c += 32) {
+    const float p = expf(out[c] + shift - mx) / sum;
+    const float y = (float)label[c];
+    const float dp = (p - y) / fmaxf((1.f - p) * p, 1e-12f) * invN;
+    const float d = coef * p * (dp - dot);
+    dl[c] = accumulate ? dl[c] + d : d;
+    rs += d;
+  }
+  *rowsum = warp_sum(rs);
+  return loss;
+}
+
+}
diff --git a/news_recommendation_model_b200/csrc/nrm_loss_adam.cu b/news_recommendation_model_b200/csrc/nrm_loss_adam.cu
--- a/news_recommendation_model_b200/csrc/nrm_loss_adam.cu
+++ b/news_recommendation_model_b200/csrc/nrm_loss_adam.cu
@@ -1,4 +1,5 @@
 #include "nrm_kernels.cuh"
+#include "nrm_loss.cuh"
 
 namespace nrm {
 
@@ -18,49 +19,6 @@
   ls.lpart = (double*)take(sizeof(double) * LOSS_BLOCKS * 2);
   ls.ticket = (unsigned*)take(sizeof(unsigned));
   return off;
-}
-
-__device__ __forceinline__ float warp_max(float v) {
-#pragma unroll
-  for (int o = 16; o > 0; o >>= 1) v = fmaxf(v, __shfl_xor_sync(0xffffffffu, v, o));
-  return v;
-}
-__device__ __forceinline__ float warp_sum(float v) {
-#pragma unroll
-  for (int o = 16; o > 0; o >>= 1) v += __shfl_xor_sync(0xffffffffu, v, o);
-  return v;
-}
-
-__device__ __forceinline__ float bce_softmax_term(const float* __restrict__ out, const double* __restrict__ label, int C,
-                                                  float shift, float invN, float coef, float* __restrict__ dl,
-                                                  bool accumulate, float* rowsum) {
-  const int lane = threadIdx.x & 31;
-  float mx = -INFINITY;
-  for (int c = lane; c < C; c += 32) mx = fmaxf(mx, out[c] + shift);
-  mx = warp_max(mx);
-  float sum = 0.f;
-  for (int c = lane; c < C; c += 32) sum += expf(out[c] + shift - mx);
-  sum = warp_sum(sum);
-  float loss = 0.f, dot = 0.f;
-  for (int c = lane; c < C; c += 32) {
-    const float p = expf(out[c] + shift - mx) / sum;
-    const float y = (float)label[c];
-    loss -= y * fmaxf(logf(p), -100.f) + (1.f - y) * fmaxf(logf(1.f - p), -100.f);
-    const float dp = (p - y) / fmaxf((1.f - p) * p, 1e-12f) * invN;
-    dot = fmaf(dp, p, dot);
-  }
-  dot = warp_sum(dot);
-  float rs = 0.f;
-  for (int c = lane; c < C; c += 32) {
-    const float p = expf(out[c] + shift - mx) / sum;
-    const float y = (float)label[c];
-    const float dp = (p - y) / fmaxf((1.f - p) * p, 1e-12f) * invN;
-    const float d = coef * p * (dp - dot);
-    dl[c] = accumulate ? dl[c] + d : d;
-    rs += d;
-  }
-  *rowsum = warp_sum(rs);
-  return loss;
 }
 
 __global__ void __launch_bounds__(256)
@@ -515,17 +473,16 @@
   return NRM_OK;
 }
 
-extern "C" int nrm_loss_backward(const long long* user_id, int B, int C, const float* grad_loss, float* dlogits,
-                                 float* ddelta, long long delta_numel, const void* scratch, size_t scratch_bytes, void* stream) {
-  if (!user_id || !grad_loss || !dlogits || !scratch || B <= 0 || C <= 0) {
-    set_error("nrm_loss_backward: bad argument"); return NRM_EINVAL;
-  }
+namespace nrm {
+
+int launch_loss_backward(const long long* user_id, int B, int C, const float* grad_loss, float* dlogits, float* ddelta, long long delta_numel,
+                         const void* scratch, cudaStream_t s) {
   LossScratch ls;
-  if (carve_loss(ls, const_cast<void*>(scratch), B, C) > scratch_bytes) { set_error("nrm_loss_backward: scratch too small"); return NRM_EWORKSPACE; }
-  cudaStream_t s = (cudaStream_t)stream;
+  carve_loss(ls, const_cast<void*>(scratch), B, C);
   const long long n = (long long)B * C;
-  const int nscale = (int)((n + 255) / 256);
+  const int nscale = dlogits != nullptr ? (int)((n + 255) / 256) : 0;
   const bool want_delta = ddelta != nullptr && delta_numel > 0;
+  if (nscale == 0 && !want_delta) return NRM_OK;
   if (want_delta) NRM_CUDA(cudaMemsetAsync(ddelta, 0, sizeof(float) * (size_t)delta_numel, s));
   launch_pdl(loss_backward_kernel, dim3(nscale + (want_delta ? (B + 7) / 8 : 0)), dim3(256),
              (want_delta && B <= LOSS_UID_STAGE) ? sizeof(long long) * (size_t)B : 0, s, ls.dlog, grad_loss, n, nscale, dlogits,
@@ -534,6 +491,30 @@
   return NRM_OK;
 }
 
+int launch_loss_backward_sparse(const long long* user_id, int B, int C, const float* grad_loss, float* dlogits, long long delta_numel,
+                                long long* sparse_uid, float* sparse_val, const void* scratch, cudaStream_t s) {
+  LossScratch ls;
+  carve_loss(ls, const_cast<void*>(scratch), B, C);
+  const long long n = dlogits != nullptr ? (long long)B * C : 0;
+  const long long threads = n > B ? n : B;
+  launch_pdl(loss_backward_sparse_kernel, dim3((int)((threads + 255) / 256)), dim3(256), 0, s, ls.dlog, grad_loss, n, dlogits, user_id,
+             ls.drow, B, delta_numel, sparse_uid, sparse_val);
+  NRM_LAUNCH_CHECK("loss_backward_sparse_kernel");
+  return NRM_OK;
+}
+
+}
+
+extern "C" int nrm_loss_backward(const long long* user_id, int B, int C, const float* grad_loss, float* dlogits,
+                                 float* ddelta, long long delta_numel, const void* scratch, size_t scratch_bytes, void* stream) {
+  if (!user_id || !grad_loss || !dlogits || !scratch || B <= 0 || C <= 0) {
+    set_error("nrm_loss_backward: bad argument"); return NRM_EINVAL;
+  }
+  LossScratch ls;
+  if (carve_loss(ls, const_cast<void*>(scratch), B, C) > scratch_bytes) { set_error("nrm_loss_backward: scratch too small"); return NRM_EWORKSPACE; }
+  return launch_loss_backward(user_id, B, C, grad_loss, dlogits, ddelta, delta_numel, scratch, (cudaStream_t)stream);
+}
+
 extern "C" int nrm_loss_backward_sparse(const long long* user_id, int B, int C, const float* grad_loss, float* dlogits, long long delta_numel,
                                         long long* sparse_uid, float* sparse_val, const void* scratch, size_t scratch_bytes, void* stream) {
   if (!user_id || !grad_loss || !dlogits || !sparse_uid || !sparse_val || !scratch || B <= 0 || C <= 0) {
@@ -541,11 +522,7 @@
   }
   LossScratch ls;
   if (carve_loss(ls, const_cast<void*>(scratch), B, C) > scratch_bytes) { set_error("nrm_loss_backward_sparse: scratch too small"); return NRM_EWORKSPACE; }
-  const long long n = (long long)B * C;
-  launch_pdl(loss_backward_sparse_kernel, dim3((int)((n + 255) / 256)), dim3(256), 0, (cudaStream_t)stream, ls.dlog, grad_loss, n, dlogits, user_id,
-             ls.drow, B, delta_numel, sparse_uid, sparse_val);
-  NRM_LAUNCH_CHECK("loss_backward_sparse_kernel");
-  return NRM_OK;
+  return launch_loss_backward_sparse(user_id, B, C, grad_loss, dlogits, delta_numel, sparse_uid, sparse_val, scratch, (cudaStream_t)stream);
 }
 
 extern "C" int nrm_adam_step(float* param, const float* grad, float* exp_avg, float* exp_avg_sq, long long n, float lr,
diff --git a/news_recommendation_model_b200/trainer.py b/news_recommendation_model_b200/trainer.py
--- a/news_recommendation_model_b200/trainer.py
+++ b/news_recommendation_model_b200/trainer.py
@@ -56,6 +56,7 @@
         self.precision = model._precision_code()
         self.mode = engine.MODE_BN_BATCH_STATS | engine.MODE_KEEP_FOR_BWD
         self.compact_direct = self.precision != 0
+        self.fold_loss = self.precision != 0 and not (self.dp is not None and self.dp.sync_bn)
         n = self.flat.total
         self.sparse_delta = self.dp is not None and self.flat.delta_numel >= self.SPARSE_DELTA_MIN
         self.peer = None
@@ -140,6 +141,22 @@
                                             self.mode, self.precision, _p(gsums), B * C * self.world, _p(self.logits), _p(self.ws), self.ws.numel(), st),
                        'nrm_forward_head')
         delta = f.buf[f.fixed:f.fixed + f.delta_numel]
+        if self.fold_loss:
+            if self.peer is not None and not warming:
+                _lib.check(lib.nrm_peer_wait_consumed(_p(self.adam_state), _p(self.peer.ctx), st), 'nrm_peer_wait_consumed')
+            if self.sparse_delta and not warming:
+                ddelta, suid, sval = None, _p(self.peer.sparse_uid), _p(self.peer.sparse_val)
+            else:
+                ddelta, suid, sval = _p(self.grads[f.fixed:f.fixed + f.delta_numel]), None, None
+            loss_args = (_p(self.logits), _p(s.uid), _p(s.label), _p(delta), f.delta_numel, self.alpha, _p(self.one), _p(loss_out),
+                         _p(loss_scratch), loss_scratch.numel(), _p(self.dlogits), _p(self.grads), ddelta, suid, sval, _p(self.ws),
+                         self.ws.numel(), st)
+            if direct:
+                _lib.check(lib.nrm_train_backward_compact(cb, B, H, C, _p(f.buf), self.mode, self.precision, *loss_args), 'nrm_train_backward_compact')
+            else:
+                _lib.check(lib.nrm_train_backward(_p(s.xh), _p(s.xt), C * TGT_COLS, _p(s.xg), C * GLOBAL_COLS, B, H, C, _p(f.buf), self.mode,
+                                                  self.precision, *loss_args), 'nrm_train_backward')
+            return
         _lib.check(lib.nrm_loss_forward(_p(self.logits), _p(delta), f.delta_numel, _p(s.uid), _p(s.label), B, C, self.alpha, _p(loss_out),
                                         _p(loss_scratch), loss_scratch.numel(), st), 'nrm_loss_forward')
         if self.peer is not None and not warming:
```
